# zehuichen123/Graph-DETR4D

Measured on AMD Instinct MI355X. Metric: decoder_samples_per_sec_900q_T4, higher is better.
Workload: dtype f32 (bf16x3 GEMMs)

## Files before the change

graph-detr4d_amd/csrc/gd4d_rowchain.hip:

```cpp
#include <stdlib.h>

#include "gd4d_common.h"
#include "gd4d_bf16x3.h"
#include "gd4d_pyramid_fill.h"
#include "gd4d_mha_dropout.h"
#include "gd4d_value_proj_body.h"

namespace gd4d {

GD4D_TRACE_UNIT(rowchain)

constexpr int RC_M = 16;
#ifndef RC_WAVES_N
#define RC_WAVES_N 8
#endif
#ifndef RC_TILES_N
#define RC_TILES_N 2
#endif
constexpr int RC_WAVES = RC_WAVES_N;
#ifndef RC_KPERM
#define RC_KPERM 1
#endif
#ifndef RC_LD_N
#define RC_LD_N 520
#endif
constexpr int RC_W = 512;
constexpr int RC_LD = RC_LD_N;
static_assert(RC_LD >= RC_W + 4 && RC_LD % 4 == 0, "row pitch");
constexpr int RC_KG = RC_KPERM ? 4 : 8;
constexpr int RC_K2 = RC_KPERM ? 16 : 4;
constexpr int RC_BUFS = 4;
#ifndef RC_DEPTH_N
#define RC_DEPTH_N 2
#endif
constexpr int RC_DEPTH = RC_DEPTH_N;
constexpr int RC_TILES = RC_TILES_N;
constexpr int RC_COLS = 16 * RC_TILES;
constexpr int RC_ROWS_PER_WAVE = RC_M / RC_WAVES;
static_assert((RC_TILES == 1 || RC_TILES % 2 == 0) && RC_M % RC_WAVES == 0 && RC_WAVES * RC_COLS == 256, "a pass of all waves covers 256 columns");

typedef gd4d_chain_op ChainOp;

__device__ __forceinline__ float rc_act_in(float v, int flags) { return (flags & GD4D_CHAIN_INV_SIGMOID) ? inv_sigmoid(v) : v; }

#ifndef RC_ROTATE
#define RC_ROTATE 1
#endif
#ifndef RC_PREFETCH
#define RC_PREFETCH 1
#endif
#ifndef RC_TRACE_OPS
#define RC_TRACE_OPS 0
#endif
#ifndef RC_DBG
#define RC_DBG 0
#endif
template <int PLANES>
__global__ __launch_bounds__(256) void chain_weight_image_kernel(const float* __restrict__ w, char* __restrict__ img, int N, int K) {
  const int ksteps = K / 32;
  const int frag = blockIdx.x * 4 + (threadIdx.x >> 6), lane = threadIdx.x & 63;
  const int tiles = (N + 15) / 16;
  if (frag >= tiles * ksteps) return;
  const int t = frag / ksteps, s = frag - t * ksteps;
  const int n = 16 * t + (lane & 15);
  float v[8];
#pragma unroll
  for (int j = 0; j < 8; ++j) v[j] = n < N ? w[(size_t)n * K + 32 * s + RC_KG * (lane >> 4) + (j < 4 ? j : RC_K2 + j - 4)] : 0.f;
  char* dst = img + (size_t)frag * (PLANES * 1024) + lane * 16;
  if (PLANES == 3) {
    u32x4 h, m, l;
    split8x3(v, h, m, l);
    *reinterpret_cast<u32x4*>(dst) = h;
    *reinterpret_cast<u32x4*>(dst + 1024) = m;
    *reinterpret_cast<u32x4*>(dst + 2048) = l;
  } else {
    u32x4 h, l;
    split8(v, h, l);
    *reinterpret_cast<u32x4*>(dst) = h;
    *reinterpret_cast<u32x4*>(dst + 1024) = l;
  }
}

__global__ __launch_bounds__(256) void chain_weight_image_group_kernel(const gd4d_image_job* __restrict__ jobs, int count, int total) {
  __shared__ int s_frag0[GD4D_IMAGE_JOBS_MAX];
  for (int i = threadIdx.x; i < count; i += 256) s_frag0[i] = jobs[i].frag0;
  __syncthreads();
  const int frag = blockIdx.x * 4 + (threadIdx.x >> 6), lane = threadIdx.x & 63;
  if (frag >= total) return;
  int lo = 0, hi = count - 1;
  while (lo < hi) {
    const int mid = (lo + hi + 1) >> 1;
    if (s_frag0[mid] <= frag) lo = mid; else hi = mid - 1;
  }
  const gd4d_image_job J = jobs[lo];
  const int f = frag - J.frag0;
  const int R = J.rows[0] + J.rows[1] + J.rows[2];
  auto elem = [&](int r, int c) -> float {
    if (r >= R || c >= J.cols) return 0.f;
    int j = 0;
    if (r >= J.rows[0]) { r -= J.rows[0]; j = 1; if (r >= J.rows[1]) { r -= J.rows[1]; j = 2; } }
    return J.seg[j][(size_t)r * J.cols + c];
  };
  if (J.planes == 0) {
    const int i = f * 64 + lane;
    if (i < R) static_cast<float*>(J.image)[i] = elem(i, 0);
    return;
  }
  const int N = J.transposed ? J.cols : R, K = J.transposed ? R : J.cols;
  const int ksteps = ((K + 63) & ~63) / 32;
  const int t = f / ksteps, s = f - t * ksteps;
  const int n = 16 * t + (lane & 15);
  float v[8];
  if (!J.transposed && (J.cols & 3) == 0 && RC_KG == 4) {
    float4 a = make_float4(0.f, 0.f, 0.f, 0.f), b = a;
    if (n < N) {
      int r = n, j = 0;
      if (r >= J.rows[0]) { r -= J.rows[0]; j = 1; if (r >= J.rows[1]) { r -= J.rows[1]; j = 2; } }
      const float* rowp = J.seg[j] + (size_t)r * J.cols + 32 * s + RC_KG * (lane >> 4);
      if (32 * s + RC_KG * (lane >> 4) + 3 < J.cols) a = *reinterpret_cast<const float4*>(rowp);
      if (32 * s + RC_KG * (lane >> 4) + RC_K2 + 3 < J.cols) b = *reinterpret_cast<const float4*>(rowp + RC_K2);
    }
    v[0] = a.x; v[1] = a.y; v[2] = a.z; v[3] = a.w; v[4] = b.x; v[5] = b.y; v[6] = b.z; v[7] = b.w;
  } else {
#pragma unroll
    for (int j = 0; j < 8; ++j) {
      const int k = 32 * s + RC_KG * (lane >> 4) + (j < 4 ? j : RC_K2 + j - 4);
      v[j] = n < N ? (J.transposed ? elem(k, n) : elem(n, k)) : 0.f;
    }
  }
  char* dst = static_cast<char*>(J.image) + (size_t)f * (J.planes * 1024) + lane * 16;
  if (J.planes == 3) {
    u32x4 h, m, l;
    split8x3(v, h, m, l);
    *reinterpret_cast<u32x4*>(dst) = h;
    *reinterpret_cast<u32x4*>(dst + 1024) = m;
    *reinterpret_cast<u32x4*>(dst + 2048) = l;
  } else {
    u32x4 h, l;
    split8(v, h, l);
    *reinterpret_cast<u32x4*>(dst) = h;
    *reinterpret_cast<u32x4*>(dst + 1024) = l;
  }
}

template <bool EXACT, bool TRAIN>
__device__ __forceinline__ void rc_gemm(const ChainOp& op, float (*bufs)[RC_M][RC_LD], int m0, int M, int lane, int wave) {
  constexpr int FRAG = EXACT ? 3072 : 2048;
  const int i16 = lane & 15, g = lane >> 4;
  const int K = op.K, N = op.N;
  const int steps = K / 32, tiles = (N + 15) / 16;
  const char* img = reinterpret_cast<const char*>(op.p0);
  const bool src2 = (op.flags & GD4D_CHAIN_SRC2) != 0, split_out = (op.flags & GD4D_CHAIN_SPLIT_OUT) != 0;
  const bool split_kv = (op.flags & GD4D_CHAIN_SPLIT_KV) != 0;
  const bool kv_fp32_too = (op.flags & GD4D_CHAIN_SPLIT_KV_KEEP) != 0;
  const bool mask_p2 = TRAIN && (op.flags & GD4D_CHAIN_MASK_P2) != 0;
  const float mask_scale = op.eps != 0.f ? op.eps : 1.f;
  const bool drop = TRAIN && (op.flags & GD4D_CHAIN_DROPOUT) != 0;
  const uint32_t drop_lo = drop ? reinterpret_cast<const uint32_t*>(op.p3)[0] : 0u;
  const uint32_t drop_hi = drop ? reinterpret_cast<const uint32_t*>(op.p3)[1] : 0u;
  for (int n_base = RC_COLS * wave; n_base < N; n_base += RC_COLS * RC_WAVES) {
    const float* a_row = &bufs[(src2 && n_base >= op.ld0) ? op.res : op.src][i16][RC_KG * g];
    const char* wf[RC_TILES];
#pragma unroll
    for (int c = 0; c < RC_TILES; ++c) wf[c] = img + (size_t)min(n_base / 16 + c, tiles - 1) * steps * FRAG + lane * 16;
    f32x4 acc[RC_TILES];
#pragma unroll
    for (int c = 0; c < RC_TILES; ++c) acc[c] = f32x4{0.f, 0.f, 0.f, 0.f};
    float e_bias[RC_TILES];
    {
      const float* bias_p = op.p1 ? op.p1 : reinterpret_cast<const float*>(op.p0);
      const float bias_on = op.p1 ? 1.f : 0.f;
#pragma unroll
      for (int c = 0; c < RC_TILES; ++c) e_bias[c] = bias_p[min(n_base + 16 * c + i16, N - 1)] * bias_on;
    }
    float e_add[RC_TILES][4];
    if (op.p2 && !split_out && !split_kv) {
#pragma unroll
      for (int c = 0; c < RC_TILES; ++c) {
        const int n = min(n_base + 16 * c + i16, N - 1);
#pragma unroll
        for (int r = 0; r < 4; ++r) {
          const size_t m = (size_t)min(m0 + 4 * g + r, M - 1);
          const float a2 = op.p2[m * op.ld2 + n];
          e_add[c][r] = (op.p3 && !drop) ? a2 + op.p3[m * op.ld1 + n] : a2;
        }
      }
    }
    u32x4 bh[RC_DEPTH][RC_TILES], bl[RC_DEPTH][RC_TILES], bm[EXACT ? RC_DEPTH : 1][RC_TILES];
    auto issue = [&](int slot, int j) {
      if (RC_DBG & 2) return;
#pragma unroll
      for (int c = 0; c < RC_TILES; ++c) {
        bh[slot][c] = *reinterpret_cast<const u32x4*>(wf[c] + (size_t)j * FRAG);
        if (EXACT) bm[slot][c] = *reinterpret_cast<const u32x4*>(wf[c] + (size_t)j * FRAG + 1024);
        bl[slot][c] = *reinterpret_cast<const u32x4*>(wf[c] + (size_t)j * FRAG + (EXACT ? 2048 : 1024));
      }
    };
    if (RC_DBG & 2) {
#pragma unroll
      for (int d = 0; d < RC_DEPTH; ++d)
#pragma unroll
        for (int c = 0; c < RC_TILES; ++c) { bh[d][c] = u32x4{1u, 2u, 3u, (unsigned)lane}; bl[d][c] = bh[d][c]; if (EXACT) bm[d][c] = bh[d][c]; }
    }
    const int rot = RC_ROTATE ? (int)(((unsigned)(m0 / RC_M) >> 3) % (unsigned)steps) : 0;
    auto kstep = [&](int j) { const int r = j + rot; return r >= steps ? r - steps : r; };
#pragma unroll
    for (int d = 0; d < RC_DEPTH; ++d) issue(d, kstep(min(d, steps - 1)));
    auto consume = [&](int d, int j0_) {
      const int j = kstep(j0_);
      const float4 t0 = *reinterpret_cast<const float4*>(a_row + 32 * j);
      const float4 t1 = *reinterpret_cast<const float4*>(a_row + 32 * j + RC_K2);
      const float a[8] = {t0.x, t0.y, t0.z, t0.w, t1.x, t1.y, t1.z, t1.w};
      if (EXACT) {
        u32x4 ah, am, al;
        split8x3(a, ah, am, al);
#pragma unroll
        for (int c = 0; c < RC_TILES; ++c) {
          acc[c] = __builtin_amdgcn_mfma_f32_16x16x32_bf16(frag(al), frag(bh[d][c]), acc[c], 0, 0, 0);
          acc[c] = __builtin_amdgcn_mfma_f32_16x16x32_bf16(frag(ah), frag(bl[d][c]), acc[c], 0, 0, 0);
          acc[c] = __builtin_amdgcn_mfma_f32_16x16x32_bf16(frag(am), frag(bm[d][c]), acc[c], 0, 0, 0);
          acc[c] = __builtin_amdgcn_mfma_f32_16x16x32_bf16(frag(am), frag(bh[d][c]), acc[c], 0, 0, 0);
          acc[c] = __builtin_amdgcn_mfma_f32_16x16x32_bf16(frag(ah), frag(bm[d][c]), acc[c], 0, 0, 0);
          acc[c] = __builtin_amdgcn_mfma_f32_16x16x32_bf16(frag(ah), frag(bh[d][c]), acc[c], 0, 0, 0);
        }
        return;
      }
      u32x4 ah, al;
      split8(a, ah, al);
      if (RC_DBG & 1) { asm volatile("" ::"v"(ah), "v"(al), "v"(bh[d][0]), "v"(bl[d][3])); return; }
#pragma unroll
      for (int c = 0; c < RC_TILES; ++c) {
        acc[c] = __builtin_amdgcn_mfma_f32_16x16x32_bf16(frag(ah), frag(bh[d][c]), acc[c], 0, 0, 0);
        acc[c] = __builtin_amdgcn_mfma_f32_16x16x32_bf16(frag(al), frag(bh[d][c]), acc[c], 0, 0, 0);
        acc[c] = __builtin_amdgcn_mfma_f32_16x16x32_bf16(frag(ah), frag(bl[d][c]), acc[c], 0, 0, 0);
      }
    };
    for (int j0 = 0; j0 + RC_DEPTH < steps; j0 += RC_DEPTH) {
#pragma unroll
      for (int d = 0; d < RC_DEPTH; ++d) {
        consume(d, j0 + d);
        issue(d, kstep(j0 + d + RC_DEPTH));
      }
    }
#pragma unroll
    for (int d = 0; d < RC_DEPTH; ++d) consume(d, steps - RC_DEPTH + d);
#pragma unroll
    for (int c = 0; c < RC_TILES; ++c) {
      const int n = n_base + 16 * c + i16;
      if (n >= N) continue;
      float kv[4] = {0.f, 0.f, 0.f, 0.f};
#pragma unroll
      for (int r = 0; r < 4; ++r) {
        const int row = 4 * g + r, m = m0 + row;
        float v = acc[c][r] + e_bias[c];
        if (op.flags & GD4D_CHAIN_RELU) v = fmaxf(v, 0.f);
        if (op.flags & GD4D_CHAIN_SIGMOID) v = 1.0f / (1.0f + expf(-v));
        if (drop) v = mha_drop_keep(drop_lo, drop_hi, (uint32_t)m * (uint32_t)N + (uint32_t)n, (uint32_t)op.reserved) ? v * op.eps : 0.f;
        if (mask_p2) v = e_add[c][r] > 0.f ? v * mask_scale : 0.f;
        if (op.res >= 0 && !src2) v += bufs[op.res][row][n];
        if (op.p2 && !split_out && !mask_p2 && !split_kv) v += e_add[c][r];
        if (split_kv) kv[r] = v;
        if (op.dst >= 0) bufs[op.dst][row][op.dst_col + n] = v;
        if (split_out) {
          if (m < M) {
            const int c1 = op.ldg, c2 = op.ldg + op.ld2;
            float* o = n < c1 ? op.gout + (size_t)m * op.ldg + n
                     : n < c2 ? const_cast<float*>(op.p2) + (size_t)m * op.ld2 + (n - c1)
                              : const_cast<float*>(op.p3) + (size_t)m * op.ld1 + (n - c2);
            *o = v;
          }
        } else if (op.gout && m < M && !(split_kv && !kv_fp32_too && n_base >= RC_COLS * RC_WAVES)) {
          op.gout[(size_t)m * op.ldg + n] = v;
        }
      }
      if (split_kv && n_base >= RC_COLS * RC_WAVES) {
        const unsigned h01 = cvt_pk_bf16(kv[0], kv[1]), h23 = cvt_pk_bf16(kv[2], kv[3]);
        const unsigned l01 = cvt_pk_bf16(kv[0] - __uint_as_float(h01 << 16), kv[1] - __uint_as_float(h01 & 0xffff0000u));
        const unsigned l23 = cvt_pk_bf16(kv[2] - __uint_as_float(h23 << 16), kv[3] - __uint_as_float(h23 & 0xffff0000u));
        constexpr int C3 = RC_COLS * RC_WAVES;
        const int blk = m0 / RC_M, blocks = (M + RC_M - 1) / RC_M;
        if (n_base < 2 * C3) {
          const int nn = n - C3, hd = nn >> 5, cc = nn & 31;
          unsigned short* kh = reinterpret_cast<unsigned short*>(const_cast<float*>(op.p2)) +
                               (((size_t)hd * blocks + blk) * 64 + (cc >> 3) * 16 + 4 * g) * 8 + (cc & 7);
          unsigned short* kl = kh + op.ld2;
          const unsigned hh[4] = {h01 & 0xffffu, h01 >> 16, h23 & 0xffffu, h23 >> 16};
          const unsigned ll[4] = {l01 & 0xffffu, l01 >> 16, l23 & 0xffffu, l23 >> 16};
#pragma unroll
          for (int r = 0; r < 4; ++r) { kh[r * 8] = (unsigned short)hh[r]; kl[r * 8] = (unsigned short)ll[r]; }
        } else {
          const int nn = n - 2 * C3, hd = nn >> 5, dd = nn & 31, steps = (blocks + 1) >> 1;
          unsigned short* vh = reinterpret_cast<unsigned short*>(const_cast<float*>(op.p3)) +
                               ((((size_t)hd * steps + (blk >> 1)) * 2 + (dd >> 4)) * 64 + 16 * g + (dd & 15)) * 8 + 4 * (blk & 1);
          unsigned short* vl = vh + op.ld1;
          *reinterpret_cast<uint2*>(vh) = make_uint2(h01, h23);
          *reinterpret_cast<uint2*>(vl) = make_uint2(l01, l23);
          if (blk == blocks - 1 && !(blk & 1)) {
            *reinterpret_cast<uint2*>(vh + 4) = make_uint2(0u, 0u);
            *reinterpret_cast<uint2*>(vl + 4) = make_uint2(0u, 0u);
          }
        }
      }
    }
  }
}

__device__ __forceinline__ void rc_headgemm(const ChainOp& op, float (*bufs)[RC_M][RC_LD], int m0, int M, int lane, int wave) {
  constexpr int HD = 2;
  const int i16 = lane & 15, g = lane >> 4;
  const int K = op.K, N = op.N, heads = op.ld0, Dh = N / heads;
  const int steps = K / 32, tiles = (N + 15) / 16;
  const char* img = reinterpret_cast<const char*>(op.p0);
  const int m_ld = min(m0 + i16, M - 1);
  for (int n_base = RC_COLS * wave; n_base < N; n_base += RC_COLS * RC_WAVES) {
    const char* wf[RC_TILES];
#pragma unroll
    for (int c = 0; c < RC_TILES; ++c) wf[c] = img + (size_t)min(n_base / 16 + c, tiles - 1) * steps * 2048 + lane * 16;
    constexpr int TPG = RC_TILES >= 2 ? 2 : 1;
    constexpr int NG = RC_TILES / TPG;
    int hg[NG];
    const float* ag[NG];
#pragma unroll
    for (int gi = 0; gi < NG; ++gi) {
      hg[gi] = min((n_base + 16 * TPG * gi) / Dh, heads - 1);
      ag[gi] = op.p2 + ((size_t)m_ld * heads + hg[gi]) * K + RC_KG * g;
    }
    f32x4 acc[RC_TILES];
#pragma unroll
    for (int c = 0; c < RC_TILES; ++c) acc[c] = f32x4{0.f, 0.f, 0.f, 0.f};
    float e_bias[RC_TILES];
    {
      const float* bias_p = op.p1 ? op.p1 : reinterpret_cast<const float*>(op.p0);
      const float bias_on = op.p1 ? 1.f : 0.f;
#pragma unroll
      for (int c = 0; c < RC_TILES; ++c) e_bias[c] = bias_p[min(n_base + 16 * c + i16, N - 1)] * bias_on;
    }
    float addend[RC_TILES][4];
    if (op.flags & GD4D_CHAIN_ADD_GOUT) {
#pragma unroll
      for (int c = 0; c < RC_TILES; ++c)
#pragma unroll
        for (int r = 0; r < 4; ++r)
          addend[c][r] = op.gout[(size_t)min(m0 + 4 * g + r, M - 1) * op.ldg + min(n_base + 16 * c + i16, N - 1)];
    }
    u32x4 bh[HD][RC_TILES], bl[HD][RC_TILES];
    float4 av[HD][NG][2];
    auto issue = [&](int slot, int j) {
#pragma unroll
      for (int c = 0; c < RC_TILES; ++c) {
        bh[slot][c] = *reinterpret_cast<const u32x4*>(wf[c] + (size_t)j * 2048);
        bl[slot][c] = *reinterpret_cast<const u32x4*>(wf[c] + (size_t)j * 2048 + 1024);
      }
#pragma unroll
      for (int gi = 0; gi < NG; ++gi) {
        av[slot][gi][0] = *reinterpret_cast<const float4*>(ag[gi] + 32 * j);
        av[slot][gi][1] = *reinterpret_cast<const float4*>(ag[gi] + 32 * j + RC_K2);
      }
    };
    auto consume = [&](int d) {
#pragma unroll
      for (int hh = 0; hh < NG; ++hh) {
        const float a[8] = {av[d][hh][0].x, av[d][hh][0].y, av[d][hh][0].z, av[d][hh][0].w,
                            av[d][hh][1].x, av[d][hh][1].y, av[d][hh][1].z, av[d][hh][1].w};
        u32x4 ah, al;
        split8(a, ah, al);
#pragma unroll
        for (int c = TPG * hh; c < TPG * hh + TPG; ++c) {
          acc[c] = __builtin_amdgcn_mfma_f32_16x16x32_bf16(frag(ah), frag(bh[d][c]), acc[c], 0, 0, 0);
          acc[c] = __builtin_amdgcn_mfma_f32_16x16x32_bf16(frag(al), frag(bh[d][c]), acc[c], 0, 0, 0);
          acc[c] = __builtin_amdgcn_mfma_f32_16x16x32_bf16(frag(ah), frag(bl[d][c]), acc[c], 0, 0, 0);
        }
      }
    };
#pragma unroll
    for (int d = 0; d < HD; ++d) issue(d, min(d, steps - 1));
    for (int j0 = 0; j0 + HD < steps; j0 += HD) {
#pragma unroll
      for (int d = 0; d < HD; ++d) {
        consume(d);
        issue(d, j0 + d + HD);
      }
    }
#pragma unroll
    for (int d = 0; d < HD; ++d) consume(d);
#pragma unroll
    for (int c = 0; c < RC_TILES; ++c) {
      const int n = n_base + 16 * c + i16;
      if (n >= N) continue;
      const int hc = hg[c / TPG];
#pragma unroll
      for (int r = 0; r < 4; ++r) {
        const int row = 4 * g + r, m = m0 + row;
        float v = fmaf(e_bias[c], op.p3[(size_t)min(m, M - 1) * heads + hc], acc[c][r]);
        if (op.res >= 0) v += bufs[op.res][row][n];
        if (op.flags & GD4D_CHAIN_ADD_GOUT) v += addend[c][r];
        if (op.dst >= 0) bufs[op.dst][row][op.dst_col + n] = v;
        if (op.gout && !(op.flags & GD4D_CHAIN_ADD_GOUT) && m < M) op.gout[(size_t)m * op.ldg + n] = v;
      }
    }
  }
}

__device__ __forceinline__ void rc_layernorm(const ChainOp& op, float (*bufs)[RC_M][RC_LD], int m0, int M, int lane, int wave) {
  constexpr int MAXCH = RC_W / 64;
  if (wave >= RC_M / 4) return;
  const int row = 4 * wave + (lane >> 4), l16 = lane & 15, N = op.N, nch = N / 64;
  float4 gm[MAXCH], bt[MAXCH], x[MAXCH], ad[MAXCH];
  const bool second = op.res >= 0 && op.p2;
  const size_t m_ld = (size_t)min(m0 + row, M - 1);
#pragma unroll
  for (int ch = 0; ch < MAXCH; ++ch) {
    const int n = min(64 * ch, N - 64) + 4 * l16;
    gm[ch] = *reinterpret_cast<const float4*>(op.p0 + n);
    bt[ch] = *reinterpret_cast<const float4*>(op.p1 + n);
    if (second) ad[ch] = *reinterpret_cast<const float4*>(op.p2 + m_ld * op.ld2 + n);
    x[ch] = *reinterpret_cast<const float4*>(&bufs[op.src][row][n]);
  }
  float s = 0.f;
#pragma unroll
  for (int ch = 0; ch < MAXCH; ++ch)
    if (ch < nch) s += (x[ch].x + x[ch].y) + (x[ch].z + x[ch].w);
#pragma unroll
  for (int o = 1; o < 16; o <<= 1) s += __shfl_xor(s, o);
  const float mean = s / (float)N;
  float q = 0.f;
#pragma unroll
  for (int ch = 0; ch < MAXCH; ++ch)
    if (ch < nch) {
      const float a = x[ch].x - mean, b = x[ch].y - mean, c = x[ch].z - mean, d = x[ch].w - mean;
      q += (a * a + b * b) + (c * c + d * d);
    }
#pragma unroll
  for (int o = 1; o < 16; o <<= 1) q += __shfl_xor(q, o);
  const float rstd = 1.0f / sqrtf(q / (float)N + op.eps);
  const int m = m0 + row;
  const bool relu = op.flags & GD4D_CHAIN_RELU;
#pragma unroll
  for (int ch = 0; ch < MAXCH; ++ch) {
    if (ch >= nch) break;
    const int n = 64 * ch + 4 * l16;
    float4 v;
    v.x = (x[ch].x - mean) * rstd * gm[ch].x + bt[ch].x; v.y = (x[ch].y - mean) * rstd * gm[ch].y + bt[ch].y;
    v.z = (x[ch].z - mean) * rstd * gm[ch].z + bt[ch].z; v.w = (x[ch].w - mean) * rstd * gm[ch].w + bt[ch].w;
    if (relu) { v.x = fmaxf(v.x, 0.f); v.y = fmaxf(v.y, 0.f); v.z = fmaxf(v.z, 0.f); v.w = fmaxf(v.w, 0.f); }
    if (op.dst >= 0) *reinterpret_cast<float4*>(&bufs[op.dst][row][n]) = v;
    if (op.gout && m < M) *reinterpret_cast<float4*>(op.gout + (size_t)m * op.ldg + n) = v;
    if (second)
      *reinterpret_cast<float4*>(&bufs[op.res][row][n]) = make_float4(ad[ch].x + v.x, ad[ch].y + v.y, ad[ch].z + v.z, ad[ch].w + v.w);
  }
}

__device__ __forceinline__ void rc_layernorm_bwd(const ChainOp& op, float (*bufs)[RC_M][RC_LD], float* scratch, int m0, int M, int wg,
                                                 int tid) {
  constexpr int MAXCH = RC_W / 64;
  const int lane = tid & 63, wave = tid >> 6;
  const int N = op.N, nch = N / 64;
  const bool relu = op.flags & GD4D_CHAIN_RELU;
  if (wave < RC_M / 4) {
    const int row = 4 * wave + (lane >> 4), l16 = lane & 15;
    const bool live = m0 + row < M;
    float4 gm[MAXCH], bt[MAXCH], x[MAXCH], d[MAXCH];
#pragma unroll
    for (int ch = 0; ch < MAXCH; ++ch) {
      const int n = min(64 * ch, N - 64) + 4 * l16;
      gm[ch] = *reinterpret_cast<const float4*>(op.p0 + n);
      bt[ch] = relu ? *reinterpret_cast<const float4*>(op.p1 + n) : make_float4(0.f, 0.f, 0.f, 0.f);
      x[ch] = op.p3 ? *reinterpret_cast<const float4*>(op.p3 + (size_t)min(m0 + row, M - 1) * op.ld1 + n)
                    : *reinterpret_cast<const float4*>(&bufs[op.res][row][n]);
      d[ch] = *reinterpret_cast<const float4*>(&bufs[op.src][row][n]);
      if (!live) d[ch] = make_float4(0.f, 0.f, 0.f, 0.f);
    }
    float s = 0.f;
#pragma unroll
    for (int ch = 0; ch < MAXCH; ++ch)
      if (ch < nch) s += (x[ch].x + x[ch].y) + (x[ch].z + x[ch].w);
#pragma unroll
    for (int o = 1; o < 16; o <<= 1) s += __shfl_xor(s, o);
    const float mean = s / (float)N;
    float q = 0.f;
#pragma unroll
    for (int ch = 0; ch < MAXCH; ++ch)
      if (ch < nch) {
        const float a = x[ch].x - mean, b = x[ch].y - mean, c = x[ch].z - mean, e = x[ch].w - mean;
        q += (a * a + b * b) + (c * c + e * e);
      }
#pragma unroll
    for (int o = 1; o < 16; o <<= 1) q += __shfl_xor(q, o);
    const float rstd = 1.0f / sqrtf(q / (float)N + op.eps);
    float s1 = 0.f, s2 = 0.f;
    float4 xh[MAXCH], g[MAXCH];
#pragma unroll
    for (int ch = 0; ch < MAXCH; ++ch) {
      xh[ch] = make_float4((x[ch].x - mean) * rstd, (x[ch].y - mean) * rstd, (x[ch].z - mean) * rstd, (x[ch].w - mean) * rstd);
      if (relu) {
        if (xh[ch].x * gm[ch].x + bt[ch].x <= 0.f) d[ch].x = 0.f;
        if (xh[ch].y * gm[ch].y + bt[ch].y <= 0.f) d[ch].y = 0.f;
        if (xh[ch].z * gm[ch].z + bt[ch].z <= 0.f) d[ch].z = 0.f;
        if (xh[ch].w * gm[ch].w + bt[ch].w <= 0.f) d[ch].w = 0.f;
      }
      g[ch] = make_float4(d[ch].x * gm[ch].x, d[ch].y * gm[ch].y, d[ch].z * gm[ch].z, d[ch].w * gm[ch].w);
      if (ch < nch) {
        s1 += (g[ch].x + g[ch].y) + (g[ch].z + g[ch].w);
        s2 += (g[ch].x * xh[ch].x + g[ch].y * xh[ch].y) + (g[ch].z * xh[ch].z + g[ch].w * xh[ch].w);
      }
    }
#pragma unroll
    for (int o = 1; o < 16; o <<= 1) { s1 += __shfl_xor(s1, o); s2 += __shfl_xor(s2, o); }
    const float m1 = s1 / (float)N, m2 = s2 / (float)N;
    const int m = m0 + row;
#pragma unroll
    for (int ch = 0; ch < MAXCH; ++ch) {
      if (ch >= nch) break;
      const int n = 64 * ch + 4 * l16;
      const float4 v = make_float4(rstd * (g[ch].x - m1 - xh[ch].x * m2), rstd * (g[ch].y - m1 - xh[ch].y * m2),
                                   rstd * (g[ch].z - m1 - xh[ch].z * m2), rstd * (g[ch].w - m1 - xh[ch].w * m2));
      if (op.dst >= 0) *reinterpret_cast<float4*>(&bufs[op.dst][row][n]) = v;
      if (op.gout && m < M) *reinterpret_cast<float4*>(op.gout + (size_t)m * op.ldg + n) = v;
      if (op.p2) {
        float4 a = make_float4(d[ch].x * xh[ch].x, d[ch].y * xh[ch].y, d[ch].z * xh[ch].z, d[ch].w * xh[ch].w), b = d[ch];
#pragma unroll
        for (int o = 16; o < 64; o <<= 1) {
          a.x += __shfl_xor(a.x, o); a.y += __shfl_xor(a.y, o); a.z += __shfl_xor(a.z, o); a.w += __shfl_xor(a.w, o);
          b.x += __shfl_xor(b.x, o); b.y += __shfl_xor(b.y, o); b.z += __shfl_xor(b.z, o); b.w += __shfl_xor(b.w, o);
        }
        if (lane < 16) {
          *reinterpret_cast<float4*>(scratch + (wave * 2 + 0) * RC_W + n) = a;
          *reinterpret_cast<float4*>(scratch + (wave * 2 + 1) * RC_W + n) = b;
        }
      }
    }
  }
  if (!op.p2) return;
  __syncthreads();
  float* part = const_cast<float*>(op.p2);
  for (int e = tid; e < 2 * N; e += 64 * RC_WAVES) {
    const int k = e / N, c = e - k * N;
    const float t = (scratch[(0 * 2 + k) * RC_W + c] + scratch[(1 * 2 + k) * RC_W + c]) +
                    (scratch[(2 * 2 + k) * RC_W + c] + scratch[(3 * 2 + k) * RC_W + c]);
    part[((size_t)wg * 2 + k) * N + c] = t;
  }
}

template <bool IS_ADD, bool TRAIN>
__device__ __forceinline__ void rc_rows(const ChainOp& op, float (*bufs)[RC_M][RC_LD], int m0, int M, int lane, int wave) {
  const int N = op.N;
  const float* ga = IS_ADD ? op.p2 : op.p0;
  const float* gb = IS_ADD ? nullptr : op.p1;
  const int lda = IS_ADD ? op.ld2 : op.ld0, ldb = op.ld1;
  float4 va[RC_ROWS_PER_WAVE][2], vb[RC_ROWS_PER_WAVE][2];
#pragma unroll
  for (int r = 0; r < RC_ROWS_PER_WAVE; ++r) {
    const int m = min(m0 + RC_ROWS_PER_WAVE * wave + r, M - 1);
#pragma unroll
    for (int cb = 0; cb < 2; ++cb) {
      const int n = min(256 * cb + 4 * lane, N - 4);
      va[r][cb] = ga ? *reinterpret_cast<const float4*>(ga + (size_t)m * lda + n) : make_float4(0.f, 0.f, 0.f, 0.f);
      vb[r][cb] = gb ? *reinterpret_cast<const float4*>(gb + (size_t)m * ldb + n) : make_float4(0.f, 0.f, 0.f, 0.f);
    }
  }
#pragma unroll
  for (int r = 0; r < RC_ROWS_PER_WAVE; ++r) {
    const int row = RC_ROWS_PER_WAVE * wave + r;
#pragma unroll
    for (int cb = 0; cb < 2; ++cb) {
      const int n = 256 * cb + 4 * lane;
      if (n >= N) continue;
      float4 v = va[r][cb];
      if (!IS_ADD && (op.flags & GD4D_CHAIN_INV_SIGMOID)) { v.x = inv_sigmoid(v.x); v.y = inv_sigmoid(v.y); v.z = inv_sigmoid(v.z); v.w = inv_sigmoid(v.w); }
      v.x += vb[r][cb].x; v.y += vb[r][cb].y; v.z += vb[r][cb].z; v.w += vb[r][cb].w;
      if (IS_ADD) {
        const float4 s0 = *reinterpret_cast<const float4*>(&bufs[op.src][row][n]);
        v.x += s0.x; v.y += s0.y; v.z += s0.z; v.w += s0.w;
        if (op.res >= 0) {
          const float4 s1 = *reinterpret_cast<const float4*>(&bufs[op.res][row][n]);
          v.x += s1.x; v.y += s1.y; v.z += s1.z; v.w += s1.w;
        }
      }
      *reinterpret_cast<float4*>(&bufs[op.dst][row][(IS_ADD ? 0 : op.dst_col) + n]) = v;
      if (TRAIN && op.gout && m0 + row < M) *reinterpret_cast<float4*>(op.gout + (size_t)(m0 + row) * op.ldg + n) = v;
    }
  }
}

struct ChainProgram {
  int nops, M, nops2, split;
  ChainOp ops[GD4D_CHAIN_MAX_OPS];
};

#if defined(__HIP_DEVICE_COMPILE__)
typedef const __attribute__((address_space(4))) ChainProgram* rc_prog_ptr_t;
#else
typedef const ChainProgram* rc_prog_ptr_t;
#endif

template <bool TRAIN>
__device__ __forceinline__ void row_chain_body(const rc_prog_ptr_t pp, const int bx) {
  const int M = pp->M, split = pp->split;
  const int blocks = (M + RC_M - 1) / RC_M;
  if (split > 0 && bx >= blocks && bx < split) return;
  const bool second = split > 0 && bx >= split;
  const int op_base = second ? pp->nops : 0;
  const int nops = second ? pp->nops2 : pp->nops;
  const int wg = second ? bx - split : bx;
  const int wg_lo = second ? split : 0, wg_hi = wg_lo + blocks;
  extern __shared__ __attribute__((aligned(16))) char rc_smem[];
  float (*bufs)[RC_M][RC_LD] = reinterpret_cast<float (*)[RC_M][RC_LD]>(rc_smem);
  const int tid = threadIdx.x, lane = tid & 63, wave = tid >> 6;
  const int m0 = wg * RC_M;
  trace_mark_if(g_trace_rowchain, (second ? 7ull : 1ull) | ((unsigned long long)nops << 8), wg == 0);
#if RC_PREFETCH
  typedef __attribute__((address_space(3))) void rc_lds_void_t;
  typedef const __attribute__((address_space(1))) void rc_glb_void_t;
  rc_lds_void_t* rc_dump = (rc_lds_void_t*)(rc_smem + sizeof(float) * RC_BUFS * RC_M * RC_LD + 256 * wave);
  auto touch1 = [&](const char* q) { __builtin_amdgcn_global_load_lds((rc_glb_void_t*)q, rc_dump, 4, 0, 0); };
  const unsigned xcd = (unsigned)bx & 7u;
  const unsigned first = (unsigned)wg_lo + ((xcd - (unsigned)wg_lo) & 7u);
  const unsigned mine = ((unsigned)bx - first) >> 3, share = ((unsigned)wg_hi - 1u - first) / 8u + 1u;
  auto touch = [&](const void* base, size_t bytes) {
    if (!base || bytes < 4) return;
    const char* b = reinterpret_cast<const char*>(base);
    const unsigned pieces = (unsigned)((bytes + 63) / 64) + 1u;
    for (unsigned c = tid; c < pieces; c += 64 * RC_WAVES) touch1(b + min((size_t)c * 64, bytes - 4));
  };
  auto touch_small = [&](int from) {
    const int rows = min(RC_M, M - m0);
    for (int oi = from; oi < op_base + nops; ++oi) {
      const ChainOp& o = pp->ops[oi];
      const size_t nb = (size_t)o.N * 4;
      switch (o.kind) {
        case GD4D_CHAIN_LOAD:
          for (int r = 0; r < rows; ++r) {
            touch(o.p0 + (size_t)(m0 + r) * o.ld0, nb);
            if (o.p1) touch(o.p1 + (size_t)(m0 + r) * o.ld1, nb);
          }
          break;
        case GD4D_CHAIN_ADD:
          if (o.p2) for (int r = 0; r < rows; ++r) touch(o.p2 + (size_t)(m0 + r) * o.ld2, nb);
          break;
        case GD4D_CHAIN_GEMM: touch(o.p1, nb); break;
        case GD4D_CHAIN_HEADGEMM: touch(o.p1, nb); touch(o.p3 + (size_t)m0 * o.ld0, (size_t)rows * o.ld0 * 4); break;
        case GD4D_CHAIN_LAYERNORM: touch(o.p0, nb); touch(o.p1, nb); break;
        case GD4D_CHAIN_SMALL_LINEAR: touch(o.p0, nb * o.K); touch(o.p1, nb); break;
        case GD4D_CHAIN_REFINE: touch(o.p0 + (size_t)m0 * 3, (size_t)rows * 12); break;
        default: break;
      }
    }
  };
  auto touch_images = [&]() {
    for (int oi = op_base; oi < op_base + nops; ++oi) {
      if (pp->ops[oi].kind == GD4D_CHAIN_HEADGEMM) {
        const int rows = min(RC_M, M - m0);
        const char* a = reinterpret_cast<const char*>(pp->ops[oi].p2 + (size_t)m0 * pp->ops[oi].ld0 * pp->ops[oi].K);
        const unsigned pieces = (unsigned)rows * (unsigned)pp->ops[oi].ld0 * (unsigned)pp->ops[oi].K / 16u;
        for (unsigned c = tid; c < pieces; c += 64 * RC_WAVES) touch1(a + (size_t)c * 64);
      }
      if (pp->ops[oi].kind != GD4D_CHAIN_GEMM && pp->ops[oi].kind != GD4D_CHAIN_HEADGEMM) continue;
      const char* img = reinterpret_cast<const char*>(pp->ops[oi].p0);
      const unsigned chunks = (unsigned)((pp->ops[oi].N + 15) / 16) * (unsigned)(pp->ops[oi].K / 32) *
                              ((pp->ops[oi].flags & GD4D_CHAIN_EXACT) ? 48u : 32u);
      const unsigned lo = (unsigned)((unsigned long long)chunks * mine / share), hi = (unsigned)((unsigned long long)chunks * (mine + 1) / share);
      for (unsigned c = lo + tid; c < hi; c += 64 * RC_WAVES) touch1(img + (size_t)c * 64);
    }
  };
  int lead = 0;
  if (RC_PREFETCH & 4)
    while (lead < nops && pp->ops[op_base + lead].kind == GD4D_CHAIN_LOAD) ++lead;
  if (RC_PREFETCH & 2) touch_small(op_base + lead);
  if ((RC_PREFETCH & 1) && lead == 0) touch_images();
#endif
  __shared__ int rc_poison;
  if (tid == 0) rc_poison = 0;
  bool poisoned = false;
  for (int oi = op_base; oi < op_base + nops; ++oi) {
#if RC_PREFETCH
    if ((RC_PREFETCH & 1) && lead > 0 && oi == op_base + lead) touch_images();
#endif
    const ChainOp op = pp->ops[oi];
    switch (op.kind) {
      case GD4D_CHAIN_LOAD: {
        if ((op.N & 3) == 0 && (op.dst_col & 3) == 0) { rc_rows<false, TRAIN>(op, bufs, m0, M, lane, wave); break; }
        for (int e = tid; e < RC_M * op.N; e += 64 * RC_WAVES) {
          const int row = e / op.N, n = e - row * op.N;
          const int m = min(m0 + row, M - 1);
          float v = rc_act_in(op.p0[(size_t)m * op.ld0 + n], op.flags);
          if (op.p1) v += op.p1[(size_t)m * op.ld1 + n];
          bufs[op.dst][row][op.dst_col + n] = v;
          if (TRAIN && op.gout && m0 + row < M) op.gout[(size_t)(m0 + row) * op.ldg + n] = v;
        }
        break;
      }
      case GD4D_CHAIN_GEMM:
        if (op.flags & GD4D_CHAIN_EXACT) rc_gemm<true, TRAIN>(op, bufs, m0, M, lane, wave);
        else rc_gemm<false, TRAIN>(op, bufs, m0, M, lane, wave);
        break;
      case GD4D_CHAIN_HEADGEMM: rc_headgemm(op, bufs, m0, M, lane, wave); break;
      case GD4D_CHAIN_LAYERNORM: rc_layernorm(op, bufs, m0, M, lane, wave); break;
      case GD4D_CHAIN_ADD: rc_rows<true, TRAIN>(op, bufs, m0, M, lane, wave); break;
      case GD4D_CHAIN_DROPMASK: {
        if (!TRAIN) break;
        const uint32_t lo = reinterpret_cast<const uint32_t*>(op.p0)[0], hi = reinterpret_cast<const uint32_t*>(op.p0)[1];
        const int nv = op.N / 4;
        for (int e = tid; e < RC_M * nv; e += 64 * RC_WAVES) {
          const int row = e / nv, n = 4 * (e - row * nv);
          const uint32_t id = (uint32_t)(m0 + row) * (uint32_t)op.N + (uint32_t)n;
          float4 v = *reinterpret_cast<const float4*>(&bufs[op.src][row][n]);
          v.x = mha_drop_keep(lo, hi, id, (uint32_t)op.reserved) ? v.x * op.eps : 0.f;
          v.y = mha_drop_keep(lo, hi, id + 1, (uint32_t)op.reserved) ? v.y * op.eps : 0.f;
          v.z = mha_drop_keep(lo, hi, id + 2, (uint32_t)op.reserved) ? v.z * op.eps : 0.f;
          v.w = mha_drop_keep(lo, hi, id + 3, (uint32_t)op.reserved) ? v.w * op.eps : 0.f;
          *reinterpret_cast<float4*>(&bufs[op.dst][row][n]) = v;
          if (op.gout && m0 + row < M) *reinterpret_cast<float4*>(op.gout + (size_t)(m0 + row) * op.ldg + n) = v;
        }
        break;
      }
      case GD4D_CHAIN_LN_BWD:
        if (TRAIN)
          rc_layernorm_bwd(op, bufs, reinterpret_cast<float*>(rc_smem + sizeof(float) * RC_BUFS * RC_M * RC_LD + 256 * RC_WAVES), m0, M, wg, tid);
        break;
      case GD4D_CHAIN_SMALL_LINEAR: {
        const int K = op.K, N = op.N;
        if (op.flags & GD4D_CHAIN_INV_SIGMOID) {
          if (tid < RC_M * K) {
            const int row = tid / K, k = tid - row * K;
            bufs[op.src][row][8 + k] = inv_sigmoid(bufs[op.src][row][k]);
          }
          __syncthreads();
        }
        const int col0 = (op.flags & GD4D_CHAIN_INV_SIGMOID) ? 8 : 0;
        if ((64 * RC_WAVES) % N == 0) {
          const int n = tid % N;
          float w[8];
#pragma unroll
          for (int k = 0; k < 8; ++k) w[k] = k < K ? op.p0[(size_t)n * K + k] : 0.f;
          const float b = op.p1 ? op.p1[n] : 0.f;
          for (int row = tid / N; row < RC_M; row += (64 * RC_WAVES) / N) {
            float v = b;
#pragma unroll
            for (int k = 0; k < 8; ++k)
              if (k < K) v = fmaf(bufs[op.src][row][col0 + k], w[k], v);
            if (op.flags & GD4D_CHAIN_RELU) v = fmaxf(v, 0.f);
            bufs[op.dst][row][n] = v;
            if (TRAIN && op.gout && m0 + row < M) op.gout[(size_t)(m0 + row) * op.ldg + n] = v;
          }
        } else {
          for (int e = tid; e < RC_M * N; e += 64 * RC_WAVES) {
            const int row = e / N, n = e - row * N;
            float v = op.p1 ? op.p1[n] : 0.f;
            for (int k = 0; k < K; ++k) v = fmaf(bufs[op.src][row][col0 + k], op.p0[(size_t)n * K + k], v);
            if (op.flags & GD4D_CHAIN_RELU) v = fmaxf(v, 0.f);
            bufs[op.dst][row][n] = v;
            if (TRAIN && op.gout && m0 + row < M) op.gout[(size_t)(m0 + row) * op.ldg + n] = v;
          }
        }
        break;
      }
      case GD4D_CHAIN_REFINE: {
        if (tid < RC_M && m0 + tid < M) {
          const int m = m0 + tid;
          const float* t = bufs[op.src][tid];
          const float* r = op.p0 + (size_t)m * 3;
          float* o = op.gout + (size_t)m * 3;
          const float x = t[0] + inv_sigmoid(r[0]), y = t[1] + inv_sigmoid(r[1]), z = t[4] + inv_sigmoid(r[2]);
          o[0] = 1.0f / (1.0f + expf(-x));
          o[1] = 1.0f / (1.0f + expf(-y));
          o[2] = 1.0f / (1.0f + expf(-z));
          if (op.dst >= 0) { bufs[op.dst][tid][0] = o[0]; bufs[op.dst][tid][1] = o[1]; bufs[op.dst][tid][2] = o[2]; }
        } else if (tid < RC_M && op.dst >= 0) {
          bufs[op.dst][tid][0] = bufs[op.dst][tid][1] = bufs[op.dst][tid][2] = 0.5f;
        }
        break;
      }
      case GD4D_CHAIN_SIGNAL: {
        asm volatile("s_waitcnt vmcnt(0)" ::: "memory");
        __syncthreads();
        if (tid == 0) __hip_atomic_store(reinterpret_cast<unsigned*>(op.gout) + wg, 1u, __ATOMIC_RELAXED, __HIP_MEMORY_SCOPE_AGENT);
        break;
      }
      case GD4D_CHAIN_WAIT: {
        if (tid == 0) {
          const unsigned* f = reinterpret_cast<const unsigned*>(op.p0) + wg;
          unsigned spins = 0;
          while (__hip_atomic_load(f, __ATOMIC_RELAXED, __HIP_MEMORY_SCOPE_AGENT) == 0u) {
            if (++spins > (1u << 20)) {
              if (op.gout) atomicAdd(reinterpret_cast<unsigned*>(op.gout), 1u);
              rc_poison = 1;
              break;
            }
            __builtin_amdgcn_s_sleep(8);
          }
          if (!rc_poison) __hip_atomic_store(const_cast<unsigned*>(f), 0u, __ATOMIC_RELAXED, __HIP_MEMORY_SCOPE_AGENT);
        }
        break;
      }
      default: break;
    }
    __syncthreads();
    if (op.kind == GD4D_CHAIN_WAIT) poisoned = rc_poison != 0;
    if (poisoned && op.kind == GD4D_CHAIN_LOAD && op.dst >= 0) {
      for (int e = tid; e < RC_M * op.N; e += 64 * RC_WAVES) {
        const int row = e / op.N, n = e - row * op.N;
        bufs[op.dst][row][op.dst_col + n] = __builtin_nanf("");
        if (TRAIN && op.gout && m0 + row < M) op.gout[(size_t)(m0 + row) * op.ldg + n] = __builtin_nanf("");
      }
      __syncthreads();
    }
#if RC_TRACE_OPS
    trace_mark_if(g_trace_rowchain, 0x40ull | ((unsigned long long)op.kind << 8) | ((unsigned long long)op.N << 16) | ((unsigned long long)op.K << 32) | (second ? 1ull << 63 : 0ull), wg == 0);
#endif
  }
  trace_mark_if(g_trace_rowchain, (second ? 0x87ull : 0x81ull) | ((unsigned long long)nops << 8), wg == 0);
}

template <bool TRAIN>
__global__ __launch_bounds__(64 * RC_WAVES) void row_chain_kernel(const ChainProgram by_value) {
#if defined(__HIP_DEVICE_COMPILE__)
  const rc_prog_ptr_t pp = (rc_prog_ptr_t)__builtin_amdgcn_kernarg_segment_ptr();
#else
  const ChainProgram* pp = &by_value;
#endif
  (void)by_value;
  row_chain_body<TRAIN>(pp, (int)blockIdx.x);
}

template <bool IN_CHLAST>
__global__ __launch_bounds__(64 * RC_WAVES) void row_chain_guest_kernel(const ChainProgram by_value, const VpaParams guest, const int gbase,
                                                                         const int gcount) {
#if defined(__HIP_DEVICE_COMPILE__)
  const rc_prog_ptr_t pp = (rc_prog_ptr_t)__builtin_amdgcn_kernarg_segment_ptr();
#else
  const ChainProgram* pp = &by_value;
#endif
  (void)by_value;
  if ((int)blockIdx.x >= gbase) {
    extern __shared__ __attribute__((aligned(16))) char rc_smem[];
    trace_mark_if(g_trace_rowchain, 9ull, (int)blockIdx.x == gbase);
    value_proj_astat_body<RC_WAVES, false, false, false, 0, IN_CHLAST>(guest, (int)blockIdx.x - gbase, gcount, rc_smem);
    trace_mark_if(g_trace_rowchain, 0x89ull, (int)blockIdx.x == gbase);
    return;
  }
  row_chain_body<false>(pp, (int)blockIdx.x);
}

#ifndef RC_FILL_FP
#define RC_FILL_FP 8
#endif
__global__ __launch_bounds__(64 * RC_WAVES) void row_chain_fill_kernel(const ChainProgram by_value, const FillGuest fg, const int gbase,
                                                                        const int gcount) {
#if defined(__HIP_DEVICE_COMPILE__)
  const rc_prog_ptr_t pp = (rc_prog_ptr_t)__builtin_amdgcn_kernarg_segment_ptr();
#else
  const ChainProgram* pp = &by_value;
#endif
  (void)by_value;
  if ((int)blockIdx.x >= gbase) {
    const int rows0 = fg.BQ[0] * fg.HH, rows1 = fg.hdr[1] ? fg.BQ[1] * fg.HH : 0;
    const int wave = (int)(threadIdx.x >> 6), step = gcount * RC_WAVES;
    for (int ph = ((int)blockIdx.x - gbase) * RC_WAVES + wave; ph < rows0 + rows1; ph += step) {
      const int job = ph >= rows0 ? 1 : 0;
      pyramid_grad_fill_body<RC_FILL_FP>(fg.hdr[job], fg.pair[job], fg.slots[job], fg.cap_t, fg.HH, fg.BQ[job], fg.start, fg.rec,
                                         fg.order[job], fg.id_base[job], ph - (job ? rows0 : 0));
    }
    return;
  }
  row_chain_body<true>(pp, (int)blockIdx.x);
}

__global__ void xcd_placement_probe_kernel(int32_t* out) {
  unsigned v;
  asm volatile("s_getreg_b32 %0, hwreg(HW_REG_XCC_ID)" : "=s"(v));
  if (threadIdx.x == 0) out[blockIdx.x] = (int32_t)(v & 0xfu);
}

}

extern "C" void gd4d_trace_set_rowchain(unsigned long long* p) { gd4d::trace_set_rowchain(p); }

extern "C" size_t gd4d_chain_op_bytes(void) { return sizeof(gd4d_chain_op); }

extern "C" size_t gd4d_chain_weight_image_bytes(int N, int K) {
  if (N <= 0 || K <= 0 || K % 32 != 0) return 0;
  return (size_t)((N + 15) / 16) * (K / 32) * 2048;
}

extern "C" int gd4d_chain_weight_image(const float* weight, int N, int K, void* image, void* stream) {
  using namespace gd4d;
  if (!weight || !image || N <= 0 || K <= 0) return GD4D_EINVAL;
  if (K % 64 != 0) return GD4D_EUNSUPPORTED;
  if (!aligned16(image)) return GD4D_EALIGN;
  const int frags = ((N + 15) / 16) * (K / 32);
  hipLaunchKernelGGL(chain_weight_image_kernel<2>, dim3((frags + 3) / 4), dim3(256), 0, static_cast<hipStream_t>(stream), weight,
                     static_cast<char*>(image), N, K);
  return check_launch();
}

extern "C" size_t gd4d_chain_weight_image_exact_bytes(int N, int K) {
  if (N <= 0 || K <= 0 || K % 32 != 0) return 0;
  return (size_t)((N + 15) / 16) * (K / 32) * 3072;
}

extern "C" int gd4d_chain_weight_image_exact(const float* weight, int N, int K, void* image, void* stream) {
  using namespace gd4d;
  if (!weight || !image || N <= 0 || K <= 0) return GD4D_EINVAL;
  if (K % 64 != 0) return GD4D_EUNSUPPORTED;
  if (!aligned16(image)) return GD4D_EALIGN;
  const int frags = ((N + 15) / 16) * (K / 32);
  hipLaunchKernelGGL(chain_weight_image_kernel<3>, dim3((frags + 3) / 4), dim3(256), 0, static_cast<hipStream_t>(stream), weight,
                     static_cast<char*>(image), N, K);
  return check_launch();
}

extern "C" size_t gd4d_image_job_bytes(void) { return sizeof(gd4d_image_job); }

extern "C" int gd4d_chain_weight_image_group(const gd4d_image_job* jobs_device, int count, int total_frags, void* stream) {
  using namespace gd4d;
  if (!jobs_device || count <= 0 || total_frags <= 0) return GD4D_EINVAL;
  if (count > GD4D_IMAGE_JOBS_MAX) return GD4D_EUNSUPPORTED;
  hipLaunchKernelGGL(chain_weight_image_group_kernel, dim3((total_frags + 3) / 4), dim3(256), 0, static_cast<hipStream_t>(stream),
                     jobs_device, count, total_frags);
  return check_launch();
}

static int rc_validate(const gd4d_chain_op* program, int nops, int which) {
  const bool two_programs = which != 0;
  using namespace gd4d;
  for (int i = 0; i < nops; ++i) {
    const gd4d_chain_op& op = program[i];
    const bool buf_ok = op.src < RC_BUFS && op.dst < RC_BUFS && op.res < RC_BUFS;
    if (!buf_ok) return GD4D_EINVAL;
    switch (op.kind) {
      case GD4D_CHAIN_LOAD:
        if (!op.p0 || op.dst < 0 || op.N <= 0 || op.dst_col < 0 || op.dst_col + op.N > RC_W) return GD4D_EINVAL;
        if ((op.N & 3) == 0 && (op.dst_col & 3) == 0 &&
            (!aligned16(op.p0) || (op.ld0 & 3) || (op.p1 && (!aligned16(op.p1) || (op.ld1 & 3))))) return GD4D_EALIGN;
        if (op.gout && (op.N & 3) == 0 && (op.dst_col & 3) == 0 && (!aligned16(op.gout) || (op.ldg & 3))) return GD4D_EALIGN;
        break;
      case GD4D_CHAIN_GEMM:
        if (!op.p0 || op.src < 0 || op.K <= 0 || op.N <= 0 || (op.dst < 0 && !op.gout)) return GD4D_EINVAL;
        if (op.p3 && !op.p2 && !(op.flags & GD4D_CHAIN_DROPOUT)) return GD4D_EINVAL;
        if (op.K % (32 * RC_DEPTH) != 0 || op.K > RC_W) return GD4D_EUNSUPPORTED;
        if (op.dst >= 0 && (op.dst_col < 0 || op.dst_col + op.N > RC_W)) return GD4D_EINVAL;
        if (op.dst >= 0 && op.dst == op.src) return GD4D_EINVAL;
        if (!aligned16(op.p0)) return GD4D_EALIGN;
        if (op.flags & GD4D_CHAIN_SRC2)
          if (op.res < 0 || op.res == op.dst || op.ld0 <= 0 || op.ld0 % (RC_COLS * RC_WAVES) != 0 || op.ld0 >= op.N) return GD4D_EINVAL;
        if ((op.flags & GD4D_CHAIN_DROPOUT) && (!op.p3 || ((uintptr_t)op.p3 & 7) || (op.flags & (GD4D_CHAIN_SPLIT_OUT | GD4D_CHAIN_MASK_P2))))
          return GD4D_EINVAL;
        if ((op.flags & GD4D_CHAIN_MASK_P2) && (!op.p2 || op.p3 || (op.flags & (GD4D_CHAIN_SPLIT_OUT | GD4D_CHAIN_SRC2)))) return GD4D_EINVAL;
        if (op.flags & GD4D_CHAIN_SPLIT_OUT)
          if (!op.gout || !op.p2 || !op.p3 || op.ldg <= 0 || op.ld2 <= 0 || op.ld1 <= 0 || op.ldg + op.ld2 + op.ld1 != op.N)
            return GD4D_EINVAL;
        if (op.flags & GD4D_CHAIN_SPLIT_KV) {
          if (op.flags & (GD4D_CHAIN_SPLIT_OUT | GD4D_CHAIN_MASK_P2 | GD4D_CHAIN_DROPOUT | GD4D_CHAIN_RELU | GD4D_CHAIN_SIGMOID)) return GD4D_EINVAL;
          if (op.N != 3 * RC_COLS * RC_WAVES) return GD4D_EUNSUPPORTED;
          if (!op.p2 || !op.p3 || op.ld2 <= 0 || op.ld1 <= 0 || (op.ld1 & 7) || (op.ld2 & 7)) return GD4D_EINVAL;
          if (!aligned16(op.p2) || !aligned16(op.p3)) return GD4D_EALIGN;
        }
        break;
      case GD4D_CHAIN_HEADGEMM:
        if (!op.p0 || !op.p2 || !op.p3 || op.K <= 0 || op.N <= 0 || op.ld0 <= 0 || (op.dst < 0 && !op.gout)) return GD4D_EINVAL;
        if (op.N % op.ld0 != 0 || (op.N / op.ld0) % 32 != 0 || op.K % 64 != 0 || op.N % 64 != 0) return GD4D_EUNSUPPORTED;
        if ((op.flags & GD4D_CHAIN_ADD_GOUT) && (!op.gout || op.dst < 0 || op.ldg < op.N)) return GD4D_EINVAL;
        if (op.dst >= 0 && (op.dst_col < 0 || op.dst_col + op.N > RC_W)) return GD4D_EINVAL;
        if (!aligned16(op.p0) || !aligned16(op.p2)) return GD4D_EALIGN;
        break;
      case GD4D_CHAIN_LAYERNORM:
        if (!op.p0 || !op.p1 || op.src < 0 || op.N <= 0 || op.N > RC_W || (op.dst < 0 && !op.gout)) return GD4D_EINVAL;
        if (op.N % 64 != 0) return GD4D_EUNSUPPORTED;
        if (!aligned16(op.p0) || !aligned16(op.p1) || (op.gout && (!aligned16(op.gout) || (op.ldg & 3)))) return GD4D_EALIGN;
        if (op.p2 && (op.res < 0 || op.res == op.src || op.res == op.dst)) return GD4D_EINVAL;
        if (op.p2 && (!aligned16(op.p2) || (op.ld2 & 3))) return GD4D_EALIGN;
        break;
      case GD4D_CHAIN_DROPMASK:
        if (!op.p0 || ((uintptr_t)op.p0 & 7) || op.src < 0 || op.dst < 0 || op.N <= 0 || op.N > RC_W || (op.N & 3)) return GD4D_EINVAL;
        if (op.gout && (!aligned16(op.gout) || (op.ldg & 3))) return GD4D_EALIGN;
        break;
      case GD4D_CHAIN_LN_BWD:
        if (!op.p0 || op.src < 0 || op.N <= 0 || op.N > RC_W) return GD4D_EINVAL;
        if (!op.p3 && (op.res < 0 || op.res == op.src || op.res == op.dst)) return GD4D_EINVAL;
        if (op.p3 && (!aligned16(op.p3) || (op.ld1 & 3) || op.ld1 < op.N)) return GD4D_EALIGN;
        if (op.dst < 0 && !op.gout && !op.p2) return GD4D_EINVAL;
        if ((op.flags & GD4D_CHAIN_RELU) && !op.p1) return GD4D_EINVAL;
        if (op.N % 64 != 0) return GD4D_EUNSUPPORTED;
        if (!aligned16(op.p0) || (op.p1 && !aligned16(op.p1)) || (op.gout && (!aligned16(op.gout) || (op.ldg & 3)))) return GD4D_EALIGN;
        break;
      case GD4D_CHAIN_ADD:
        if (op.src < 0 || op.dst < 0 || op.N <= 0 || op.N > RC_W || (op.N & 3)) return GD4D_EINVAL;
        if (op.p2 && (!aligned16(op.p2) || (op.ld2 & 3))) return GD4D_EALIGN;
        if (op.gout && (!aligned16(op.gout) || (op.ldg & 3))) return GD4D_EALIGN;
        break;
      case GD4D_CHAIN_SMALL_LINEAR:
        if (!op.p0 || op.src < 0 || op.dst < 0 || op.dst == op.src || op.K <= 0 || op.K > 8 || op.N <= 0 || op.N > RC_W)
          return GD4D_EINVAL;
        break;
      case GD4D_CHAIN_REFINE:
        if (op.src < 0 || !op.p0 || !op.gout || (op.dst >= 0 && op.dst == op.src)) return GD4D_EINVAL;
        break;
      case GD4D_CHAIN_SIGNAL:
        if (!op.gout || !two_programs || which != 1) return GD4D_EINVAL;
        break;
      case GD4D_CHAIN_WAIT:
        if (!op.p0 || !op.gout || !two_programs || which != 2 || i + 1 >= nops || program[i + 1].kind != GD4D_CHAIN_LOAD) return GD4D_EINVAL;
        break;
      default: return GD4D_EINVAL;
    }
  }
  return GD4D_OK;
}

static int rc_launch(const gd4d_chain_op* a, int na, const gd4d_chain_op* b, int nb, int M, void* stream,
                     const gd4d_chain_guest* guest = nullptr, const gd4d::FillGuest* fills = nullptr, int fill_workgroups = 0) {
  using namespace gd4d;
  if (!a || na <= 0 || M <= 0 || nb < 0 || (nb > 0 && !b)) return GD4D_EINVAL;
  if (na + nb > GD4D_CHAIN_MAX_OPS) return GD4D_EUNSUPPORTED;
  if (int rc = rc_validate(a, na, nb > 0 ? 1 : 0)) return rc;
  if (nb > 0)
    if (int rc = rc_validate(b, nb, 2)) return rc;
  for (int w = 0; w < 2; ++w)
    for (int i = 0; i < (w ? nb : na); ++i) {
      const gd4d_chain_op& op = (w ? b : a)[i];
      if (op.kind == GD4D_CHAIN_GEMM && (op.flags & GD4D_CHAIN_SPLIT_KV)) {
        const long long blocks = (M + RC_M - 1) / RC_M, heads = RC_COLS * RC_WAVES / 32;
        if (op.ld2 < heads * blocks * 512 || op.ld1 < heads * ((blocks + 1) / 2) * 1024) return GD4D_EINVAL;
      }
    }
  bool train = false;
  for (int w = 0; w < 2; ++w) {
    const gd4d_chain_op* pr = w ? b : a;
    for (int i = 0; i < (w ? nb : na); ++i) {
      const gd4d_chain_op& op = pr[i];
      train = train || op.kind == GD4D_CHAIN_LN_BWD || op.kind == GD4D_CHAIN_DROPMASK ||
              (op.kind == GD4D_CHAIN_GEMM && (op.flags & (GD4D_CHAIN_MASK_P2 | GD4D_CHAIN_DROPOUT))) ||
              ((op.kind == GD4D_CHAIN_LOAD || op.kind == GD4D_CHAIN_ADD || op.kind == GD4D_CHAIN_SMALL_LINEAR) && op.gout);
    }
  }
  VpaParams g{};
  if (guest) {
    if (train) return GD4D_EUNSUPPORTED;
    if (int rc = va_guest_params(guest, g)) return rc;
  }
  const size_t lds = sizeof(float) * RC_BUFS * RC_M * RC_LD + 256 * RC_WAVES + (train ? sizeof(float) * 8 * RC_W : 0);
  const void* kern = train ? reinterpret_cast<const void*>(row_chain_kernel<true>) : reinterpret_cast<const void*>(row_chain_kernel<false>);
  if (!allow_dynamic_lds(kern, (int)lds)) return GD4D_ELAUNCH;
  const int blocks = (M + RC_M - 1) / RC_M;
  ChainProgram prog{};
  const int split = nb > 0 ? (blocks + 7) & ~7 : 0;
  prog.nops = na; prog.M = M; prog.nops2 = nb; prog.split = split;
  for (int i = 0; i < na; ++i) prog.ops[i] = a[i];
  for (int i = 0; i < nb; ++i) prog.ops[na + i] = b[i];
  if (guest) {
    const int base = g.total;
    if (va_lds_bytes(1, false, RC_WAVES) > lds) return GD4D_EUNSUPPORTED;
    const int chain_wgs = nb > 0 ? split + blocks : blocks;
    const int gbase = chain_wgs;
    int cus = 256, dev = 0;
    if (hipGetDevice(&dev) != hipSuccess || hipDeviceGetAttribute(&cus, hipDeviceAttributeMultiprocessorCount, dev) != hipSuccess || cus <= 0) cus = 256;
    const int need = (base + RC_WAVES - 1) / RC_WAVES;
    int gcount = guest->workgroups > 0 ? guest->workgroups : cus;
    if (gcount < 8) gcount = 8;
    if (gcount > need) gcount = need;
    auto go = [&](auto kern) -> int {
      if (!allow_dynamic_lds(reinterpret_cast<const void*>(kern), (int)lds)) return GD4D_ELAUNCH;
      hipLaunchKernelGGL(kern, dim3(gbase + gcount), dim3(64 * RC_WAVES), lds, static_cast<hipStream_t>(stream), prog, g, gbase, gcount);
      return check_launch();
    };
    return g.in_chlast ? go(row_chain_guest_kernel<true>) : go(row_chain_guest_kernel<false>);
  }
  if (fills) {
    if (guest) return GD4D_EINVAL;
    const void* fk = reinterpret_cast<const void*>(row_chain_fill_kernel);
    const size_t flds = sizeof(float) * RC_BUFS * RC_M * RC_LD + 256 * RC_WAVES + sizeof(float) * 8 * RC_W;
    if (!allow_dynamic_lds(fk, (int)flds)) return GD4D_ELAUNCH;
    const int gbase = nb > 0 ? split + blocks : blocks;
    int cus = 256, dev = 0;
    if (hipGetDevice(&dev) != hipSuccess || hipDeviceGetAttribute(&cus, hipDeviceAttributeMultiprocessorCount, dev) != hipSuccess || cus <= 0) cus = 256;
    const int rows = fills->BQ[0] * fills->HH + (fills->hdr[1] ? fills->BQ[1] * fills->HH : 0);
    const int need = (rows + RC_WAVES - 1) / RC_WAVES;
    int gcount = fill_workgroups > 0 ? fill_workgroups : 2 * cus;
    if (gcount > need) gcount = need;
    if (gcount < 1) gcount = 1;
    hipLaunchKernelGGL(row_chain_fill_kernel, dim3(gbase + gcount), dim3(64 * RC_WAVES), flds, static_cast<hipStream_t>(stream), prog, *fills,
                       gbase, gcount);
    return check_launch();
  }
  if (train)
    hipLaunchKernelGGL(row_chain_kernel<true>, dim3(nb > 0 ? split + blocks : blocks), dim3(64 * RC_WAVES), lds, static_cast<hipStream_t>(stream), prog);
  else
    hipLaunchKernelGGL(row_chain_kernel<false>, dim3(nb > 0 ? split + blocks : blocks), dim3(64 * RC_WAVES), lds, static_cast<hipStream_t>(stream), prog);
  return check_launch();
}

extern "C" int gd4d_xcd_placement_probe(int32_t* out, int blocks, void* stream) {
  if (!out || blocks <= 0) return GD4D_EINVAL;
  hipLaunchKernelGGL(gd4d::xcd_placement_probe_kernel, dim3(blocks), dim3(64), 0, static_cast<hipStream_t>(stream), out);
  return gd4d::check_launch();
}

extern "C" int gd4d_row_chain_fwd(const gd4d_chain_op* program, int nops, int M, void* stream) {
  return rc_launch(program, nops, nullptr, 0, M, stream);
}

extern "C" int gd4d_row_chain2_fwd(const gd4d_chain_op* program_a, int nops_a, const gd4d_chain_op* program_b, int nops_b, int M,
                                   void* stream) {
  if (!program_b || nops_b <= 0) return GD4D_EINVAL;
  return rc_launch(program_a, nops_a, program_b, nops_b, M, stream);
}

extern "C" size_t gd4d_chain_guest_bytes(void) { return sizeof(gd4d_chain_guest); }

extern "C" int gd4d_row_chain_guest_fwd(const gd4d_chain_op* program_a, int nops_a, const gd4d_chain_op* program_b, int nops_b, int M,
                                        const gd4d_chain_guest* guest, void* stream) {
  if (!guest || nops_b < 0 || (nops_b > 0 && !program_b)) return GD4D_EINVAL;
  return rc_launch(program_a, nops_a, nops_b > 0 ? program_b : nullptr, nops_b, M, stream, guest);
}

extern "C" int gd4d_row_chain_fill_fwd(const gd4d_chain_op* program_a, int nops_a, const gd4d_chain_op* program_b, int nops_b, int M,
                                       const gd4d_fill_job* jobs, int njobs, const int32_t* start, void* records, int fill_B, int fill_N,
                                       int fill_Hh, int fill_P, int workgroups, void* stream) {
  using namespace gd4d;
  if (!jobs || njobs < 1 || njobs > 2 || !start || !records || fill_B <= 0 || fill_N <= 0 || fill_Hh <= 0) return GD4D_EINVAL;
  if (nops_b < 0 || (nops_b > 0 && !program_b) || workgroups < 0) return GD4D_EINVAL;
  if ((fill_P != kPoints && fill_P != 8) || fill_N > 64 || fill_B > 16 || fill_Hh > kPlanHdr) return GD4D_EUNSUPPORTED;
  FillGuest fg{};
  for (int j = 0; j < njobs; ++j) {
    const gd4d_fill_job& jb = jobs[j];
    if (!jb.plan || !jb.slots || jb.Q <= 0) return GD4D_EINVAL;
    if ((unsigned long long)jb.id_base + (unsigned long long)fill_B * jb.Q * fill_Hh > (1ull << 26)) return GD4D_EUNSUPPORTED;
    fg.hdr[j] = static_cast<const int*>(jb.plan);
    fg.pair[j] = reinterpret_cast<const uint2*>(static_cast<const char*>(jb.plan) + plan_hdr_bytes(fill_B, jb.Q));
    fg.slots[j] = static_cast<const uint2*>(jb.slots);
    fg.order[j] = jb.query_order;
    fg.id_base[j] = jb.id_base;
    fg.BQ[j] = fill_B * jb.Q;
  }
  fg.HH = fill_Hh;
  fg.cap_t = plan_cap_t(fill_N, fill_P);
  fg.start = start;
  fg.rec = static_cast<uint2*>(records);
  return rc_launch(program_a, nops_a, nops_b > 0 ? program_b : nullptr, nops_b, M, stream, nullptr, &fg, workgroups);
}
```

graph-detr4d_amd/functional.py:

```python
import numpy as np
import os

import torch

from . import _lib, ops


def wants_grad(module, *tensors):
    if not torch.is_grad_enabled():
        return False
    if any(t is not None and torch.is_tensor(t) and t.requires_grad for t in tensors):
        return True
    return module is not None and any(p.requires_grad for p in module.parameters())


def require_inference(*tensors):
    if torch.is_grad_enabled() and any(t is not None and t.requires_grad for t in tensors):
        raise NotImplementedError(
            'graph-detr4d_amd: this entry point has no backward - call it under torch.no_grad()')


def main_grad(t, rows=None):
    m = getattr(t, '_gd4d_main_grad', None) if t is not None else None
    if m is None or rows is None:
# ... 206 lines not shown
    return layer_norm(linear(x, weight, bias, **kw), norm, relu=relu_after)


def take_fused_norm(kwargs, autograd=False):
    holder = kwargs.get(NORM_KEY)
    if holder is None or holder['done'] or bool(holder.get('autograd')) != autograd:
        return None
    return holder


def position_encoder(seq, ref):
    if ref.shape[-1] <= 4 and seq[0].out_features % 4 == 0 and seq[0].out_features <= 1024:
        h = ops.small_linear_layernorm_fwd(ref.contiguous(), seq[0].weight.contiguous(), seq[0].bias,
                                           seq[1].weight.contiguous(), seq[1].bias.contiguous(), seq[1].eps,
                                           relu=True, inv_sigmoid_in=True)
    else:
        h = linear(ref, seq[0].weight, seq[0].bias, inv_sigmoid_in=True)
        h = layer_norm(h, seq[1], relu=True)
    return linear_norm(h, seq[3].weight, seq[3].bias, seq[4], relu_after=True)


def use_head_major(value_dtype):
    import os
    o = os.environ.get('GD4D_VALUE_LAYOUT')
    if o in ('pixel', 'head'):
        return o == 'head'
    return value_dtype == torch.bfloat16


def value_projection(value, weight, bias, num_heads, out_dtype=torch.float32, max_cus=0):
    shapes = [tuple(v.shape[-2:]) for v in value]
    b, n, c = value[0].shape[:3]
    hm = use_head_major(out_dtype)
    out = ops.value_proj_fwd([v.contiguous() for v in value], weight.contiguous(),
                             None if bias is None else bias.contiguous(), out_dtype,
                             num_heads=num_heads, head_major=hm, bf16_math=out_dtype == torch.bfloat16, max_cus=max_cus)
    return (out if hm else out.view(b * n, -1, num_heads, c // num_heads)), shapes


def run_branch(branch, x):
    nn = torch.nn
    mods = list(branch) if isinstance(branch, nn.Sequential) else None
    if not mods or not x.is_cuda or not all(isinstance(m, (nn.Linear, nn.ReLU, nn.LayerNorm)) for m in mods) \
            or not isinstance(mods[0], nn.Linear):
        return branch(x)
    i = 0
    while i < len(mods):
        m = mods[i]
        relu = i + 1 < len(mods) and isinstance(mods[i + 1], nn.ReLU)
        if isinstance(m, nn.Linear):
            x = linear(x, m.weight, m.bias, relu=relu)
        elif isinstance(m, nn.LayerNorm):
            x = layer_norm(x, m, relu=relu)
        else:
            x, relu = torch.relu(x), False
        i += 2 if relu else 1
    return x


def _branch_program(branch, x_rows, out_rows, exact=False, width=512):
    nn = torch.nn
    mods = list(branch) if isinstance(branch, nn.Sequential) else None
    if not mods or not isinstance(mods[0], nn.Linear) or not isinstance(mods[-1], nn.Linear):
        return None
    prog, src, i = [ops.chain_load(0, x_rows)], 0, 0
    while i < len(mods):
        m = mods[i]
        relu = i + 1 < len(mods) and isinstance(mods[i + 1], nn.ReLU)
        last = i + (2 if relu else 1) >= len(mods)
        dst = (src + 1) % 3
        if isinstance(m, nn.Linear):
            if m.in_features % 64 or m.in_features > width or (not last and (m.out_features % 64 or m.out_features > width)):
                return None
            prog.append(ops.chain_gemm(src, m.weight, m.bias, dst=-1 if last else dst, relu=relu, exact=exact,
                                       out=out_rows if last else None))
        elif isinstance(m, nn.LayerNorm) and not last:
            if len(m.normalized_shape) != 1 or m.normalized_shape[0] % 64 or m.weight is None:
                return None
            prog.append(ops.chain_layernorm(src, m, dst=dst, relu=relu))
        else:
            return None
        src = dst
        i += 2 if relu else 1
    return prog


def head_outputs(hs, init_reference, inter_references, cls_branches, reg_branches, pc_range, depth_factor=None):
    hs = hs.permute(0, 2, 1, 3)
    classes, coords = [], []
    if wants_grad(cls_branches, hs) or wants_grad(reg_branches):
        from .autograd import BoxHeadFunction
        tmps = []
        for lvl in range(hs.shape[0]):
            x = hs[lvl].contiguous()
            classes.append(sequential_autograd(cls_branches[lvl], x))
            tmps.append(sequential_autograd(reg_branches[lvl], x))
        refs = torch.cat([init_reference.unsqueeze(0), inter_references[:-1]], 0) if hs.shape[0] > 1 else init_reference.unsqueeze(0)
        boxes = BoxHeadFunction.apply(torch.stack(tmps), refs, pc_range, 1.0 if depth_factor is None else float(depth_factor))
        return {'all_cls_scores': torch.stack(classes), 'all_bbox_preds': boxes,
                'enc_cls_scores': None, 'enc_bbox_preds': None}
    chains = hs.is_cuda and hs.dtype == torch.float32 and os.environ.get('GD4D_HEAD_CHAINS', '1') != '0'
    for lvl in range(hs.shape[0]):
        reference = init_reference if lvl == 0 else inter_references[lvl - 1]
        x = hs[lvl].contiguous()
        if chains:
            rows = x.view(-1, x.shape[-1])
            last_c, last_r = cls_branches[lvl][-1], reg_branches[lvl][-1]
            if isinstance(last_c, torch.nn.Linear) and isinstance(last_r, torch.nn.Linear):
                cls = torch.empty(*x.shape[:-1], last_c.out_features, device=x.device, dtype=torch.float32)
                tmp = torch.empty(*x.shape[:-1], last_r.out_features, device=x.device, dtype=torch.float32)
                pc = _branch_program(cls_branches[lvl], rows, cls.view(rows.shape[0], -1))
                pr = _branch_program(reg_branches[lvl], rows, tmp.view(rows.shape[0], -1), exact=True)
                if pc is not None and pr is not None:
                    ops.row_chain2_fwd(pc, pr, rows.shape[0])
                    classes.append(cls)
                    coords.append(ops.box_head_fwd(tmp, reference.contiguous(), pc_range,
                                                   1.0 if depth_factor is None else float(depth_factor), out=tmp))
                    continue
        classes.append(run_branch(cls_branches[lvl], x))
        tmp = run_branch(reg_branches[lvl], x).contiguous()
        coords.append(ops.box_head_fwd(tmp, reference.contiguous(), pc_range,
                                       1.0 if depth_factor is None else float(depth_factor), out=tmp))
    return {'all_cls_scores': torch.stack(classes), 'all_bbox_preds': torch.stack(coords),
            'enc_cls_scores': None, 'enc_bbox_preds': None}


def refine_reference(tmp, reference_points):
    return ops.refine_reference_fwd(tmp.contiguous(), reference_points.contiguous())


VALUE_CACHE_KEY = '_gd4d_value_cache'


def project_values_for_layers(modules, value):
    shapes = [tuple(v.shape[-2:]) for v in value]
    b, n, c = value[0].shape[:3]
    hh = modules[0].num_heads
    hm = use_head_major(modules[0].value_dtype)
    outs = ops.value_proj_multi_fwd([v.contiguous() for v in value],
                                    [m.value_proj.weight.contiguous() for m in modules],
                                    [m.value_proj.bias.contiguous() for m in modules],
                                    modules[0].value_dtype, num_heads=hh, head_major=hm,
                                    bf16_math=modules[0].value_dtype == torch.bfloat16)
    return {id(m): ((o if hm else o.view(b * n, -1, hh, c // hh)), shapes, value) for m, o in zip(modules, outs)}


def raw_pyramid_for_training(modules, value):
    if os.environ.get('GD4D_TRAIN_VALUES', 'raw') != 'raw' or not LateValues.applicable(modules, value, ignore_mode=True):
        return None
    if any(v.dtype != torch.float32 for v in value):
        return None
    from .autograd import PyramidSourceFunction, RawPyramid
    raw = RawPyramid()
    raw.copy_dtype = modules[0].value_dtype
    token = PyramidSourceFunction.apply(raw, *value)
    shapes = [tuple(v.shape[-2:]) for v in value]
    return {id(m): (None, shapes, value, (raw, token)) for m in modules}


def project_values_for_layers_autograd(modules, value):
    from .autograd import ValueProjMultiFunction
    shapes = [tuple(v.shape[-2:]) for v in value]
    b, n, c = value[0].shape[:3]
    hh = modules[0].num_heads
    cl = None
    if LateValues.applicable(modules, value, ignore_mode=True):
        with torch.no_grad():
# ... 337 lines not shown
```

graph-detr4d_amd/fused_decoder.py:

```python
import ctypes
import os
import weakref

import torch
import torch.nn as nn

from . import _lib
from . import functional as Fn
from . import ops
from .deform3d_cross_attn import Deform3DCrossAttn
from .transformer_layers import FFN, MultiheadAttention

ORDER = ('self_attn', 'norm', 'cross_attn', 'norm', 'ffn', 'norm')
OFFSETS_EXACT = True


def _plain_reg_branch(branch, c):
    if not isinstance(branch, nn.Sequential) or len(branch) % 2 == 0:
        return None
    lins = []
    for i, m in enumerate(branch):
        if i % 2 == 0:
            if not isinstance(m, nn.Linear) or m.in_features != c or (i + 1 < len(branch) and m.out_features != c):
                return None
# ... 8 lines not shown
            decoder, query, query_pos, reference_points, *(value if isinstance(value, (list, tuple)) else ())):
        return False
    if not query.is_cuda or query.dtype != torch.float32 or query.dim() != 3 or query.shape[1] != 1:
        return False
    if reference_points is None or reference_points.shape[-1] != 3 or not isinstance(value, (list, tuple)):
        return False
    c = query.shape[-1]
    if c % 64 or c > 512:
        return False
    for layer in decoder.layers:
        if tuple(layer.operation_order) != ORDER or layer.training or len(layer.attentions) != 2 or len(layer.ffns) != 1:
            return False
        sa, ca, ffn = layer.attentions[0], layer.attentions[1], layer.ffns[0]
        if not isinstance(sa, MultiheadAttention) or sa.batch_first or sa.embed_dims != c:
            return False
        if type(ca) is not Deform3DCrossAttn or ca.embed_dims != c or len(value) != ca.num_levels:
            return False
        if ca.num_points not in ((1, 2, 4, 8) if ca.num_heads == 8 else (4,)):
            return False
        if not isinstance(ffn, FFN) or len(ffn.layers) != 3 or not ffn.add_identity or ffn.feedforward_channels % 64 \
                or ffn.feedforward_channels > 512:
            return False
    if attn_masks is not None and not (isinstance(attn_masks, (list, tuple)) or torch.is_tensor(attn_masks)):
        return False
    if reg_branches is not None and any(_plain_reg_branch(reg_branches[i], c) is None for i in range(len(decoder.layers))):
        return False
    return True


def takes_single_stream_loop(decoder, query, value, reference_points, reg_branches, attn_masks, query_pos):
    if not applicable(decoder, query, value, reference_points, reg_branches, attn_masks, query_pos=query_pos):
        return False
    c = query.shape[-1]
    return all((c // l.attentions[1].num_heads) % 32 == 0 and not l.attentions[1].depth_encode for l in decoder.layers)


def _in_proj_ops(sa, x_pos_buf, x_buf, qkv, kv=None):
    c = sa.embed_dims
    w, b = sa.attn.in_proj_weight, sa.attn.in_proj_bias
    if c % 128 == 0:
        return [ops.chain_gemm_two_sources(x_pos_buf, x_buf, 2 * c, w, b, qkv, kv=kv)]
    return [ops.chain_gemm(x_pos_buf, w[:2 * c], b[:2 * c], out=qkv[..., :2 * c]),
            ops.chain_gemm(x_buf, w[2 * c:], b[2 * c:], out=qkv[..., 2 * c:])]


def _kv_planes(layers, q, c, attn_mask, dev):
    if c != 256 or (attn_mask is not None and attn_mask.dim() != 2) or os.environ.get('GD4D_MHA_FP32') == '1':
        return None
    if layers[0].attentions[0].num_heads != 8:
        return None
    return ops.KVPlanes(q, c, dev, heads=8)


def initial_reference(linear, query_pos):
    q = query_pos.shape[0]
    out = torch.empty(1, q, linear.out_features, device=query_pos.device, dtype=torch.float32)
    if query_pos.device.index != torch.cuda.current_device():
        with torch.cuda.device(query_pos.device):
            return initial_reference(linear, query_pos)
    ops.row_chain_fwd([ops.chain_load(0, query_pos),
                       ops.chain_gemm(0, linear.weight, linear.bias, out=out.view(q, -1), sigmoid=True, exact=True)], q)
    return out


def fast_input(module, query_embed, mlvl_feats):
    return (os.environ.get('GD4D_FUSED_DECODER', '1') != '0' and query_embed.is_cuda and query_embed.dtype == torch.float32
            and mlvl_feats[0].size(0) == 1 and query_embed.dim() == 2 and query_embed.stride(1) == 1
            and query_embed.shape[1] % 8 == 0 and (query_embed.shape[1] // 2) % 128 == 0
            and not Fn.wants_grad(module, query_embed, *mlvl_feats))


def _position_features(ca, reference_points, q):
    ref3d = reference_points
    if ca.depth_encode:
        depth = (ref3d[..., 0:1] ** 2 + ref3d[..., 1:2] ** 2) ** 0.5
        ref3d = torch.cat([ref3d, depth], dim=-1).contiguous()
    seq = ca.position_encoder
    out = torch.empty(1, q, ca.embed_dims, device=ref3d.device, dtype=torch.float32)
    prog = [ops.chain_load(0, ref3d.view(q, -1), inv_sigmoid=True),
            ops.chain_small_linear(0, seq[0].weight, seq[0].bias, 1),
            ops.chain_layernorm(1, seq[1], dst=0, relu=True),
            ops.chain_gemm(0, seq[3].weight, seq[3].bias, dst=1),
            ops.chain_layernorm(1, seq[4], relu=True, out=out.view(q, -1))]
    ops.row_chain_fwd(prog, q)
    return out, ref3d


def _position_ops(ca, out, ref=None, ref_buf=None):
    seq = ca.position_encoder
    if ref_buf is None:
        head, src, inv = [ops.chain_load(0, ref, inv_sigmoid=True)], 0, False
    else:
        head, src, inv = [], ref_buf, True
    mid = 1 if src != 1 else 2
    nxt = [b for b in (0, 2, 3) if b not in (src, mid)][0]
    return head + [ops.chain_small_linear(src, seq[0].weight, seq[0].bias, mid, inv_sigmoid=inv),
                   ops.chain_layernorm(mid, seq[1], dst=nxt, relu=True),
                   ops.chain_gemm(nxt, seq[3].weight, seq[3].bias, dst=mid),
                   ops.chain_layernorm(mid, seq[4], relu=True, out=out)]


def run_single(decoder, query, query_pos, value, reference_points, reg_branches, img_metas, attn_masks, order,
               return_intermediate, late):
    q, _, c = query.shape
    dev = query.device
    layers = list(decoder.layers)
    nl = len(layers)
    if attn_masks is None:
        attn_masks = [None, None]
    elif torch.is_tensor(attn_masks):
        attn_masks = [attn_masks, attn_masks]
    lidar2img = Fn.lidar2img_device(img_metas, query)
    img_h, img_w = Fn.img_hw(img_metas)
    x = query[:, 0, :]
    pos = query_pos[:, 0, :]
    keep = []
    qkv = torch.empty(q, 1, 3 * c, device=dev, dtype=torch.float32)
    kv = _kv_planes(layers, q, c, attn_masks[0], dev)
    coarse = late.mode == 'sliced' and late.coarse_setup([l.attentions[1] for l in layers])
    first_guest = None
    if coarse and not late.take_first(layers[0].attentions[1]):
        first_guest = late.coarse_guest(layers[0].attentions[1])
    ops.row_chain_fwd([ops.chain_load(0, x, pos), ops.chain_load(1, x)] + _in_proj_ops(layers[0].attentions[0], 0, 1, qkv.view(q, -1), kv), q,
                      guest=first_guest)
    n_out = nl if return_intermediate else 1
    out_all = torch.empty(n_out, q, 1, c, device=dev, dtype=torch.float32)
    ref_all = torch.empty(n_out, 1, q, 3, device=dev, dtype=torch.float32)
    ref = reference_points.contiguous()
    pending = None
    pos_late = ops.handoff_enabled(dev, 'GD4D_POS_ENCODER')
    if pos_late:
        blocks = (q + 15) // 16
        flags = ops.handoff_flags(dev, nl, (blocks + 7) // 8 * 8 + 8, Fn.slot_key(dev))
        err = ops.handoff_error_word(dev)
        keep.append(flags)
    for lid, layer in enumerate(layers):
        sa, ca, ffn = layer.attentions[0], layer.attentions[1], layer.ffns[0]
        hh, npt, nlv, ncam = ca.num_heads, ca.num_points, ca.num_levels, ca.num_cams
        last = lid + 1 == nl
        slot = lid if return_intermediate else 0
        qh, kh, vh = qkv.split(c, dim=-1)
        if kv is not None:
            o = ops.mha_core_presplit_fwd(qh, kv, sa.num_heads, attn_masks[0])
        else:
            o = ops.mha_core_fwd(qh, kh, vh, sa.num_heads, attn_masks[0])

        x1 = torch.empty(q, c, device=dev, dtype=torch.float32)
        cam = torch.empty(1, q, ncam, device=dev, dtype=torch.float32)
        off = torch.empty(1, q, hh * npt * 3, device=dev, dtype=torch.float32)
        att = torch.empty(1, q, hh * nlv * npt, device=dev, dtype=torch.float32)
        prog_a = [ops.chain_load(0, o.view(q, c)),
                  ops.chain_gemm(0, sa.attn.out_proj.weight, sa.attn.out_proj.bias, dst=1, add=x),
                  ops.chain_layernorm(1, layer.norms[0], dst=2, out=x1, dst2=0, add=pos)]
        prog_a.append(ops.chain_gemm_three_outputs(
            0, [ca.cam_attention_weights, ca.deform_sampling_offsets, ca.attention_weights],
            [cam.view(q, -1), off.view(q, -1), att.view(q, -1)], exact=OFFSETS_EXACT))
        pos_feat = torch.empty(1, q, c, device=dev, dtype=torch.float32)
        if pending is not None:
            lins, x_prev, ref_prev, new_ref = pending
            prog_b, src, tmp = [ops.chain_load(3, x_prev)], 3, (1, 2)
            for i, lin in enumerate(lins):
                prog_b.append(ops.chain_gemm(src, lin.weight, lin.bias, dst=tmp[i % 2], relu=i + 1 < len(lins), exact=True))
                src = tmp[i % 2]
            park = 0 if src != 0 else 3
            prog_b.append(ops.chain_refine(src, ref_prev, new_ref, dst=-1 if pos_late else park))
            if not pos_late:
                prog_b += _position_ops(ca, pos_feat.view(q, c), ref_buf=park)
            keep += [x_prev, ref_prev]
            ref = new_ref
        else:
            prog_b = None if pos_late else _position_ops(ca, pos_feat.view(q, c), ref=ref.view(q, 3))
        if prog_b is None:
            ops.row_chain_fwd(prog_a, q)
        else:
            ops.row_chain2_fwd(prog_a, prog_b, q)

        if late.mode != 'sliced':
            agg = late.sample_aggregate(ca, ref, off.view(1, q, hh, npt, 3), att.view(1, q, hh, nlv, npt), cam, lidar2img,
                                        img_h, img_w, order=order)
            first = ops.chain_load(0, agg.view(q, c))
            agg_raw, wsum = agg, agg
        elif coarse:
            agg_raw, wsum, pagg = late.aggregate(ca, ref, off.view(1, q, hh, npt, 3), att.view(1, q, hh, nlv, npt), cam, lidar2img,
                                                 img_h, img_w, order=order, coarse=True)
            first = ops.chain_headgemm(agg_raw, wsum, ca.value_proj.weight, ca.value_proj.bias, dst=0, addend=pagg.view(q, c))
            keep.append(pagg)
        else:
            agg_raw, wsum = late.aggregate(ca, ref, off.view(1, q, hh, npt, 3), att.view(1, q, hh, nlv, npt), cam, lidar2img,
                                           img_h, img_w, order=order)
            first = ops.chain_headgemm(agg_raw, wsum, ca.value_proj.weight, ca.value_proj.bias, dst=0)
        guest = late.coarse_guest(layers[lid + 1].attentions[1]) if coarse and not last else None
        x3 = out_all[slot]
        prog = [first] + ([ops.chain_wait(flags[lid], err)] if pos_late else []) + [
                ops.chain_load(3, x1, pos_feat.view(q, c)),
                ops.chain_gemm(0, ca.output_proj.weight, ca.output_proj.bias, dst=1, res=3),
                ops.chain_layernorm(1, layer.norms[1], dst=2),
                ops.chain_gemm(2, ffn.layers[0][0].weight, ffn.layers[0][0].bias, dst=0, relu=True),
                ops.chain_gemm(0, ffn.layers[1].weight, ffn.layers[1].bias, dst=1, res=2)]
        if not last:
            qkv = torch.empty(q, 1, 3 * c, device=dev, dtype=torch.float32)
            prog.append(ops.chain_layernorm(1, layer.norms[2], dst=3, out=x3.view(q, c), dst2=0, add=pos))
            prog += _in_proj_ops(layers[lid + 1].attentions[0], 0, 3, qkv.view(q, -1), kv)
        else:
            prog.append(ops.chain_layernorm(1, layer.norms[2], dst=3, out=x3.view(q, c)))
        pending = None
        if reg_branches is not None:
            lins = _plain_reg_branch(reg_branches[lid], c)
            new_ref = ref_all[slot]
            if last:
                src, tmp = 3, (1, 2)
                for i, lin in enumerate(lins):
                    prog.append(ops.chain_gemm(src, lin.weight, lin.bias, dst=tmp[i % 2], relu=i + 1 < len(lins), exact=True))
                    src = tmp[i % 2]
                prog.append(ops.chain_refine(src, ref, new_ref))
            else:
                pending = (lins, x3.view(q, c), ref, new_ref)
        elif return_intermediate or last:
            ops.copy_into(ref_all[slot], ref)
        if pos_late:
            ops.row_chain2_fwd(_position_ops(ca, pos_feat.view(q, c), ref=ref.view(q, 3)) + [ops.chain_signal(flags[lid])], prog, q,
                               guest=guest)
        else:
            ops.row_chain_fwd(prog, q, guest=guest)
        keep += [o, x1, cam, off, att, agg_raw, wsum, pos_feat, x]
        x = x3.view(q, c)
    if pos_late and _lib.recorder() is None:
        ops.poll_handoff(dev)
    del keep
    return out_all, ref_all


def run(decoder, query, query_pos, value, reference_points, reg_branches, img_metas, attn_masks, pipeline, value_cache,
        order, order_pc_range, return_intermediate, late=None):
    if query.device.index != torch.cuda.current_device():
        with torch.cuda.device(query.device):
            return run(decoder, query, query_pos, value, reference_points, reg_branches, img_metas, attn_masks, pipeline,
                       value_cache, order, order_pc_range, return_intermediate, late=late)
    q, _, c = query.shape
    dev = query.device
    layers = list(decoder.layers)
    nl = len(layers)
    if late is not None and all((c // l.attentions[1].num_heads) % 32 == 0 and not l.attentions[1].depth_encode for l in layers):
        if order is None or order.numel() != q:
            order = Fn.query_order(reference_points.contiguous(), layers[0].attentions[1].pc_range)
        return run_single(decoder, query, query_pos, value, reference_points, reg_branches, img_metas, attn_masks, order,
                          return_intermediate, late)
    main = torch.cuda.current_stream(dev)
    aux = Fn.aux_stream(dev)
    if attn_masks is None:
        attn_masks = [None, None]
    elif torch.is_tensor(attn_masks):
        attn_masks = [attn_masks, attn_masks]
    lidar2img = Fn.lidar2img_device(img_metas, query)
    img_h, img_w = Fn.img_hw(img_metas)
    x = query[:, 0, :]
    pos = query_pos[:, 0, :]
    keep = []

    qkv = torch.empty(q, 1, 3 * c, device=dev, dtype=torch.float32)
    ops.row_chain_fwd([ops.chain_load(0, x, pos), ops.chain_load(1, x)] + _in_proj_ops(layers[0].attentions[0], 0, 1, qkv.view(q, -1)), q)

    n_out = nl if return_intermediate else 1
    out_all = torch.empty(n_out, q, 1, c, device=dev, dtype=torch.float32)
    ref_all = torch.empty(n_out, 1, q, 3, device=dev, dtype=torch.float32)
    ref = reference_points.contiguous()
    ref_event = None
    for lid, layer in enumerate(layers):
        sa, ca, ffn = layer.attentions[0], layer.attentions[1], layer.ffns[0]
        hh, npt, nlv, ncam = ca.num_heads, ca.num_points, ca.num_levels, ca.num_cams
        ev_pos = None
        if aux is not None:
            fork = torch.cuda.Event()
            fork.record(main)
            with torch.cuda.stream(aux):
                aux.wait_event(fork)
                pos_feat, ref_keep = _position_features(ca, ref, q)
                ev_pos = torch.cuda.Event()
                ev_pos.record(aux)
        else:
            if ref_event is not None:
                main.wait_event(ref_event)
            pos_feat, ref_keep = _position_features(ca, ref, q)
        keep += [pos_feat, ref_keep]

        qh, kh, vh = qkv.split(c, dim=-1)
        o = ops.mha_core_fwd(qh, kh, vh, sa.num_heads, attn_masks[0])

        x1 = torch.empty(q, c, device=dev, dtype=torch.float32)
        cam = torch.empty(1, q, ncam, device=dev, dtype=torch.float32)
        off = torch.empty(1, q, hh * npt * 3, device=dev, dtype=torch.float32)
        att = torch.empty(1, q, hh * nlv * npt, device=dev, dtype=torch.float32)
        prog = [ops.chain_load(0, o.view(q, c)),
                ops.chain_load(3, x),
                ops.chain_gemm(0, sa.attn.out_proj.weight, sa.attn.out_proj.bias, dst=1, res=3),
                ops.chain_layernorm(1, layer.norms[0], dst=2, out=x1),
                ops.chain_add(0, 2, c, add=pos),
                ops.chain_gemm(0, ca.cam_attention_weights.weight, ca.cam_attention_weights.bias, out=cam.view(q, -1)),
                ops.chain_gemm(0, ca.deform_sampling_offsets.weight, ca.deform_sampling_offsets.bias, out=off.view(q, -1)),
                ops.chain_gemm(0, ca.attention_weights.weight, ca.attention_weights.bias, out=att.view(q, -1))]
        ops.row_chain_fwd(prog, q)

# ... 7 lines not shown
                                           img_h, img_w, order=order)
            agg = agg_raw
        elif late is not None:
            agg = late.sample_aggregate(ca, ref, off.view(1, q, hh, npt, 3), att.view(1, q, hh, nlv, npt), cam, lidar2img,
                                        img_h, img_w, order=order)
        else:
            taken = pipeline.take(ca, value) if pipeline is not None else None
            cached = (value_cache or {}).get(id(ca))
            if taken is not None:
                val, shapes = taken
            elif cached is not None and cached[2] is value:
                val, shapes = cached[0], cached[1]
            else:
                val, shapes = Fn.value_projection(value, ca.value_proj.weight, ca.value_proj.bias, hh, ca.value_dtype)
            agg = Fn.sample_aggregate(val, shapes, ref, off.view(1, q, hh, npt, 3), att.view(1, q, hh, nlv, npt), cam,
                                      lidar2img, ca.pc_range, img_h, img_w, order=order)
            if taken is not None:
                del val, taken
                pipeline.gather_enqueued(ca)

        if ev_pos is not None:
            main.wait_event(ev_pos)
        last = lid + 1 == nl
        slot = lid if return_intermediate else 0
        x3 = out_all[slot]
        if agg_raw is not None:
            bias = ca.value_proj.bias
            first = ops.chain_headgemm(agg_raw, wsum, ca.value_proj.weight, bias, dst=0)
            keep.append(wsum)
        else:
            first = ops.chain_load(0, agg.view(q, c))
        prog = [first,
                ops.chain_load(3, x1, pos_feat.view(q, c)),
                ops.chain_gemm(0, ca.output_proj.weight, ca.output_proj.bias, dst=1, res=3),
                ops.chain_layernorm(1, layer.norms[1], dst=2),
                ops.chain_gemm(2, ffn.layers[0][0].weight, ffn.layers[0][0].bias, dst=0, relu=True),
                ops.chain_gemm(0, ffn.layers[1].weight, ffn.layers[1].bias, dst=1, res=2),
                ops.chain_layernorm(1, layer.norms[2], dst=3, out=x3.view(q, c))]
        if not last:
            qkv = torch.empty(q, 1, 3 * c, device=dev, dtype=torch.float32)
            prog += [ops.chain_add(0, 3, c, add=pos)] + _in_proj_ops(layers[lid + 1].attentions[0], 0, 3, qkv.view(q, -1))
        new_ref = None
        reg_prog = []
        if reg_branches is not None:
            lins = _plain_reg_branch(reg_branches[lid], c)
            src, tmp = 3, (1, 2)
            for i, lin in enumerate(lins):
                reg_prog.append(ops.chain_gemm(src, lin.weight, lin.bias, dst=tmp[i % 2], relu=i + 1 < len(lins), exact=True))
                src = tmp[i % 2]
            new_ref = ref_all[slot]
            reg_prog.append(ops.chain_refine(src, ref, new_ref))
        split_reg = bool(reg_prog) and aux is not None
        if not split_reg:
            prog += reg_prog
        ops.row_chain_fwd(prog, q)
        keep += [o, x1, cam, off, att, agg, x]

        x = x3.view(q, c)
        if new_ref is not None:
            old_ref, ref = ref, new_ref
            ref_event = None
            if aux is not None and (split_reg or (not last and order is not None)):
                done = torch.cuda.Event()
                done.record(main)
                with torch.cuda.stream(aux):
                    aux.wait_event(done)
                    if split_reg:
                        ops.row_chain_fwd([ops.chain_load(3, x)] + reg_prog, q)
                        keep.append(old_ref)
                    if not last and order is not None:
                        order = Fn.query_order(ref, order_pc_range)
                    ref_event = torch.cuda.Event()
                    ref_event.record(aux)
            elif not last and order is not None:
                order = Fn.query_order(ref, order_pc_range)
        if new_ref is None and (return_intermediate or last):
            ref_all[slot].copy_(ref)
    if aux is not None:
        main.wait_stream(aux)
    del keep
    return out_all, ref_all


ROUTE_SWITCHES = ('GD4D_POS_ENCODER', 'GD4D_COARSE', 'GD4D_FIRST_PROJ', 'GD4D_MHA_FP32', 'GD4D_AGG', 'GD4D_PLAN', 'GD4D_PROJECT',
                  'GD4D_COPY_CUS', 'GD4D_COARSE_MAX_ROWS', 'GD4D_QUERY_ORDER')
_PROGRAMS = weakref.WeakKeyDictionary()
_B_QUERY, _B_POS, _B_REF, _B_L2I, _B_IMG_H, _B_IMG_W, _B_MASK, _B_OUT, _B_REFS, _B_LEVEL0 = range(10)


def request_enabled():
    return os.environ.get('GD4D_REQUEST', '0') == '1' and _lib.recorder() is None and not torch.cuda.is_current_stream_capturing()


class RequestProgram:

    def __init__(self, decoder, query, query_pos, reference_points, reg_branches, value, img_metas, mask):
        dev = query.device
        self.device = dev
        self.sources = list(decoder.parameters()) + ([] if reg_branches is None else [p for b in reg_branches for p in b.parameters()])
        try:
            self.regs = None if reg_branches is None else weakref.ref(reg_branches)
        except TypeError:
            self.regs = (lambda held: (lambda: held))(reg_branches)
        self.stamp = ops._Stamp(self.sources)
        ops.handoff_enabled(dev, 'GD4D_POS_ENCODER')
        main = torch.cuda.current_stream(dev)
        lib = _lib.load()
        Fn.lidar2img_device(img_metas, query)
        self.pool = torch.cuda.MemPool()
        rec = ops.StepRecorder(lib, main.cuda_stream)
        kwargs = dict(key=None, value=value, query_pos=query_pos, img_metas=img_metas)
        if mask is not None:
            kwargs['attn_masks'] = [mask, None]
        with torch.cuda.use_mem_pool(self.pool, device=dev), _lib.recording(rec):
            outs, refs = decoder(query, reference_points=reference_points, reg_branches=reg_branches, **kwargs)
        lead = () if decoder.return_intermediate else (1,)
        self.out_shape, self.ref_shape = lead + tuple(outs.shape), lead + tuple(refs.shape)
        tensors = {_B_QUERY: query, _B_POS: query_pos, _B_REF: reference_points, _B_OUT: outs, _B_REFS: refs}
        if mask is not None:
            tensors[_B_MASK] = mask
        tensors.update({_B_LEVEL0 + i: v for i, v in enumerate(value)})
        self.nbindings = _B_LEVEL0 + len(value)
        steps, keep = rec.steps(tensors, {'lidar2img': _B_L2I, 'img_h': _B_IMG_H, 'img_w': _B_IMG_W})
        handle = ctypes.c_void_p()
        _lib.check(lib.gd4d_decoder_request_create(ctypes.addressof(steps), len(steps), self.nbindings, ctypes.addressof(handle)),
                   'gd4d_decoder_request_create')
        del keep
        self.handle, self.nsteps, self._lib = handle, len(steps), lib
        self.main, self.side = main.cuda_stream, rec.side
        self.bind = (ops.RequestBinding * self.nbindings)()
        self.polls = ops.handoff_enabled(dev, 'GD4D_POS_ENCODER')

    def valid(self, reg_branches=None):
        return self.handle is not None and (self.regs is None or self.regs() is reg_branches) and self.stamp.valid(self.sources)

    def describe(self):
        return [self._lib.gd4d_decoder_request_describe(self.handle, i).decode() for i in range(self.nsteps)]

    def run(self, query, query_pos, reference_points, value, img_metas, mask):
        b, dev = self.bind, self.device
        lidar2img = Fn.lidar2img_device(img_metas, query)
        img_h, img_w = Fn.img_hw(img_metas)
        out_all = torch.empty(self.out_shape, device=dev, dtype=torch.float32)
        ref_all = torch.empty(self.ref_shape, device=dev, dtype=torch.float32)
        b[_B_QUERY].ptr, b[_B_POS].ptr, b[_B_REF].ptr = query.data_ptr(), query_pos.data_ptr(), reference_points.data_ptr()
        b[_B_L2I].ptr, b[_B_IMG_H].scalar, b[_B_IMG_W].scalar = lidar2img.data_ptr(), img_h, img_w
        b[_B_MASK].ptr = None if mask is None else mask.data_ptr()
        b[_B_OUT].ptr, b[_B_REFS].ptr = out_all.data_ptr(), ref_all.data_ptr()
        for i, v in enumerate(value):
            b[_B_LEVEL0 + i].ptr = v.data_ptr()
        code = _lib.load().gd4d_decoder_request_run(self.handle, b, self.nbindings, self.main, self.side)
        _lib.check(code, 'gd4d_decoder_request_run')
        if self.polls:
            ops.poll_handoff(dev)
        return out_all, ref_all

    def close(self):
        if self.handle is not None:
            torch.cuda.synchronize(self.device)
            self._lib.gd4d_decoder_request_destroy(self.handle)
            self.handle = None

    def __del__(self):
        try:
            self.close()
        except Exception:
            pass
# ... 62 lines not shown
```

graph-detr4d_amd/ops.py:

```python
import ctypes
import functools
import inspect
import os
import weakref

import torch

from . import _lib


def _dev(t, name, dtype=None):
    if not t.is_cuda:
        raise _lib.Gd4dError(f'{name} must live on the GPU (no CPU fallback in graph-detr4d_amd)')
    if dtype is not None and t.dtype != dtype:
        raise TypeError(f'{name} must be {dtype}, got {t.dtype}')
    if not t.is_contiguous():
        raise ValueError(f'{name} must be contiguous')
    return ctypes.c_void_p(t.data_ptr())


def _stream():
    return ctypes.c_void_p(torch.cuda.current_stream().cuda_stream)


# ... 1600 lines not shown

def distill_loss_fwd_bwd(s_cls, s_box, t_cls, t_box, assigned, code_weights, avg_factors, reweight_score=False,
                         loss_cls_weight=1.0, loss_reg_weight=1.0):
    lib = _lib.load()
    f32, i32 = torch.float32, torch.int32
    nl, b, qs, c = s_cls.shape
    qt = t_cls.shape[2]
    if tuple(assigned.shape) != (nl, b, qs) or tuple(t_box.shape) != (nl, b, qt, 10) or tuple(t_cls.shape) != (nl, b, qt, c):
        raise ValueError('distill_loss_fwd_bwd: shapes disagree')
    loss = torch.empty(nl, 2, device=s_cls.device, dtype=f32)
    gcls, gbox = torch.empty_like(s_cls), torch.empty_like(s_box)
    code = lib.gd4d_distill_loss_fwd_bwd(_dev(s_cls, 's_cls', f32), _dev(s_box, 's_box', f32), _dev(t_cls, 't_cls', f32),
                                         _dev(t_box, 't_box', f32), _dev(assigned, 'assigned', i32),
                                         _dev(code_weights, 'code_weights', f32), _dev(avg_factors, 'avg_factors', f32),
                                         _dev(loss, 'loss'), _dev(gcls, 'grad_cls'), _dev(gbox, 'grad_box'), nl, b, qs, qt, c,
                                         s_box.shape[-1], 1 if reweight_score else 0, float(loss_cls_weight), float(loss_reg_weight),
                                         _stream())
    _lib.check(code, 'gd4d_distill_loss_fwd_bwd')
    return loss, gcls, gbox


def _feat_distill_levels(levels, name, like=None):
    if not levels or any(t.dim() != 4 for t in levels) or any(t.shape[0] != levels[0].shape[0] or t.shape[1] != levels[0].shape[1] for t in levels):
        raise ValueError(f'{name}: levels (R, C, H_l, W_l) with the same R and C expected')
    if like is not None and [tuple(t.shape) for t in levels] != [tuple(t.shape) for t in like]:
        raise ValueError(f'{name}: the levels\' shapes differ from the other pyramid\'s')
    nl = len(levels)
    ptrs = (ctypes.c_void_p * nl)(*[_dev(t, name, torch.float32).value for t in levels])
    lv = (ctypes.c_int32 * (2 * nl))(*[int(x) for t in levels for x in t.shape[2:]])
    return ptrs, lv, int(levels[0].shape[0])


def feat_distill_stats_fwd(teacher, temperature=0.5):
    lib = _lib.load()
    f32 = torch.float32
    tp, lv, r = _feat_distill_levels(teacher, 'teacher')
    nl, c, dev = len(teacher), int(teacher[0].shape[1]), teacher[0].device
    a_c = [torch.empty(r, t.shape[2] * t.shape[3], device=dev, dtype=f32) for t in teacher]
    a_s = [torch.empty(r, c, device=dev, dtype=f32) for t in teacher]
    ws = torch.empty(max(int(lib.gd4d_feat_distill_stats_workspace_bytes(lv, nl, r)), 16), device=dev, dtype=torch.uint8)
    cp = (ctypes.c_void_p * nl)(*[_dev(t, 'a_c', f32).value for t in a_c])
    sp = (ctypes.c_void_p * nl)(*[_dev(t, 'a_s', f32).value for t in a_s])
    code = lib.gd4d_feat_distill_stats_fwd(tp, lv, nl, r, c, float(temperature), cp, sp, _dev(ws, 'workspace', torch.uint8), ws.numel(),
                                           _stream())
    _lib.check(code, 'gd4d_feat_distill_stats_fwd')
    return a_c, a_s


def feat_distill_fwd(student, teacher, weight, bias, loss_weight, a_c=None, a_s=None):
    lib = _lib.load()
    f32 = torch.float32
    sp, lv, r = _feat_distill_levels(student, 'student')
    tp, _, _ = _feat_distill_levels(teacher, 'teacher', like=student)
    nl, c, dev = len(student), int(student[0].shape[1]), student[0].device
    if tuple(weight.shape) != (nl, c, c) or tuple(bias.shape) != (nl, c):
        raise ValueError(f'feat_distill_fwd: weight ({nl}, {c}, {c}) and bias ({nl}, {c}) expected')
    if (a_c is None) != (a_s is None):
        raise ValueError('feat_distill_fwd: both attention maps or neither')
    cp = ap = None
    if a_c is not None:
        if len(a_c) != nl or len(a_s) != nl or any(tuple(m.shape) != (r, s.shape[2] * s.shape[3]) for m, s in zip(a_c, student)) or \
                any(tuple(m.shape) != (r, c) for m in a_s):
            raise ValueError('feat_distill_fwd: a_c[l] (R, H_l W_l) and a_s[l] (R, C) expected')
        cp = (ctypes.c_void_p * nl)(*[_dev(t, 'a_c', f32).value for t in a_c])
        ap = (ctypes.c_void_p * nl)(*[_dev(t, 'a_s', f32).value for t in a_s])
    loss = torch.empty(1, device=dev, dtype=f32)
    gx = [torch.empty_like(s) for s in student]
    gw, gb = torch.empty_like(weight), torch.empty_like(bias)
    gp = (ctypes.c_void_p * nl)(*[_dev(t, 'grad_student', f32).value for t in gx])
    ws = torch.empty(max(int(lib.gd4d_feat_distill_workspace_bytes(lv, nl, r)), 16), device=dev, dtype=torch.uint8)
    code = lib.gd4d_feat_distill_fwd(sp, tp, lv, nl, r, c, _dev(weight, 'weight', f32), _dev(bias, 'bias', f32), cp, ap, float(loss_weight),
                                     _dev(loss, 'loss', f32), gp, _dev(gw, 'grad_weight', f32), _dev(gb, 'grad_bias', f32),
                                     _dev(ws, 'workspace', torch.uint8), ws.numel(), _stream())
    _lib.check(code, 'gd4d_feat_distill_fwd')
    return loss, gx, gw, gb


class ChainOp(ctypes.Structure):
    _fields_ = [('kind', ctypes.c_int32), ('src', ctypes.c_int32), ('dst', ctypes.c_int32), ('res', ctypes.c_int32),
                ('K', ctypes.c_int32), ('N', ctypes.c_int32), ('flags', ctypes.c_int32), ('dst_col', ctypes.c_int32),
                ('ld0', ctypes.c_int32), ('ld1', ctypes.c_int32), ('ld2', ctypes.c_int32), ('ldg', ctypes.c_int32),
                ('eps', ctypes.c_float), ('reserved', ctypes.c_int32),
                ('p0', ctypes.c_void_p), ('p1', ctypes.c_void_p), ('p2', ctypes.c_void_p), ('gout', ctypes.c_void_p),
                ('p3', ctypes.c_void_p)]


CHAIN_LOAD, CHAIN_GEMM, CHAIN_LAYERNORM, CHAIN_ADD, CHAIN_REFINE, CHAIN_SMALL_LINEAR, CHAIN_HEADGEMM, CHAIN_SIGNAL, CHAIN_WAIT = 1, 2, 3, 4, 5, 6, 7, 8, 9
CHAIN_LN_BWD, CHAIN_DROPMASK = 10, 11
CHAIN_RELU, CHAIN_INV_SIGMOID, CHAIN_SIGMOID, CHAIN_EXACT, CHAIN_SRC2, CHAIN_SPLIT_OUT, CHAIN_MASK_P2, CHAIN_DROPOUT = 1, 2, 4, 8, 16, 32, 64, 128
CHAIN_SPLIT_KV, CHAIN_SPLIT_KV_KEEP, CHAIN_ADD_GOUT = 256, 512, 1024


def _rows(t, name):
    if t is None:
        return None, 0
    if not t.is_cuda or t.dtype != torch.float32:
        raise _lib.Gd4dError(f'{name} must be a float32 GPU tensor')
    if t.dim() == 1:
        return t.data_ptr(), 0
    if t.stride(-1) != 1:
        raise ValueError(f'{name}: the last dimension must be dense')
    ld = t.stride(-2)
    for d in range(t.dim() - 2):
        if t.shape[d] != 1 and t.stride(d) != t.stride(d + 1) * t.shape[d + 1]:
            raise ValueError(f'{name}: rows must have one stride')
    return t.data_ptr(), ld


def chain_load(dst, x, x2=None, dst_col=0, inv_sigmoid=False, out=None):
    p0, ld0 = _rows(x, 'x')
    p1, ld1 = _rows(x2, 'x2')
    g, ldg = _rows(out, 'out')
    return ChainOp(kind=CHAIN_LOAD, src=-1, dst=dst, res=-1, N=x.shape[-1], dst_col=dst_col, ld0=ld0, ld1=ld1, ldg=ldg,
                   flags=CHAIN_INV_SIGMOID if inv_sigmoid else 0, p0=p0, p1=p1, gout=g)


_CHAIN_IMAGES = {}
_CHAIN_EPOCH = [0]


def invalidate_chain_images():
    for table in (_CHAIN_IMAGES, _VP_IMAGES, _STACKED):
        table.clear()
    _CHAIN_EPOCH[0] += 1


class _Stamp:
    __slots__ = ('_refs', '_marks', '_epoch')

    def __init__(self, sources=(), on_death=None):
        self._refs = [weakref.ref(_base(t), on_death) for t in sources if t is not None]
        self._marks = [_mark(t) for t in sources]
        self._epoch = _CHAIN_EPOCH[0] if sources else -1

    def valid(self, sources):
        return self._epoch == _CHAIN_EPOCH[0] and all(r() is not None for r in self._refs) and [_mark(t) for t in sources] == self._marks

    def __reduce__(self):
        return _Stamp, ()


def _base(t):
    return t if t._base is None else t._base


def _mark(t):
    return None if t is None else (id(_base(t)), t.data_ptr(), t.shape, t.dtype, t.device, t._version)


def _kept(table, key, sources, build):
    hit = table.get(key)
    if hit is not None and hit[0].valid(sources):
        return hit[1]
    value = build()
    table[key] = (_Stamp(sources, lambda _r: table.pop(key, None)), value)
    return value


def chain_weight_image(weight, exact=False):
    if not weight.is_cuda or weight.dtype != torch.float32 or weight.dim() != 2 or weight.stride(1) != 1 \
            or weight.stride(0) != weight.shape[1]:
        raise ValueError('chain weights must be dense (N, K) float32 GPU tensors')

    def build():
        lib = _lib.load()
        n, k = weight.shape
        nbytes = (lib.gd4d_chain_weight_image_exact_bytes if exact else lib.gd4d_chain_weight_image_bytes)(n, k)
        if nbytes == 0:
            raise _lib.Gd4dError(f'chain GEMM: K = {k} must be a multiple of 64')
        img = torch.empty(nbytes, device=weight.device, dtype=torch.uint8)
        with torch.cuda.device(weight.device):
            fn = lib.gd4d_chain_weight_image_exact if exact else lib.gd4d_chain_weight_image
            code = fn(ctypes.c_void_p(weight.data_ptr()), n, k, ctypes.c_void_p(img.data_ptr()), _stream())
# ... 156 lines not shown
    img, n, k = _image_of(weight, ALL_EXACT[0])
    op = ChainOp(kind=CHAIN_GEMM, src=src, dst=-1, res=src2, K=k, N=n, flags=CHAIN_SRC2 | (CHAIN_EXACT if ALL_EXACT[0] else 0), ld0=int(split),
                 ldg=ldg, p0=img, p1=None if bias is None else bias.data_ptr(), gout=g)
    if kv is not None:
        if n != 3 * kv.c or kv.c != 256 or kv.heads != 8:
            raise ValueError('kv planes: the packed in-projection of 256 channels, 8 heads')
        op.flags |= CHAIN_SPLIT_KV | (CHAIN_SPLIT_KV_KEEP if keep_fp32 else 0)
        op.p2, op.ld2 = kv.k.data_ptr(), kv.k[0].numel()
        op.p3, op.ld1 = kv.v.data_ptr(), kv.v[0].numel()
    return op


_STACKED = {}


def _stacked_linears(linears):
    def build():
        with torch.no_grad():
            w = torch.cat([m.weight for m in linears], 0).contiguous()
            b = torch.cat([m.bias if m.bias is not None else m.weight.new_zeros(m.weight.shape[0]) for m in linears], 0).contiguous()
        return w, b
    if len(_STACKED) > 256:
        _STACKED.clear()
    return _kept(_STACKED, tuple(id(m) for m in linears), [t for m in linears for t in (m.weight, m.bias)], build)


def chain_gemm_three_outputs(src, linears, outs, stacked=None, exact=False):
    if len(linears) != 3 or len(outs) != 3:
        raise ValueError('chain_gemm_three_outputs takes three Linears and three outputs')
    ptrs = [_rows(o, 'out') for o in outs]
    for (ptr, ld), m in zip(ptrs, linears):
        if ld != m.weight.shape[0]:
            raise ValueError('chain_gemm_three_outputs: every output must be dense, as wide as its Linear')
    if stacked is not None:
        img, n, k = _image_of(stacked[0], exact)
        b = stacked[1]
    else:
        w, b = _stacked_linears(linears)
        img, n, k = _image_of(w, exact)
    return ChainOp(kind=CHAIN_GEMM, src=src, dst=-1, res=-1, K=k, N=n, flags=CHAIN_SPLIT_OUT | (CHAIN_EXACT if exact else 0),
                   ldg=ptrs[0][1], ld2=ptrs[1][1], ld1=ptrs[2][1], p0=img, p1=b.data_ptr(),
                   gout=ptrs[0][0], p2=ptrs[1][0], p3=ptrs[2][0])


def chain_headgemm(agg, wsum, weight, bias=None, dst=-1, res=-1, out=None, addend=None):
    heads, k = agg.shape[-2], agg.shape[-1]
    img, n, wk = _image_of(weight)
    if wk != k or n % heads or (n // heads) % 32 or wsum.numel() * k != agg.numel():
        raise ValueError('chain_headgemm: weight (N, K), agg (..., Hh, K), wsum (..., Hh) with (N / Hh) % 32 == 0')
    if addend is not None and (out is not None or dst < 0 or addend.shape[-1] != n):
        raise ValueError('chain_headgemm: an addend (M, N) goes with dst >= 0 and no `out`')
    g, ldg = _rows(out if addend is None else addend, 'out')
    return ChainOp(kind=CHAIN_HEADGEMM, src=-1, dst=dst, res=res, K=k, N=n, ld0=heads, ldg=ldg, p0=img,
                   flags=CHAIN_ADD_GOUT if addend is not None else 0,
                   p1=None if bias is None else bias.data_ptr(), p2=_dev(agg, 'agg', torch.float32).value,
                   p3=_dev(wsum, 'wsum', torch.float32).value, gout=g)


def chain_small_linear(src, weight, bias, dst, relu=False, inv_sigmoid=False, out=None):
    g, ldg = _rows(out, 'out')
    return ChainOp(kind=CHAIN_SMALL_LINEAR, src=src, dst=dst, res=-1, K=weight.shape[1], N=weight.shape[0], ldg=ldg, gout=g,
                   flags=(CHAIN_RELU if relu else 0) | (CHAIN_INV_SIGMOID if inv_sigmoid else 0), p0=weight.data_ptr(),
                   p1=None if bias is None else bias.data_ptr())


def chain_layernorm_bwd(src, x_buf, norm, dst=-1, relu=False, out=None, part=None):
    g, ldg = _rows(out, 'out')
    p3, ld3 = (None, 0) if isinstance(x_buf, int) else _rows(x_buf, 'x')
    return ChainOp(kind=CHAIN_LN_BWD, src=src, dst=dst, res=x_buf if isinstance(x_buf, int) else -1, N=norm.weight.shape[0],
                   eps=float(norm.eps), flags=CHAIN_RELU if relu else 0, ldg=ldg, ld1=ld3, p0=norm.weight.data_ptr(),
                   p1=norm.bias.data_ptr(), p2=None if part is None else _dev(part, 'part', torch.float32).value, gout=g, p3=p3)


def chain_layernorm(src, norm, dst=-1, relu=False, out=None, dst2=-1, add=None):
    g, ldg = _rows(out, 'out')
    p2, ld2 = _rows(add, 'add')
    if (p2 is None) != (dst2 < 0):
        raise ValueError('chain_layernorm: dst2 and add go together')
    return ChainOp(kind=CHAIN_LAYERNORM, src=src, dst=dst, res=dst2, N=norm.weight.shape[0], eps=float(norm.eps),
                   flags=CHAIN_RELU if relu else 0, ldg=ldg, ld2=ld2, p0=norm.weight.data_ptr(), p1=norm.bias.data_ptr(),
                   p2=p2, gout=g)


def chain_add(dst, src, n, res=-1, add=None, out=None):
    p2, ld2 = _rows(add, 'add')
    g, ldg = _rows(out, 'out')
    return ChainOp(kind=CHAIN_ADD, src=src, dst=dst, res=res, N=n, ld2=ld2, p2=p2, ldg=ldg, gout=g)


def chain_refine(src, ref, out, dst=-1):
    return ChainOp(kind=CHAIN_REFINE, src=src, dst=dst, res=-1, p0=ref.data_ptr(), gout=out.data_ptr())


def chain_signal(flags):
    return ChainOp(kind=CHAIN_SIGNAL, src=-1, dst=-1, res=-1, gout=_dev(flags, 'flags', torch.int32).value)


_HANDOFF = {}


def _handoff_state(device):
    device = torch.device(device)
    idx = device.index if device.index is not None else torch.cuda.current_device()
    st = _HANDOFF.get(idx)
    if st is None:
        dev = torch.device('cuda', idx)
        st = _HANDOFF[idx] = {'word': None, 'dev': dev, 'pinned': None, 'event': None, 'placement': None}
    return st


def handoff_error_word(device):
    st = _handoff_state(device)
    if st['word'] is None:
        st['word'] = torch.zeros(1, device=st['dev'], dtype=torch.int32)
    return st['word']


_HANDOFF_FLAGS = {}


def handoff_flags(device, rows, cols, slot_key):
    device = torch.device(device)
    key = (device.index, slot_key, int(rows), int(cols))
    buf = _HANDOFF_FLAGS.get(key)
    if buf is None:
        if torch.cuda.is_current_stream_capturing():
            return torch.zeros(rows, cols, device=device, dtype=torch.int32)
        buf = _HANDOFF_FLAGS[key] = torch.zeros(rows, cols, device=device, dtype=torch.int32)
    return buf


def check_handoff(device=None):
    sts = list(_HANDOFF.items()) if device is None else [(None, _handoff_state(device))]
    for _, st in sts:
        if st['word'] is None:
            continue
        n = int(st['word'].item())
        st['event'] = None
        if n:
            st['word'].zero_()
            for buf in _HANDOFF_FLAGS.values():
                buf.zero_()
            st['placement'] = False
            raise _lib.Gd4dError(f'{n} SIGNAL / WAIT hand-off(s) between chain programs timed out: the affected rows are NaN. '
                                 'GD4D_POS_ENCODER=dual / GD4D_TRAIN_REG_BESIDE=0 run the same step without hand-offs.')


def poll_handoff(device):
    if torch.cuda.is_current_stream_capturing():
        return
    st = _handoff_state(device)
    if st['word'] is None:
        return
    if st['event'] is not None and st['event'].query():
        st['event'] = None
        if int(st['pinned'][0]) != 0:
            check_handoff(device)
    if st['event'] is None:
        if st['pinned'] is None:
            st['pinned'] = torch.zeros(1, dtype=torch.int32).pin_memory()
        st['pinned'].copy_(st['word'], non_blocking=True)
        st['event'] = torch.cuda.Event()
        st['event'].record()


def handoff_placement_ok(device):
    st = _handoff_state(device)
    if st['placement'] is None:
        if torch.cuda.is_current_stream_capturing():
            import warnings
            warnings.warn('graph-detr4d_amd: first use inside a graph capture - the XCD placement self-test cannot run, the step is '
                          'built without SIGNAL / WAIT hand-offs (run one eager forward before capturing to get them)')
            return False
        lib = _lib.load()
        idx = torch.device(device).index
        with torch.cuda.device(idx if idx is not None else torch.cuda.current_device()):
            blocks = 2048
            out = torch.full((blocks,), -1, device=st['dev'], dtype=torch.int32)
            _lib.check(lib.gd4d_xcd_placement_probe(_dev(out, 'out', torch.int32), blocks, _stream()), 'gd4d_xcd_placement_probe')
            ids = out.cpu()
        st['placement'] = bool((ids >= 0).all() and (ids == ids[:8].repeat(blocks // 8)).all())
        if not st['placement']:
            import warnings
            warnings.warn('graph-detr4d_amd: workgroups j and j + 8 k do not share an XCD on this device - chain programs run '
                          'without SIGNAL / WAIT hand-offs')
    return st['placement']


def handoff_enabled(device, env):
    import os
    if os.environ.get(env, '1') in ('0', 'dual'):
        return False
    return handoff_placement_ok(device)


def chain_wait(flags, errors=None):
    return ChainOp(kind=CHAIN_WAIT, src=-1, dst=-1, res=-1, p0=_dev(flags, 'flags', torch.int32).value,
                   gout=None if errors is None else _dev(errors, 'errors', torch.int32).value)


class ChainGuest(ctypes.Structure):
    _fields_ = [('feats', ctypes.c_void_p * 8), ('level_hw', ctypes.c_int32 * 16), ('L', ctypes.c_int32), ('R', ctypes.c_int32),
                ('chlast', ctypes.c_int32), ('workgroups', ctypes.c_int32), ('image', ctypes.c_void_p), ('out', ctypes.c_void_p)]


_VP_IMAGES = {}


def value_proj_image(weight, bias=None):
    if not weight.is_cuda or weight.dtype != torch.float32 or tuple(weight.shape) != (256, 256) or not weight.is_contiguous():
        raise ValueError('value_proj_image: a contiguous (256, 256) float32 GPU weight')
    if bias is not None and (bias.dtype != torch.float32 or bias.numel() != 256 or not bias.is_contiguous() or bias.device != weight.device):
        raise ValueError('value_proj_image: bias (256) float32 on the weight\'s GPU')

    def build():
        lib = _lib.load()
        img = torch.empty(int(lib.gd4d_value_proj_image_bytes()), device=weight.device, dtype=torch.uint8)
        code = lib.gd4d_value_proj_image(_dev(weight, 'weight', torch.float32), None if bias is None else _dev(bias, 'bias', torch.float32),
                                         _dev(img, 'image'), _stream())
        _lib.check(code, 'gd4d_value_proj_image')
        return img
    return _kept(_VP_IMAGES, (weight.data_ptr(), None if bias is None else bias.data_ptr()), (weight, bias), build)


def chain_guest(levels, image, out, workgroups=0):
    chlast = [PyramidView.is_channels_last_level(t) and not t.is_contiguous() for t in levels]
    if any(chlast) != all(chlast) or (not any(chlast) and not all(t.is_contiguous() for t in levels)):
        raise ValueError('chain_guest: the levels must be all NCHW-contiguous or all channels-last')
    if any(t.dtype != torch.float32 or not t.is_cuda or t.shape[-3] != 256 for t in levels) or len(levels) > 4:
        raise ValueError('chain_guest: up to 4 float32 GPU levels of 256 channels')
    r = levels[0].numel() // (256 * levels[0].shape[-1] * levels[0].shape[-2])
    s = sum(t.shape[-1] * t.shape[-2] for t in levels)
    if tuple(out.shape) != (r, s, 256) or out.dtype != torch.float32 or not out.is_contiguous() or out.device != levels[0].device:
        raise ValueError(f'chain_guest: out must be ({r}, {s}, 256) float32, contiguous')
    g = ChainGuest()
    for i, t in enumerate(levels):
        g.feats[i] = t.data_ptr()
        g.level_hw[2 * i], g.level_hw[2 * i + 1] = int(t.shape[-2]), int(t.shape[-1])
    g.L, g.R, g.chlast, g.workgroups = len(levels), r, int(all(chlast)), int(workgroups)
    g.image, g.out = image.data_ptr(), out.data_ptr()
    g._keep = (levels, image, out)
    return g


def value_proj_guest_fwd(guest, max_cus=0):
    code = _lib.load().gd4d_value_proj_guest_fwd(ctypes.byref(guest), int(max_cus), _stream())
    _lib.check(code, 'gd4d_value_proj_guest_fwd')


def _chain_fills(lib, a, na, b, nb, m, fills):
    jobs, start, records, fb, fn, fhh = fills
    arr = (FillJob * len(jobs))(*[FillJob(_dev(pl.buf, 'plan', torch.uint8).value, _dev(sl, 'slots').value,
                                           None if pl.order is None else _order_ptr(pl.order, fb * pl.q).value, int(base), int(pl.q))
                                   for pl, sl, base in jobs])
    code = lib.gd4d_row_chain_fill_fwd(a, na, b, nb, int(m), arr, len(jobs), _dev(start, 'start', torch.int32), _dev(records, 'records'),
                                       fb, fn, fhh, int(jobs[0][0].points), 0, _stream())
    _lib.check(code, 'gd4d_row_chain_fill_fwd')


def row_chain_fwd(program, m, guest=None, fills=None):
    lib = _lib.load()
    arr = (ChainOp * len(program))(*program)
    if fills is not None:
        return _chain_fills(lib, arr, len(program), None, 0, m, fills)
    if guest is not None:
        code = lib.gd4d_row_chain_guest_fwd(arr, len(program), None, 0, int(m), ctypes.byref(guest), _stream())
        _lib.check(code, 'gd4d_row_chain_guest_fwd')
        return
    code = lib.gd4d_row_chain_fwd(arr, len(program), int(m), _stream())
    _lib.check(code, 'gd4d_row_chain_fwd')


def row_chain2_fwd(program_a, program_b, m, guest=None, fills=None):
    lib = _lib.load()
    a = (ChainOp * len(program_a))(*program_a)
    b = (ChainOp * len(program_b))(*program_b)
    if fills is not None:
        return _chain_fills(lib, a, len(program_a), b, len(program_b), m, fills)
    if guest is not None:
        code = lib.gd4d_row_chain_guest_fwd(a, len(program_a), b, len(program_b), int(m), ctypes.byref(guest), _stream())
        _lib.check(code, 'gd4d_row_chain_guest_fwd')
        return
    code = lib.gd4d_row_chain2_fwd(a, len(program_a), b, len(program_b), int(m), _stream())
    _lib.check(code, 'gd4d_row_chain2_fwd')


def mha_core_presplit_fwd(q, kv, num_heads, attn_mask=None, want_lse=False, dropout_p=0., seed=None):
    lib = _lib.load()
    lq, b, c = q.shape
    _, _, _, _, _, _, kind, mptr, keep = _mha_args(q, q, q, num_heads, attn_mask)
    if b != 1 or lq != kv.m or c != kv.c or num_heads != kv.heads:
        raise ValueError('mha_core_presplit_fwd: batch 1, the planes of these rows')
    if not q.is_cuda or q.dtype != torch.float32 or q.stride(2) != 1:
        raise _lib.Gd4dError('q must be a float32 GPU tensor with unit channel stride')
    d = c // num_heads
    out = torch.empty(lq, 1, c, device=q.device, dtype=torch.float32)
    lse = torch.empty(lq, 1, num_heads, device=q.device, dtype=torch.float32) if want_lse else None
    sptr = _mha_seed(dropout_p, seed, q.device)
    code = lib.gd4d_mha_core_presplit_fwd(ctypes.c_void_p(q.data_ptr()), ctypes.c_void_p(kv.k.data_ptr()),
                                          ctypes.c_void_p(kv.v.data_ptr()), _dev(out, 'out'), lq, num_heads, d, q.stride(0), c,
                                          kv.k[0].numel(), kv.v[0].numel(), mptr, kind, 1.0 / (d ** 0.5),
                                          None if lse is None else _dev(lse, 'lse'), float(dropout_p), sptr, _stream())
    _lib.check(code, 'gd4d_mha_core_presplit_fwd')
    return (out, lse) if want_lse else out


class RequestRef(ctypes.Structure):
    _fields_ = [('binding', ctypes.c_int32), ('reserved', ctypes.c_int32), ('value', ctypes.c_int64)]


class RequestPatch(ctypes.Structure):
    _fields_ = [('table', ctypes.c_int32), ('binding', ctypes.c_int32), ('offset', ctypes.c_int64), ('add', ctypes.c_int64)]


class RequestBinding(ctypes.Union):
    _fields_ = [('ptr', ctypes.c_void_p), ('scalar', ctypes.c_double)]


class RequestStep(ctypes.Structure):
    _fields_ = [('kind', ctypes.c_int32), ('side', ctypes.c_int32), ('event', ctypes.c_int32), ('npatches', ctypes.c_int32),
                ('nops_a', ctypes.c_int32), ('nops_b', ctypes.c_int32), ('fbind', ctypes.c_int32 * 2),
                ('prog_a', ctypes.c_void_p), ('prog_b', ctypes.c_void_p), ('guest', ctypes.c_void_p), ('patches', ctypes.c_void_p),
                ('p', RequestRef * 10), ('i', ctypes.c_int32 * 10), ('l', ctypes.c_int64 * 2), ('f', ctypes.c_float * 2),
                ('table', ctypes.c_void_p * 5), ('table_bytes', ctypes.c_int64 * 5)]


(REQ_ROW_CHAIN, REQ_ROW_CHAIN2, REQ_ROW_CHAIN_GUEST, REQ_MHA_CORE, REQ_MHA_PRESPLIT, REQ_PLAN, REQ_AGG_COARSE, REQ_AGG_ITEMS,
 REQ_AGG_SLICED, REQ_SLICE_PLANAR, REQ_VALUE_PROJ_GUEST, REQ_QUERY_ORDER, REQ_EVENT_RECORD, REQ_STREAM_WAIT, REQ_COPY) = range(1, 16)


def _addr(a):
    if a is None:
        return 0
    if isinstance(a, int):
        return a
    return a.value or 0


def tensor_extent(t):
    span = sum((n - 1) * st for n, st in zip(t.shape, t.stride())) + 1 if t.numel() else 0
    return t.data_ptr(), t.data_ptr() + span * t.element_size()


class _Pending:

    def __init__(self, kind, side, **kw):
        self.kind, self.side, self.event = kind, side, 0
        self.prog_a = self.prog_b = self.guest = None
        self.p, self.i, self.l, self.f, self.tables, self.special, self.fbind = [], [], [], [], [], {}, [-1, -1]
        for k, v in kw.items():
            setattr(self, k, v)


_CHAIN_POINTERS = ('p0', 'p1', 'p2', 'gout', 'p3')


class StepRecorder:

    RUN_NOW = {'gd4d_chain_weight_image', 'gd4d_chain_weight_image_exact', 'gd4d_value_proj_image', 'gd4d_xcd_placement_probe'}

    def __init__(self, lib, main_stream):
        self._lib, self.main, self.side = lib, int(main_stream), None
        self.pending, self.events = [], 0

    def __getattr__(self, name):
        if name.startswith('gd4d_'):
            fn = getattr(self._lib, name)
            if name in self.RUN_NOW or not fn.argtypes or name.endswith('_bytes') or fn.restype is not ctypes.c_int:
                return fn
            raise _lib.Gd4dError(f'{name}: a request program (GD4D_REQUEST=1) has no step for this entry point - the route '
                                 'switches in force select a schedule it does not cover')
        raise AttributeError(name)

    def _side(self, handle):
        handle = int(_addr(handle))
        if handle == self.main:
            return 0
        if self.side not in (None, handle):
            raise _lib.Gd4dError('a request program runs on two streams: the caller\'s and one side stream')
        self.side = handle
        return 1

    def record_event(self, stream):
        if self.events >= 64:
            raise _lib.Gd4dError('a request program holds at most 64 events')
        self.pending.append(_Pending(REQ_EVENT_RECORD, self._side(stream.cuda_stream), event=self.events))
        self.events += 1
        return self.events - 1

    def wait_event(self, stream, event):
        self.pending.append(_Pending(REQ_STREAM_WAIT, self._side(stream.cuda_stream), event=event))

    def copy(self, dst, src):
        if not (dst.is_contiguous() and src.is_contiguous()) or dst.numel() != src.numel() or dst.dtype != src.dtype:
            raise ValueError('request program: a copy step takes two dense tensors of one size')
        self.pending.append(_Pending(REQ_COPY, self._side(torch.cuda.current_stream(dst.device).cuda_stream),
                                     p=[dst.data_ptr(), src.data_ptr()], l=[dst.numel() * dst.element_size()]))

    @staticmethod
    def _ops(arr, n):
        return None if arr is None or n == 0 else (ChainOp * n).from_buffer_copy(arr)

    @staticmethod
    def _guest(ref):
        return ChainGuest.from_buffer_copy(ref._obj)

    def gd4d_row_chain_fwd(self, a, na, m, stream):
        self.pending.append(_Pending(REQ_ROW_CHAIN, self._side(stream), prog_a=self._ops(a, na), i=[m]))
        return 0

    def gd4d_row_chain2_fwd(self, a, na, b, nb, m, stream):
        self.pending.append(_Pending(REQ_ROW_CHAIN2, self._side(stream), prog_a=self._ops(a, na), prog_b=self._ops(b, nb), i=[m]))
        return 0

    def gd4d_row_chain_guest_fwd(self, a, na, b, nb, m, guest, stream):
        self.pending.append(_Pending(REQ_ROW_CHAIN_GUEST, self._side(stream), prog_a=self._ops(a, na), prog_b=self._ops(b, nb), i=[m],
                                     guest=self._guest(guest)))
        return 0

    def gd4d_value_proj_guest_fwd(self, guest, max_cus, stream):
        self.pending.append(_Pending(REQ_VALUE_PROJ_GUEST, self._side(stream), guest=self._guest(guest), i=[max_cus]))
        return 0

    def gd4d_mha_core_fwd(self, q, k, v, mask, out, lq, lk, b, h, d, ldq, ldk, ldv, ldo, kind, scale, lse, drop_p, seed, stream):
        if _addr(lse) or drop_p:
            raise _lib.Gd4dError('request program: the attention core without lse / dropout (inference)')
        self.pending.append(_Pending(REQ_MHA_CORE, self._side(stream), p=[q, k, v, mask, out], i=[lq, lk, b, h, d, ldq, ldk, ldv, ldo, kind],
                                     f=[scale]))
        return 0

    def gd4d_mha_core_presplit_fwd(self, q, kp, vp, out, l, h, d, ldq, ldo, ks, vs, mask, kind, scale, lse, drop_p, seed, stream):
        if _addr(lse) or drop_p:
            raise _lib.Gd4dError('request program: the attention core without lse / dropout (inference)')
        self.pending.append(_Pending(REQ_MHA_PRESPLIT, self._side(stream), p=[q, kp, vp, out, mask], i=[l, h, d, ldq, ldo, kind], l=[ks, vs],
                                     f=[scale]))
        return 0

# ... 455 lines not shown
```

include/gd4d.h:

```cpp
#ifndef GD4D_H_
#define GD4D_H_

#include <stddef.h>
#include <stdint.h>

#ifdef __cplusplus
extern "C" {
#endif

#define GD4D_ABI_VERSION 56

enum { GD4D_F32 = 0, GD4D_BF16 = 1, GD4D_F16 = 2 };

enum { GD4D_LAYOUT_PIXEL_MAJOR = 0, GD4D_LAYOUT_HEAD_MAJOR = 1 };

enum { GD4D_VP_PRECISION_F32 = 0, GD4D_VP_PRECISION_BF16 = 1 };

enum {
  GD4D_OK = 0,
  GD4D_EINVAL = -1,
  GD4D_EUNSUPPORTED = -2,
  GD4D_EALIGN = -3,
  GD4D_ELAUNCH = -4,
  GD4D_EWORKSPACE = -5
// ... 100 lines not shown
                             int channels_last, void* stream);

int gd4d_query_order_fwd(const float* ref, const double* pc_range, int32_t* order, int B, int Q, void* stream);

int gd4d_refine_reference_order_fwd(const float* tmp, const float* ref, float* out, const double* pc_range,
                                    int32_t* order, int B, int Q, int ldt, void* stream);

int gd4d_detr3d_fwd(const void* const* feats, const int32_t* level_hw, const float* ref,
                    const float* attn_logits, const float* lidar2img, const double* pc_range,
                    float img_h, float img_w, float* out, uint8_t* mask_out, float* sampled_out,
                    int B, int N, int Q, int C, int L, int P, void* stream);

int gd4d_detr3d_bwd(const void* const* feats, const int32_t* level_hw, const float* ref, const float* attn_logits,
                    const float* lidar2img, const double* pc_range, float img_h, float img_w, const float* grad_out,
                    void* const* grad_feats, float* grad_logits, float* grad_ref, int B, int N, int Q, int C, int L, int P,
                    void* stream);

int gd4d_detr3d_v2_fwd(const void* const* feats, const int32_t* level_hw, const float* ref,
                       const float* attn_logits, const float* offsets, const float* lidar2img,
                       const double* pc_range, float img_h, float img_w, float* out, uint8_t* mask_out, int B,
                       int N, int Q, int C, int Hh, int L, int P, void* stream);
int gd4d_detr3d_v2_bwd(const void* const* feats, const int32_t* level_hw, const float* ref, const float* attn_logits,
                       const float* offsets, const float* lidar2img, const double* pc_range, float img_h, float img_w,
                       const float* grad_out, void* const* grad_feats, float* grad_logits, float* grad_offsets, float* grad_ref,
                       int B, int N, int Q, int C, int L, int Hh, void* stream);

int gd4d_value_proj_fwd(const void* const* feats, const int32_t* level_hw, const float* weight,
                        const float* bias, void* out, int R, int C, int L, int Hh, int in_dtype,
                        int out_dtype, int out_layout, int precision, void* workspace, size_t workspace_bytes,
                        int max_cus, void* stream);
size_t gd4d_value_proj_workspace_bytes(int NL);

int gd4d_value_proj_multi_fwd(const void* const* feats, const int32_t* level_hw,
                              const float* const* weights, const float* const* biases,
                              void* const* outs, int R, int C, int L, int NL, int Hh, int in_dtype,
                              int out_dtype, int out_layout, int precision, void* workspace,
                              size_t workspace_bytes, int max_cus, void* stream);

int gd4d_value_proj_bwd_input(const float* grad_out, const float* weight, float* const* grad_feats,
                              const int32_t* level_hw, int R, int C, int L, int accumulate, void* stream);
size_t gd4d_value_proj_bwd_weight_workspace_bytes(void);
int gd4d_value_proj_bwd_weight(const float* grad_out, const void* const* feats, const int32_t* level_hw,
                               float* grad_weight, float* grad_bias, void* workspace, size_t workspace_bytes, int R,
                               int C, int L, void* stream);

#define GD4D_LIN_RELU 1
#define GD4D_LIN_INV_SIGMOID_IN 2
#define GD4D_LIN_RELU_AFTER_LN 4
#define GD4D_LIN_WEIGHT_KN 8
#define GD4D_GEMM_RELU_IN 16
#define GD4D_GEMM_MASK_C 32
int gd4d_linear_fwd(const float* x, const float* x2, const float* w, const float* bias,
                    const float* r1, const float* r2, float* y, int M, int K, int N, int n_split,
                    int flags, int ldx, int ldy, int ldr1, int ldr2, float* xsum, void* stream);

int gd4d_linear_group_fwd(const float* x, const float* x2, const float* const* w, const float* const* bias,
                          float* const* y, const int32_t* n_out, int G, int M, int K, int ldx, float* xsum, void* stream);

int gd4d_linear_bwd_weight(const float* x, const float* grad_y, float* grad_w, float* grad_b, int M, int K, int N,
                           int ldx, int ldy, int accumulate, void* stream);
int gd4d_linear_bwd_weight_group(const void* const* x, const void* const* grad_y, void* const* grad_w, void* const* grad_b,
                                 const int32_t* dims, int count, int accumulate, void* stream);

int gd4d_layernorm_fwd(const float* x, const float* res, const float* gamma, const float* beta,
                       float* y, int M, int C, float eps, int relu, void* stream);

int gd4d_linear_ln_fwd(const float* x, const float* x2, const float* w, const float* bias, const float* r1,
                       const float* r2, const float* gamma, const float* beta, float* y, int M, int K, int N,
                       int n_split, int flags, float eps, int ldx, int ldy, int ldr1, int ldr2, void* stream);

enum { GD4D_CHAIN_LOAD = 1, GD4D_CHAIN_GEMM = 2, GD4D_CHAIN_LAYERNORM = 3, GD4D_CHAIN_ADD = 4, GD4D_CHAIN_REFINE = 5,
       GD4D_CHAIN_SMALL_LINEAR = 6, GD4D_CHAIN_HEADGEMM = 7, GD4D_CHAIN_SIGNAL = 8, GD4D_CHAIN_WAIT = 9, GD4D_CHAIN_LN_BWD = 10, GD4D_CHAIN_DROPMASK = 11 };
#define GD4D_CHAIN_RELU 1
#define GD4D_CHAIN_INV_SIGMOID 2
#define GD4D_CHAIN_SIGMOID 4
#define GD4D_CHAIN_EXACT 8
#define GD4D_CHAIN_SRC2 16
#define GD4D_CHAIN_SPLIT_OUT 32
#define GD4D_CHAIN_MASK_P2 64
#define GD4D_CHAIN_DROPOUT 128
#define GD4D_CHAIN_SPLIT_KV 256
#define GD4D_CHAIN_SPLIT_KV_KEEP 512
#define GD4D_CHAIN_ADD_GOUT 1024
#define GD4D_CHAIN_MAX_OPS 32
typedef struct gd4d_chain_op {
  int32_t kind, src, dst, res;
  int32_t K, N, flags, dst_col;
  int32_t ld0, ld1, ld2, ldg;
  float eps;
  int32_t reserved;
  const float* p0;
  const float* p1;
  const float* p2;
  float* gout;
  const float* p3;
} gd4d_chain_op;
size_t gd4d_chain_op_bytes(void);
size_t gd4d_chain_weight_image_bytes(int N, int K);
int gd4d_chain_weight_image(const float* weight, int N, int K, void* image, void* stream);
size_t gd4d_chain_weight_image_exact_bytes(int N, int K);
int gd4d_chain_weight_image_exact(const float* weight, int N, int K, void* image, void* stream);
#define GD4D_IMAGE_JOBS_MAX 1024
typedef struct gd4d_image_job {
  const float* seg[3];
  int32_t rows[3];
  int32_t cols, transposed, planes, frag0, reserved;
  void* image;
} gd4d_image_job;
size_t gd4d_image_job_bytes(void);
int gd4d_chain_weight_image_group(const gd4d_image_job* jobs_device, int count, int total_frags, void* stream);
int gd4d_row_chain_fwd(const gd4d_chain_op* program, int nops, int M, void* stream);
int gd4d_row_chain2_fwd(const gd4d_chain_op* program_a, int nops_a, const gd4d_chain_op* program_b, int nops_b, int M,
                        void* stream);

typedef struct gd4d_chain_guest {
  const void* feats[GD4D_MAX_LEVELS];
  int32_t level_hw[2 * GD4D_MAX_LEVELS];
  int32_t L, R, chlast, workgroups;
  const void* image;
  void* out;
} gd4d_chain_guest;
size_t gd4d_chain_guest_bytes(void);
size_t gd4d_value_proj_image_bytes(void);
int gd4d_value_proj_image(const float* weight, const float* bias, void* image, void* stream);
int gd4d_row_chain_guest_fwd(const gd4d_chain_op* program_a, int nops_a, const gd4d_chain_op* program_b, int nops_b, int M,
                             const gd4d_chain_guest* guest, void* stream);
int gd4d_value_proj_guest_fwd(const gd4d_chain_guest* job, int max_cus, void* stream);

int gd4d_mha_core_presplit_fwd(const float* q, const void* k_planes, const void* v_planes, float* out, int L, int H, int D,
                               int ldq, int ldo, long long k_plane_stride, long long v_plane_stride, const void* mask,
                               int mask_kind, float scale, float* lse, float drop_p, const void* seed, void* stream);

size_t gd4d_mlp2_image_bytes(int K1, int H, int N2);
int gd4d_mlp2_image(const float* w1, const float* b1, const float* w2, int K1, int H, int N2, void* image, void* stream);
int gd4d_mlp2_bf16x3_fwd(const float* x, const void* image, const float* b2, float* out, int M, int K1, int H, int N2, int ldx,
                         int ldo, void* stream);
int gd4d_mlp2_se_fuse_fwd(const void* const* feats, const int32_t* level_hw, int L, int R, const void* image, const float* b2,
                          const float* pe, const float* sine, void* const* outs, int C, int H, void* stream);
int gd4d_mlp2_frustum_fwd(const float* img2lidar, const int32_t* level_hw, int L, int R, float pad_h, float pad_w, int D,
                          float depth_start, const double* pc_range, const void* image, const float* b2, float* out, int H, int ldo,
                          void* stream);
int gd4d_mlp2_pe_se_fwd(const float* img2lidar, const void* const* feats, const int32_t* level_hw, int L, int R, float pad_h,
                        float pad_w, int D, float depth_start, const double* pc_range, const void* pe_image, const float* pe_b2,
                        int pe_H, const void* se_image, const float* se_b2, int se_H, const float* sine, void* const* outs,
                        float* pe_out, void* stream);

size_t gd4d_adamw_flat_workspace_bytes(void);
int gd4d_adamw_flat(float* params, const float* grads, float* exp_avg, float* exp_avg_sq, float* state, void* workspace,
                    size_t workspace_bytes, int64_t n, float lr, float beta1, float beta2, float eps, float weight_decay,
                    float max_norm, void* stream);

#define GD4D_RECIPE_MAX_RANGES 1024
#define GD4D_RECIPE_MAX_MILESTONES 16
enum { GD4D_LR_FIXED = 0, GD4D_LR_COSINE = 1, GD4D_LR_STEP = 2 };
enum { GD4D_WARMUP_NONE = 0, GD4D_WARMUP_CONSTANT = 1, GD4D_WARMUP_LINEAR = 2, GD4D_WARMUP_EXP = 3 };
typedef struct gd4d_recipe_range {
  int64_t begin, end;
  float lr_mult, decay_mult;
} gd4d_recipe_range;
typedef struct gd4d_recipe_state {
  int64_t iteration;
  int64_t optimizer_steps;
  int64_t skipped_steps;
  int64_t step_in_flight;
  float loss_scale;
  float scale_in_use;
  float lr;
  float grad_norm;
  int32_t found_inf;
  int32_t growth_tracker;
  int32_t reserved[2];
} gd4d_recipe_state;
typedef struct gd4d_recipe_config {
  double base_lr, end_lr, gamma, warmup_ratio;
  double init_scale, growth_factor, backoff_factor;
  int64_t iters_per_epoch, max_epochs, max_iters, warmup_iters, step_every;
  int64_t milestones[GD4D_RECIPE_MAX_MILESTONES];
  int32_t policy, by_epoch, warmup, n_milestones, dynamic_scale, growth_interval, zero_grads, reserved;
// ... 227 lines not shown
```

Baseline: 668.4.

## Fuse layernorm into preceding GEMM epilogue, stage op table in LDS, early wait prefetch

Adds a layernorm-epilogue mode to the row-chain GEMM and ADD ops, with a host-side pass that merges a GEMM/ADD followed by a layernorm into one op. The gamma, beta and residual operands are prefetched into LDS with global_load_lds while the GEMM runs. The chain op table is also copied into LDS and read with readfirstlane instead of coming from kernel-argument memory, and the wait op gains an early-prefetch flag. The intent is to cut per-op barriers and global-load latency between chained ops, at the cost of extra LDS use, a larger op struct and an ABI change.

```diff
diff --git a/graph-detr4d_amd/csrc/gd4d_rowchain.hip b/graph-detr4d_amd/csrc/gd4d_rowchain.hip
--- a/graph-detr4d_amd/csrc/gd4d_rowchain.hip
+++ b/graph-detr4d_amd/csrc/gd4d_rowchain.hip
@@ -48,6 +48,15 @@
 #endif
 #ifndef RC_PREFETCH
 #define RC_PREFETCH 1
+#endif
+#ifndef RC_OPS_LDS
+#define RC_OPS_LDS 1
+#endif
+#ifndef RC_LN_EPI
+#define RC_LN_EPI 1
+#endif
+#ifndef RC_WAIT_EARLY
+#define RC_WAIT_EARLY 1
 #endif
 #ifndef RC_TRACE_OPS
 #define RC_TRACE_OPS 0
@@ -143,8 +152,128 @@
   }
 }
 
+struct LnArgs {
+  const float* gamma;
+  const float* beta;
+  const float* add;
+  float* gout;
+  int src, dst, dst2, N, ld_add, ldg;
+  float eps;
+  bool relu;
+};
+template <int MAXCH>
+struct LnRegs { float4 gm[MAXCH], bt[MAXCH], ad[MAXCH]; };
+constexpr int RC_LN_EPI_CH = 4;
+
+__device__ __forceinline__ LnArgs rc_ln_of_op(const ChainOp& op) {
+  return LnArgs{op.p0, op.p1, op.p2, op.gout, op.src, op.dst, op.res, op.N, op.ld2, op.ldg, op.eps, (op.flags & GD4D_CHAIN_RELU) != 0};
+}
+__device__ __forceinline__ LnArgs rc_ln_of_epi(const ChainOp& op) {
+  const int d = op.reserved & 255, d2 = (op.reserved >> 8) & 255;
+  return LnArgs{op.ln_gamma, op.ln_beta, op.p3, op.gout, op.dst, d == 255 ? -1 : d, d2 == 255 ? -1 : d2, op.N, op.ld1, op.ldg, op.eps,
+                (op.reserved & (1 << 16)) != 0};
+}
+
+template <int MAXCH>
+__device__ __forceinline__ void rc_ln_request(const LnArgs& a, LnRegs<MAXCH>& rg, int m0, int M, int lane, int wave) {
+  if (wave >= RC_M / 4) return;
+  const int row = 4 * wave + (lane >> 4), l16 = lane & 15, N = a.N;
+  const bool second = a.dst2 >= 0 && a.add;
+  const size_t m_ld = (size_t)min(m0 + row, M - 1);
+#pragma unroll
+  for (int ch = 0; ch < MAXCH; ++ch) {
+    const int n = min(64 * ch, N - 64) + 4 * l16;
+    rg.gm[ch] = *reinterpret_cast<const float4*>(a.gamma + n);
+    rg.bt[ch] = *reinterpret_cast<const float4*>(a.beta + n);
+    if (second) rg.ad[ch] = *reinterpret_cast<const float4*>(a.add + m_ld * a.ld_add + n);
+  }
+}
+
+template <int MAXCH>
+__device__ __forceinline__ void rc_ln_apply(const LnArgs& a, const LnRegs<MAXCH>& rg, float (*bufs)[RC_M][RC_LD], int m0, int M, int lane,
+                                            int wave) {
+  if (wave >= RC_M / 4) return;
+  const int row = 4 * wave + (lane >> 4), l16 = lane & 15, N = a.N, nch = N / 64;
+  const bool second = a.dst2 >= 0 && a.add;
+  float4 x[MAXCH];
+#pragma unroll
+  for (int ch = 0; ch < MAXCH; ++ch) x[ch] = *reinterpret_cast<const float4*>(&bufs[a.src][row][min(64 * ch, N - 64) + 4 * l16]);
+  float s = 0.f;
+#pragma unroll
+  for (int ch = 0; ch < MAXCH; ++ch)
+    if (ch < nch) s += (x[ch].x + x[ch].y) + (x[ch].z + x[ch].w);
+#pragma unroll
+  for (int o = 1; o < 16; o <<= 1) s += __shfl_xor(s, o);
+  const float mean = s / (float)N;
+  float q = 0.f;
+#pragma unroll
+  for (int ch = 0; ch < MAXCH; ++ch)
+    if (ch < nch) {
+      const float a_ = x[ch].x - mean, b = x[ch].y - mean, c = x[ch].z - mean, d = x[ch].w - mean;
+      q += (a_ * a_ + b * b) + (c * c + d * d);
+    }
+#pragma unroll
+  for (int o = 1; o < 16; o <<= 1) q += __shfl_xor(q, o);
+  const float rstd = 1.0f / sqrtf(q / (float)N + a.eps);
+  const int m = m0 + row;
+#pragma unroll
+  for (int ch = 0; ch < MAXCH; ++ch) {
+    if (ch >= nch) break;
+    const int n = 64 * ch + 4 * l16;
+    const float4 gm = rg.gm[ch], bt = rg.bt[ch];
+    float4 v;
+    v.x = (x[ch].x - mean) * rstd * gm.x + bt.x; v.y = (x[ch].y - mean) * rstd * gm.y + bt.y;
+    v.z = (x[ch].z - mean) * rstd * gm.z + bt.z; v.w = (x[ch].w - mean) * rstd * gm.w + bt.w;
+    if (a.relu) { v.x = fmaxf(v.x, 0.f); v.y = fmaxf(v.y, 0.f); v.z = fmaxf(v.z, 0.f); v.w = fmaxf(v.w, 0.f); }
+    if (a.dst >= 0) *reinterpret_cast<float4*>(&bufs[a.dst][row][n]) = v;
+    if (a.gout && m < M) *reinterpret_cast<float4*>(a.gout + (size_t)m * a.ldg + n) = v;
+    if (second) {
+      const float4 ad = rg.ad[ch];
+      *reinterpret_cast<float4*>(&bufs[a.dst2][row][n]) = make_float4(ad.x + v.x, ad.y + v.y, ad.z + v.z, ad.w + v.w);
+    }
+  }
+}
+
+constexpr size_t RC_LN_PARK = sizeof(float) * 64 * RC_LN_EPI_CH * (2 + RC_M);
+__device__ __forceinline__ void rc_ln_request_lds(const LnArgs& a, char* park, int m0, int M, int lane, int wave) {
+  typedef __attribute__((address_space(3))) void lds_void_t;
+  typedef const __attribute__((address_space(1))) void glb_void_t;
+  const int nch = a.N / 64, units = (a.dst2 >= 0 && a.add) ? 2 + RC_M : 2;
+  for (int i = wave; i < units * nch; i += RC_WAVES) {
+    const int u = i / nch, ch = i - u * nch;
+    const float* src = u == 0 ? a.gamma : u == 1 ? a.beta : a.add + (size_t)min(m0 + u - 2, M - 1) * a.ld_add;
+    __builtin_amdgcn_global_load_lds((glb_void_t*)(src + 64 * ch + lane), (lds_void_t*)(park + sizeof(float) * (64 * RC_LN_EPI_CH * u + 64 * ch)), 4, 0, 0);
+  }
+}
+__device__ __forceinline__ void rc_ln_fetch_lds(const LnArgs& a, LnRegs<RC_LN_EPI_CH>& rg, const char* park, int lane, int wave) {
+  if (wave >= RC_M / 4) return;
+  const float* f = reinterpret_cast<const float*>(park);
+  const int row = 4 * wave + (lane >> 4), l16 = lane & 15;
+#pragma unroll
+  for (int ch = 0; ch < RC_LN_EPI_CH; ++ch) {
+    const int n = min(64 * ch, a.N - 64) + 4 * l16;
+    rg.gm[ch] = *reinterpret_cast<const float4*>(f + n);
+    rg.bt[ch] = *reinterpret_cast<const float4*>(f + 64 * RC_LN_EPI_CH + n);
+    rg.ad[ch] = *reinterpret_cast<const float4*>(f + 64 * RC_LN_EPI_CH * (2 + row) + n);
+  }
+}
+__device__ __forceinline__ void rc_ln_epilogue(const LnArgs& a, char* park, float (*bufs)[RC_M][RC_LD], int m0, int M, int lane, int wave) {
+  asm volatile("s_waitcnt vmcnt(0)" ::: "memory");
+  __syncthreads();
+  LnRegs<RC_LN_EPI_CH> rg;
+  rc_ln_fetch_lds(a, rg, park, lane, wave);
+  rc_ln_apply(a, rg, bufs, m0, M, lane, wave);
+}
+
+__device__ __forceinline__ void rc_layernorm(const ChainOp& op, float (*bufs)[RC_M][RC_LD], int m0, int M, int lane, int wave) {
+  const LnArgs a = rc_ln_of_op(op);
+  LnRegs<RC_W / 64> rg;
+  rc_ln_request(a, rg, m0, M, lane, wave);
+  rc_ln_apply(a, rg, bufs, m0, M, lane, wave);
+}
+
 template <bool EXACT, bool TRAIN>
-__device__ __forceinline__ void rc_gemm(const ChainOp& op, float (*bufs)[RC_M][RC_LD], int m0, int M, int lane, int wave) {
+__device__ __forceinline__ void rc_gemm(const ChainOp& op, float (*bufs)[RC_M][RC_LD], int m0, int M, int lane, int wave, char* ln_park) {
   constexpr int FRAG = EXACT ? 3072 : 2048;
   const int i16 = lane & 15, g = lane >> 4;
   const int K = op.K, N = op.N;
@@ -158,6 +287,10 @@
   const bool drop = TRAIN && (op.flags & GD4D_CHAIN_DROPOUT) != 0;
   const uint32_t drop_lo = drop ? reinterpret_cast<const uint32_t*>(op.p3)[0] : 0u;
   const uint32_t drop_hi = drop ? reinterpret_cast<const uint32_t*>(op.p3)[1] : 0u;
+  const bool ln_epi = RC_LN_EPI && !TRAIN && (op.flags & GD4D_CHAIN_LN_EPI) != 0;
+  const LnArgs ln_a = rc_ln_of_epi(op);
+  if (ln_epi) rc_ln_request_lds(ln_a, ln_park, m0, M, lane, wave);
+  const bool add2 = op.p3 && !drop && !ln_epi;
   for (int n_base = RC_COLS * wave; n_base < N; n_base += RC_COLS * RC_WAVES) {
     const float* a_row = &bufs[(src2 && n_base >= op.ld0) ? op.res : op.src][i16][RC_KG * g];
     const char* wf[RC_TILES];
@@ -182,7 +315,7 @@
         for (int r = 0; r < 4; ++r) {
           const size_t m = (size_t)min(m0 + 4 * g + r, M - 1);
           const float a2 = op.p2[m * op.ld2 + n];
-          e_add[c][r] = (op.p3 && !drop) ? a2 + op.p3[m * op.ld1 + n] : a2;
+          e_add[c][r] = add2 ? a2 + op.p3[m * op.ld1 + n] : a2;
         }
       }
     }
@@ -269,7 +402,7 @@
                               : const_cast<float*>(op.p3) + (size_t)m * op.ld1 + (n - c2);
             *o = v;
           }
-        } else if (op.gout && m < M && !(split_kv && !kv_fp32_too && n_base >= RC_COLS * RC_WAVES)) {
+        } else if (op.gout && !ln_epi && m < M && !(split_kv && !kv_fp32_too && n_base >= RC_COLS * RC_WAVES)) {
           op.gout[(size_t)m * op.ldg + n] = v;
         }
       }
@@ -303,6 +436,7 @@
       }
     }
   }
+  if (ln_epi) rc_ln_epilogue(ln_a, ln_park, bufs, m0, M, lane, wave);
 }
 
 __device__ __forceinline__ void rc_headgemm(const ChainOp& op, float (*bufs)[RC_M][RC_LD], int m0, int M, int lane, int wave) {
@@ -398,55 +532,6 @@
         if (op.gout && !(op.flags & GD4D_CHAIN_ADD_GOUT) && m < M) op.gout[(size_t)m * op.ldg + n] = v;
       }
     }
-  }
-}
-
-__device__ __forceinline__ void rc_layernorm(const ChainOp& op, float (*bufs)[RC_M][RC_LD], int m0, int M, int lane, int wave) {
-  constexpr int MAXCH = RC_W / 64;
-  if (wave >= RC_M / 4) return;
-  const int row = 4 * wave + (lane >> 4), l16 = lane & 15, N = op.N, nch = N / 64;
-  float4 gm[MAXCH], bt[MAXCH], x[MAXCH], ad[MAXCH];
-  const bool second = op.res >= 0 && op.p2;
-  const size_t m_ld = (size_t)min(m0 + row, M - 1);
-#pragma unroll
-  for (int ch = 0; ch < MAXCH; ++ch) {
-    const int n = min(64 * ch, N - 64) + 4 * l16;
-    gm[ch] = *reinterpret_cast<const float4*>(op.p0 + n);
-    bt[ch] = *reinterpret_cast<const float4*>(op.p1 + n);
-    if (second) ad[ch] = *reinterpret_cast<const float4*>(op.p2 + m_ld * op.ld2 + n);
-    x[ch] = *reinterpret_cast<const float4*>(&bufs[op.src][row][n]);
-  }
-  float s = 0.f;
-#pragma unroll
-  for (int ch = 0; ch < MAXCH; ++ch)
-    if (ch < nch) s += (x[ch].x + x[ch].y) + (x[ch].z + x[ch].w);
-#pragma unroll
-  for (int o = 1; o < 16; o <<= 1) s += __shfl_xor(s, o);
-  const float mean = s / (float)N;
-  float q = 0.f;
-#pragma unroll
-  for (int ch = 0; ch < MAXCH; ++ch)
-    if (ch < nch) {
-      const float a = x[ch].x - mean, b = x[ch].y - mean, c = x[ch].z - mean, d = x[ch].w - mean;
-      q += (a * a + b * b) + (c * c + d * d);
-    }
-#pragma unroll
-  for (int o = 1; o < 16; o <<= 1) q += __shfl_xor(q, o);
-  const float rstd = 1.0f / sqrtf(q / (float)N + op.eps);
-  const int m = m0 + row;
-  const bool relu = op.flags & GD4D_CHAIN_RELU;
-#pragma unroll
-  for (int ch = 0; ch < MAXCH; ++ch) {
-    if (ch >= nch) break;
-    const int n = 64 * ch + 4 * l16;
-    float4 v;
-    v.x = (x[ch].x - mean) * rstd * gm[ch].x + bt[ch].x; v.y = (x[ch].y - mean) * rstd * gm[ch].y + bt[ch].y;
-    v.z = (x[ch].z - mean) * rstd * gm[ch].z + bt[ch].z; v.w = (x[ch].w - mean) * rstd * gm[ch].w + bt[ch].w;
-    if (relu) { v.x = fmaxf(v.x, 0.f); v.y = fmaxf(v.y, 0.f); v.z = fmaxf(v.z, 0.f); v.w = fmaxf(v.w, 0.f); }
-    if (op.dst >= 0) *reinterpret_cast<float4*>(&bufs[op.dst][row][n]) = v;
-    if (op.gout && m < M) *reinterpret_cast<float4*>(op.gout + (size_t)m * op.ldg + n) = v;
-    if (second)
-      *reinterpret_cast<float4*>(&bufs[op.res][row][n]) = make_float4(ad[ch].x + v.x, ad[ch].y + v.y, ad[ch].z + v.z, ad[ch].w + v.w);
   }
 }
 
@@ -541,8 +626,18 @@
   }
 }
 
+__device__ __forceinline__ void rc_rows_request(const ChainOp& op, float4 (&va)[RC_ROWS_PER_WAVE][2], int m0, int M, int lane, int wave) {
+#pragma unroll
+  for (int r = 0; r < RC_ROWS_PER_WAVE; ++r) {
+    const int m = min(m0 + RC_ROWS_PER_WAVE * wave + r, M - 1);
+#pragma unroll
+    for (int cb = 0; cb < 2; ++cb) va[r][cb] = *reinterpret_cast<const float4*>(op.p0 + (size_t)m * op.ld0 + min(256 * cb + 4 * lane, op.N - 4));
+  }
+}
+
 template <bool IS_ADD, bool TRAIN>
-__device__ __forceinline__ void rc_rows(const ChainOp& op, float (*bufs)[RC_M][RC_LD], int m0, int M, int lane, int wave) {
+__device__ __forceinline__ void rc_rows(const ChainOp& op, float (*bufs)[RC_M][RC_LD], int m0, int M, int lane, int wave,
+                                        const float4 (*pre)[2] = nullptr) {
   const int N = op.N;
   const float* ga = IS_ADD ? op.p2 : op.p0;
   const float* gb = IS_ADD ? nullptr : op.p1;
@@ -554,7 +649,7 @@
 #pragma unroll
     for (int cb = 0; cb < 2; ++cb) {
       const int n = min(256 * cb + 4 * lane, N - 4);
-      va[r][cb] = ga ? *reinterpret_cast<const float4*>(ga + (size_t)m * lda + n) : make_float4(0.f, 0.f, 0.f, 0.f);
+      va[r][cb] = pre ? pre[r][cb] : ga ? *reinterpret_cast<const float4*>(ga + (size_t)m * lda + n) : make_float4(0.f, 0.f, 0.f, 0.f);
       vb[r][cb] = gb ? *reinterpret_cast<const float4*>(gb + (size_t)m * ldb + n) : make_float4(0.f, 0.f, 0.f, 0.f);
     }
   }
@@ -586,6 +681,16 @@
   int nops, M, nops2, split;
   ChainOp ops[GD4D_CHAIN_MAX_OPS];
 };
+
+constexpr size_t RC_LDS_ROWS = sizeof(float) * RC_BUFS * RC_M * RC_LD;
+constexpr size_t RC_LDS_TABLE_AT = RC_LDS_ROWS + 256 * RC_WAVES;
+constexpr size_t RC_LDS_TABLE = RC_OPS_LDS ? sizeof(ChainOp) * GD4D_CHAIN_MAX_OPS : 0;
+constexpr size_t RC_LDS_SCRATCH_AT = RC_LDS_TABLE_AT + RC_LDS_TABLE;
+constexpr size_t RC_LDS_INFER = RC_LDS_SCRATCH_AT + (RC_LN_EPI ? RC_LN_PARK : 0), RC_LDS_TRAIN = RC_LDS_SCRATCH_AT + sizeof(float) * 8 * RC_W;
+static_assert(sizeof(ChainOp) % 16 == 0 && RC_LDS_TABLE_AT % 16 == 0, "the table is copied and read in 16-byte pieces");
+static_assert(RC_LDS_TABLE <= 3584 && RC_LDS_TRAIN <= 160 * 1024 && RC_LDS_INFER <= 160 * 1024,
+              "row buffers 133120 + dump 2048 + table 3584 + (LN_EPI's operands 18432 | LN_BWD's sums 16384) = 157184 | 155136 of 163840 bytes");
+static_assert(sizeof(ChainProgram) + sizeof(VpaParams) + 8 <= 4096 && sizeof(ChainProgram) + sizeof(FillGuest) + 8 <= 4096, "the kernel argument segment");
 
 #if defined(__HIP_DEVICE_COMPILE__)
 typedef const __attribute__((address_space(4))) ChainProgram* rc_prog_ptr_t;
@@ -608,10 +713,29 @@
   const int tid = threadIdx.x, lane = tid & 63, wave = tid >> 6;
   const int m0 = wg * RC_M;
   trace_mark_if(g_trace_rowchain, (second ? 7ull : 1ull) | ((unsigned long long)nops << 8), wg == 0);
+#if RC_OPS_LDS
+  {
+    constexpr int PIECES = sizeof(ChainOp) / 16;
+    uint4* table = reinterpret_cast<uint4*>(rc_smem + RC_LDS_TABLE_AT);
+    const ChainProgram* gp = (const ChainProgram*)pp;
+    if (tid < nops * PIECES) table[tid] = reinterpret_cast<const uint4*>(gp->ops + op_base)[tid];
+    __syncthreads();
+  }
+  auto get_op = [&](int oi) -> ChainOp {
+    constexpr int WORDS = sizeof(ChainOp) / 4;
+    const uint32_t* t = reinterpret_cast<const uint32_t*>(rc_smem + RC_LDS_TABLE_AT) + (oi - op_base) * WORDS;
+    union { ChainOp op; uint32_t w[WORDS]; } u;
+#pragma unroll
+    for (int i = 0; i < WORDS; ++i) u.w[i] = (uint32_t)__builtin_amdgcn_readfirstlane((int)t[i]);
+    return u.op;
+  };
+#else
+  auto get_op = [&](int oi) -> ChainOp { const ChainOp o = pp->ops[oi]; return o; };
+#endif
 #if RC_PREFETCH
   typedef __attribute__((address_space(3))) void rc_lds_void_t;
   typedef const __attribute__((address_space(1))) void rc_glb_void_t;
-  rc_lds_void_t* rc_dump = (rc_lds_void_t*)(rc_smem + sizeof(float) * RC_BUFS * RC_M * RC_LD + 256 * wave);
+  rc_lds_void_t* rc_dump = (rc_lds_void_t*)(rc_smem + RC_LDS_ROWS + 256 * wave);
   auto touch1 = [&](const char* q) { __builtin_amdgcn_global_load_lds((rc_glb_void_t*)q, rc_dump, 4, 0, 0); };
   const unsigned xcd = (unsigned)bx & 7u;
   const unsigned first = (unsigned)wg_lo + ((xcd - (unsigned)wg_lo) & 7u);
@@ -625,7 +749,7 @@
   auto touch_small = [&](int from) {
     const int rows = min(RC_M, M - m0);
     for (int oi = from; oi < op_base + nops; ++oi) {
-      const ChainOp& o = pp->ops[oi];
+      const ChainOp o = get_op(oi);
       const size_t nb = (size_t)o.N * 4;
       switch (o.kind) {
         case GD4D_CHAIN_LOAD:
@@ -648,23 +772,24 @@
   };
   auto touch_images = [&]() {
     for (int oi = op_base; oi < op_base + nops; ++oi) {
-      if (pp->ops[oi].kind == GD4D_CHAIN_HEADGEMM) {
+      const ChainOp o = get_op(oi);
+      if (o.kind == GD4D_CHAIN_HEADGEMM) {
         const int rows = min(RC_M, M - m0);
-        const char* a = reinterpret_cast<const char*>(pp->ops[oi].p2 + (size_t)m0 * pp->ops[oi].ld0 * pp->ops[oi].K);
-        const unsigned pieces = (unsigned)rows * (unsigned)pp->ops[oi].ld0 * (unsigned)pp->ops[oi].K / 16u;
+        const char* a = reinterpret_cast<const char*>(o.p2 + (size_t)m0 * o.ld0 * o.K);
+        const unsigned pieces = (unsigned)rows * (unsigned)o.ld0 * (unsigned)o.K / 16u;
         for (unsigned c = tid; c < pieces; c += 64 * RC_WAVES) touch1(a + (size_t)c * 64);
       }
-      if (pp->ops[oi].kind != GD4D_CHAIN_GEMM && pp->ops[oi].kind != GD4D_CHAIN_HEADGEMM) continue;
-      const char* img = reinterpret_cast<const char*>(pp->ops[oi].p0);
-      const unsigned chunks = (unsigned)((pp->ops[oi].N + 15) / 16) * (unsigned)(pp->ops[oi].K / 32) *
-                              ((pp->ops[oi].flags & GD4D_CHAIN_EXACT) ? 48u : 32u);
+      if (o.kind != GD4D_CHAIN_GEMM && o.kind != GD4D_CHAIN_HEADGEMM) continue;
+      const char* img = reinterpret_cast<const char*>(o.p0);
+      const unsigned chunks = (unsigned)((o.N + 15) / 16) * (unsigned)(o.K / 32) *
+                              ((o.flags & GD4D_CHAIN_EXACT) ? 48u : 32u);
       const unsigned lo = (unsigned)((unsigned long long)chunks * mine / share), hi = (unsigned)((unsigned long long)chunks * (mine + 1) / share);
       for (unsigned c = lo + tid; c < hi; c += 64 * RC_WAVES) touch1(img + (size_t)c * 64);
     }
   };
   int lead = 0;
   if (RC_PREFETCH & 4)
-    while (lead < nops && pp->ops[op_base + lead].kind == GD4D_CHAIN_LOAD) ++lead;
+    while (lead < nops && get_op(op_base + lead).kind == GD4D_CHAIN_LOAD) ++lead;
   if (RC_PREFETCH & 2) touch_small(op_base + lead);
   if ((RC_PREFETCH & 1) && lead == 0) touch_images();
 #endif
@@ -675,7 +800,7 @@
 #if RC_PREFETCH
     if ((RC_PREFETCH & 1) && lead > 0 && oi == op_base + lead) touch_images();
 #endif
-    const ChainOp op = pp->ops[oi];
+    ChainOp op = get_op(oi);
     switch (op.kind) {
       case GD4D_CHAIN_LOAD: {
         if ((op.N & 3) == 0 && (op.dst_col & 3) == 0) { rc_rows<false, TRAIN>(op, bufs, m0, M, lane, wave); break; }
@@ -690,12 +815,21 @@
         break;
       }
       case GD4D_CHAIN_GEMM:
-        if (op.flags & GD4D_CHAIN_EXACT) rc_gemm<true, TRAIN>(op, bufs, m0, M, lane, wave);
-        else rc_gemm<false, TRAIN>(op, bufs, m0, M, lane, wave);
+        if (op.flags & GD4D_CHAIN_EXACT) rc_gemm<true, TRAIN>(op, bufs, m0, M, lane, wave, rc_smem + RC_LDS_SCRATCH_AT);
+        else rc_gemm<false, TRAIN>(op, bufs, m0, M, lane, wave, rc_smem + RC_LDS_SCRATCH_AT);
         break;
       case GD4D_CHAIN_HEADGEMM: rc_headgemm(op, bufs, m0, M, lane, wave); break;
       case GD4D_CHAIN_LAYERNORM: rc_layernorm(op, bufs, m0, M, lane, wave); break;
-      case GD4D_CHAIN_ADD: rc_rows<true, TRAIN>(op, bufs, m0, M, lane, wave); break;
+      case GD4D_CHAIN_ADD:
+        if (RC_LN_EPI && !TRAIN && (op.flags & GD4D_CHAIN_LN_EPI)) {
+          const LnArgs ln_a = rc_ln_of_epi(op);
+          rc_ln_request_lds(ln_a, rc_smem + RC_LDS_SCRATCH_AT, m0, M, lane, wave);
+          rc_rows<true, TRAIN>(op, bufs, m0, M, lane, wave);
+          rc_ln_epilogue(ln_a, rc_smem + RC_LDS_SCRATCH_AT, bufs, m0, M, lane, wave);
+          break;
+        }
+        rc_rows<true, TRAIN>(op, bufs, m0, M, lane, wave);
+        break;
       case GD4D_CHAIN_DROPMASK: {
         if (!TRAIN) break;
         const uint32_t lo = reinterpret_cast<const uint32_t*>(op.p0)[0], hi = reinterpret_cast<const uint32_t*>(op.p0)[1];
@@ -715,7 +849,7 @@
       }
       case GD4D_CHAIN_LN_BWD:
         if (TRAIN)
-          rc_layernorm_bwd(op, bufs, reinterpret_cast<float*>(rc_smem + sizeof(float) * RC_BUFS * RC_M * RC_LD + 256 * RC_WAVES), m0, M, wg, tid);
+          rc_layernorm_bwd(op, bufs, reinterpret_cast<float*>(rc_smem + RC_LDS_SCRATCH_AT), m0, M, wg, tid);
         break;
       case GD4D_CHAIN_SMALL_LINEAR: {
         const int K = op.K, N = op.N;
@@ -777,6 +911,13 @@
         break;
       }
       case GD4D_CHAIN_WAIT: {
+        const bool early = RC_WAIT_EARLY && !TRAIN && (op.flags & GD4D_CHAIN_EARLY_P0) != 0;
+        float4 pre[RC_ROWS_PER_WAVE][2];
+        ChainOp nxt = op;
+        if (early) {
+          nxt = get_op(oi + 1);
+          rc_rows_request(nxt, pre, m0, M, lane, wave);
+        }
         if (tid == 0) {
           const unsigned* f = reinterpret_cast<const unsigned*>(op.p0) + wg;
           unsigned spins = 0;
@@ -790,6 +931,16 @@
           }
           if (!rc_poison) __hip_atomic_store(const_cast<unsigned*>(f), 0u, __ATOMIC_RELAXED, __HIP_MEMORY_SCOPE_AGENT);
         }
+        if (early) {
+          __syncthreads();
+          poisoned = rc_poison != 0;
+#if RC_TRACE_OPS
+          trace_mark_if(g_trace_rowchain, 0x40ull | ((unsigned long long)op.kind << 8) | (second ? 1ull << 63 : 0ull), wg == 0);
+#endif
+          op = nxt;
+          ++oi;
+          rc_rows<false, TRAIN>(op, bufs, m0, M, lane, wave, pre);
+        }
         break;
       }
       default: break;
@@ -805,7 +956,8 @@
       __syncthreads();
     }
 #if RC_TRACE_OPS
-    trace_mark_if(g_trace_rowchain, 0x40ull | ((unsigned long long)op.kind << 8) | ((unsigned long long)op.N << 16) | ((unsigned long long)op.K << 32) | (second ? 1ull << 63 : 0ull), wg == 0);
+    trace_mark_if(g_trace_rowchain, 0x40ull | ((unsigned long long)op.kind << 8) | ((unsigned long long)op.N << 16) | ((unsigned long long)(op.K & 0xffff) << 32) |
+                  ((op.flags & GD4D_CHAIN_LN_EPI) ? 1ull << 62 : 0ull) | (second ? 1ull << 63 : 0ull), wg == 0);
 #endif
   }
   trace_mark_if(g_trace_rowchain, (second ? 0x87ull : 0x81ull) | ((unsigned long long)nops << 8), wg == 0);
@@ -920,6 +1072,20 @@
   return check_launch();
 }
 
+static int rc_validate_ln_epi(const gd4d_chain_op& op) {
+  using namespace gd4d;
+  if (op.kind == GD4D_CHAIN_GEMM && (op.flags & (GD4D_CHAIN_SPLIT_OUT | GD4D_CHAIN_SPLIT_KV | GD4D_CHAIN_SRC2))) return GD4D_EINVAL;
+  const int d = op.reserved & 255, d2 = (op.reserved >> 8) & 255, width = (op.reserved >> 17) & 1023;
+  if (op.N != width) return GD4D_EINVAL;
+  if (!op.ln_gamma || !op.ln_beta || op.dst < 0 || op.dst_col != 0) return GD4D_EINVAL;
+  if ((d != 255 && d >= RC_BUFS) || (d2 != 255 && d2 >= RC_BUFS) || (d == 255 && !op.gout)) return GD4D_EINVAL;
+  if ((d2 != 255) != (op.p3 != nullptr) || (d2 != 255 && (d2 == op.dst || d2 == d))) return GD4D_EINVAL;
+  if (op.N % 64 != 0 || op.N > 64 * RC_LN_EPI_CH) return GD4D_EUNSUPPORTED;
+  if (!aligned16(op.ln_gamma) || !aligned16(op.ln_beta) || (op.gout && (!aligned16(op.gout) || (op.ldg & 3)))) return GD4D_EALIGN;
+  if (op.p3 && (!aligned16(op.p3) || (op.ld1 & 3))) return GD4D_EALIGN;
+  return GD4D_OK;
+}
+
 static int rc_validate(const gd4d_chain_op* program, int nops, int which) {
   const bool two_programs = which != 0;
   using namespace gd4d;
@@ -927,6 +1093,11 @@
     const gd4d_chain_op& op = program[i];
     const bool buf_ok = op.src < RC_BUFS && op.dst < RC_BUFS && op.res < RC_BUFS;
     if (!buf_ok) return GD4D_EINVAL;
+    if (op.flags & GD4D_CHAIN_LN_EPI) {
+      if (!RC_LN_EPI) return GD4D_EUNSUPPORTED;
+      if (op.kind != GD4D_CHAIN_GEMM && op.kind != GD4D_CHAIN_ADD) return GD4D_EINVAL;
+      if (int rc = rc_validate_ln_epi(op)) return rc;
+    }
     switch (op.kind) {
       case GD4D_CHAIN_LOAD:
         if (!op.p0 || op.dst < 0 || op.N <= 0 || op.dst_col < 0 || op.dst_col + op.N > RC_W) return GD4D_EINVAL;
@@ -936,7 +1107,7 @@
         break;
       case GD4D_CHAIN_GEMM:
         if (!op.p0 || op.src < 0 || op.K <= 0 || op.N <= 0 || (op.dst < 0 && !op.gout)) return GD4D_EINVAL;
-        if (op.p3 && !op.p2 && !(op.flags & GD4D_CHAIN_DROPOUT)) return GD4D_EINVAL;
+        if (op.p3 && !op.p2 && !(op.flags & (GD4D_CHAIN_DROPOUT | GD4D_CHAIN_LN_EPI))) return GD4D_EINVAL;
         if (op.K % (32 * RC_DEPTH) != 0 || op.K > RC_W) return GD4D_EUNSUPPORTED;
         if (op.dst >= 0 && (op.dst_col < 0 || op.dst_col + op.N > RC_W)) return GD4D_EINVAL;
         if (op.dst >= 0 && op.dst == op.src) return GD4D_EINVAL;
@@ -1000,6 +1171,7 @@
         break;
       case GD4D_CHAIN_WAIT:
         if (!op.p0 || !op.gout || !two_programs || which != 2 || i + 1 >= nops || program[i + 1].kind != GD4D_CHAIN_LOAD) return GD4D_EINVAL;
+        if ((op.flags & GD4D_CHAIN_EARLY_P0) && ((program[i + 1].N & 3) || (program[i + 1].dst_col & 3))) return GD4D_EINVAL;
         break;
       default: return GD4D_EINVAL;
     }
@@ -1033,12 +1205,20 @@
               ((op.kind == GD4D_CHAIN_LOAD || op.kind == GD4D_CHAIN_ADD || op.kind == GD4D_CHAIN_SMALL_LINEAR) && op.gout);
     }
   }
+  if (train)
+    for (int w = 0; w < 2; ++w)
+      for (int i = 0; i < (w ? nb : na); ++i)
+        if ((w ? b : a)[i].flags & GD4D_CHAIN_LN_EPI) return GD4D_EINVAL;
+  if (fills)
+    for (int w = 0; w < 2; ++w)
+      for (int i = 0; i < (w ? nb : na); ++i)
+        if ((w ? b : a)[i].flags & (GD4D_CHAIN_LN_EPI | GD4D_CHAIN_EARLY_P0)) return GD4D_EINVAL;
   VpaParams g{};
   if (guest) {
     if (train) return GD4D_EUNSUPPORTED;
     if (int rc = va_guest_params(guest, g)) return rc;
   }
-  const size_t lds = sizeof(float) * RC_BUFS * RC_M * RC_LD + 256 * RC_WAVES + (train ? sizeof(float) * 8 * RC_W : 0);
+  const size_t lds = train ? RC_LDS_TRAIN : RC_LDS_INFER;
   const void* kern = train ? reinterpret_cast<const void*>(row_chain_kernel<true>) : reinterpret_cast<const void*>(row_chain_kernel<false>);
   if (!allow_dynamic_lds(kern, (int)lds)) return GD4D_ELAUNCH;
   const int blocks = (M + RC_M - 1) / RC_M;
@@ -1068,7 +1248,7 @@
   if (fills) {
     if (guest) return GD4D_EINVAL;
     const void* fk = reinterpret_cast<const void*>(row_chain_fill_kernel);
-    const size_t flds = sizeof(float) * RC_BUFS * RC_M * RC_LD + 256 * RC_WAVES + sizeof(float) * 8 * RC_W;
+    const size_t flds = RC_LDS_TRAIN;
     if (!allow_dynamic_lds(fk, (int)flds)) return GD4D_ELAUNCH;
     const int gbase = nb > 0 ? split + blocks : blocks;
     int cus = 256, dev = 0;
diff --git a/graph-detr4d_amd/functional.py b/graph-detr4d_amd/functional.py
--- a/graph-detr4d_amd/functional.py
+++ b/graph-detr4d_amd/functional.py
@@ -312,7 +312,7 @@
             return None
         src = dst
         i += 2 if relu else 1
-    return prog
+    return ops.chain_fuse_layernorms(prog)
 
 
 def head_outputs(hs, init_reference, inter_references, cls_branches, reg_branches, pc_range, depth_factor=None):
diff --git a/graph-detr4d_amd/fused_decoder.py b/graph-detr4d_amd/fused_decoder.py
--- a/graph-detr4d_amd/fused_decoder.py
+++ b/graph-detr4d_amd/fused_decoder.py
@@ -114,7 +114,7 @@
             ops.chain_layernorm(1, seq[1], dst=0, relu=True),
             ops.chain_gemm(0, seq[3].weight, seq[3].bias, dst=1),
             ops.chain_layernorm(1, seq[4], relu=True, out=out.view(q, -1))]
-    ops.row_chain_fwd(prog, q)
+    ops.row_chain_fwd(ops.chain_fuse_layernorms(prog), q)
     return out, ref3d
 
 
@@ -126,10 +126,10 @@
         head, src, inv = [], ref_buf, True
     mid = 1 if src != 1 else 2
     nxt = [b for b in (0, 2, 3) if b not in (src, mid)][0]
-    return head + [ops.chain_small_linear(src, seq[0].weight, seq[0].bias, mid, inv_sigmoid=inv),
-                   ops.chain_layernorm(mid, seq[1], dst=nxt, relu=True),
-                   ops.chain_gemm(nxt, seq[3].weight, seq[3].bias, dst=mid),
-                   ops.chain_layernorm(mid, seq[4], relu=True, out=out)]
+    return head + ops.chain_fuse_layernorms([ops.chain_small_linear(src, seq[0].weight, seq[0].bias, mid, inv_sigmoid=inv),
+                                             ops.chain_layernorm(mid, seq[1], dst=nxt, relu=True),
+                                             ops.chain_gemm(nxt, seq[3].weight, seq[3].bias, dst=mid),
+                                             ops.chain_layernorm(mid, seq[4], relu=True, out=out)])
 
 
 def run_single(decoder, query, query_pos, value, reference_points, reg_branches, img_metas, attn_masks, order,
@@ -202,6 +202,7 @@
             ref = new_ref
         else:
             prog_b = None if pos_late else _position_ops(ca, pos_feat.view(q, c), ref=ref.view(q, 3))
+        prog_a = ops.chain_fuse_layernorms(prog_a)
         if prog_b is None:
             ops.row_chain_fwd(prog_a, q)
         else:
@@ -223,7 +224,7 @@
             first = ops.chain_headgemm(agg_raw, wsum, ca.value_proj.weight, ca.value_proj.bias, dst=0)
         guest = late.coarse_guest(layers[lid + 1].attentions[1]) if coarse and not last else None
         x3 = out_all[slot]
-        prog = [first] + ([ops.chain_wait(flags[lid], err)] if pos_late else []) + [
+        prog = [first] + ([ops.chain_wait(flags[lid], err, early_x=True)] if pos_late else []) + [
                 ops.chain_load(3, x1, pos_feat.view(q, c)),
                 ops.chain_gemm(0, ca.output_proj.weight, ca.output_proj.bias, dst=1, res=3),
                 ops.chain_layernorm(1, layer.norms[1], dst=2),
@@ -249,6 +250,7 @@
                 pending = (lins, x3.view(q, c), ref, new_ref)
         elif return_intermediate or last:
             ops.copy_into(ref_all[slot], ref)
+        prog = ops.chain_fuse_layernorms(prog)
         if pos_late:
             ops.row_chain2_fwd(_position_ops(ca, pos_feat.view(q, c), ref=ref.view(q, 3)) + [ops.chain_signal(flags[lid])], prog, q,
                                guest=guest)
@@ -422,7 +424,7 @@
     return out_all, ref_all
 
 
-ROUTE_SWITCHES = ('GD4D_POS_ENCODER', 'GD4D_COARSE', 'GD4D_FIRST_PROJ', 'GD4D_MHA_FP32', 'GD4D_AGG', 'GD4D_PLAN', 'GD4D_PROJECT',
+ROUTE_SWITCHES = ('GD4D_LN_EPI', 'GD4D_WAIT_EARLY', 'GD4D_POS_ENCODER', 'GD4D_COARSE', 'GD4D_FIRST_PROJ', 'GD4D_MHA_FP32', 'GD4D_AGG', 'GD4D_PLAN', 'GD4D_PROJECT',
                   'GD4D_COPY_CUS', 'GD4D_COARSE_MAX_ROWS', 'GD4D_QUERY_ORDER')
 _PROGRAMS = weakref.WeakKeyDictionary()
 _B_QUERY, _B_POS, _B_REF, _B_L2I, _B_IMG_H, _B_IMG_W, _B_MASK, _B_OUT, _B_REFS, _B_LEVEL0 = range(10)
diff --git a/graph-detr4d_amd/ops.py b/graph-detr4d_amd/ops.py
--- a/graph-detr4d_amd/ops.py
+++ b/graph-detr4d_amd/ops.py
@@ -1706,13 +1706,13 @@
                 ('ld0', ctypes.c_int32), ('ld1', ctypes.c_int32), ('ld2', ctypes.c_int32), ('ldg', ctypes.c_int32),
                 ('eps', ctypes.c_float), ('reserved', ctypes.c_int32),
                 ('p0', ctypes.c_void_p), ('p1', ctypes.c_void_p), ('p2', ctypes.c_void_p), ('gout', ctypes.c_void_p),
-                ('p3', ctypes.c_void_p)]
+                ('p3', ctypes.c_void_p), ('ln_gamma', ctypes.c_void_p), ('ln_beta', ctypes.c_void_p)]
 
 
 CHAIN_LOAD, CHAIN_GEMM, CHAIN_LAYERNORM, CHAIN_ADD, CHAIN_REFINE, CHAIN_SMALL_LINEAR, CHAIN_HEADGEMM, CHAIN_SIGNAL, CHAIN_WAIT = 1, 2, 3, 4, 5, 6, 7, 8, 9
 CHAIN_LN_BWD, CHAIN_DROPMASK = 10, 11
 CHAIN_RELU, CHAIN_INV_SIGMOID, CHAIN_SIGMOID, CHAIN_EXACT, CHAIN_SRC2, CHAIN_SPLIT_OUT, CHAIN_MASK_P2, CHAIN_DROPOUT = 1, 2, 4, 8, 16, 32, 64, 128
-CHAIN_SPLIT_KV, CHAIN_SPLIT_KV_KEEP, CHAIN_ADD_GOUT = 256, 512, 1024
+CHAIN_SPLIT_KV, CHAIN_SPLIT_KV_KEEP, CHAIN_ADD_GOUT, CHAIN_LN_EPI, CHAIN_EARLY_P0 = 256, 512, 1024, 2048, 4096
 
 
 def _rows(t, name):
@@ -2035,6 +2035,44 @@
                    p2=p2, gout=g)
 
 
+def chain_ln_pack(dst, dst2, relu, width):
+    return (dst & 255) | ((dst2 & 255) << 8) | ((1 << 16) if relu else 0) | ((width & 1023) << 17)
+
+
+def ln_epi_enabled():
+    return os.environ.get('GD4D_LN_EPI', '1') != '0'
+
+
+def chain_fuse_layernorm(op, ln):
+    if ln.kind != CHAIN_LAYERNORM or op.kind not in (CHAIN_GEMM, CHAIN_ADD) or op.flags & CHAIN_LN_EPI:
+        return None
+    if op.dst < 0 or ln.src != op.dst or op.N != ln.N or op.N % 64 or op.N > 256 or op.gout or op.p3:
+        return None
+    if op.kind == CHAIN_GEMM and (op.dst_col or op.flags & (CHAIN_SPLIT_OUT | CHAIN_SPLIT_KV | CHAIN_SRC2 | CHAIN_MASK_P2 | CHAIN_DROPOUT)):
+        return None
+    if ln.res >= 0 and ln.res in (op.dst, ln.dst):
+        return None
+    out = ChainOp.from_buffer_copy(op)
+    out.flags |= CHAIN_LN_EPI
+    out.eps = ln.eps
+    out.reserved = chain_ln_pack(ln.dst if ln.dst >= 0 else 255, ln.res if ln.res >= 0 else 255, ln.flags & CHAIN_RELU, ln.N)
+    out.ln_gamma, out.ln_beta = ln.p0, ln.p1
+    out.gout, out.ldg = ln.gout, ln.ldg
+    out.p3, out.ld1 = ln.p2, ln.ld2
+    return out
+
+
+def chain_fuse_layernorms(program):
+    if not ln_epi_enabled():
+        return program
+    out, i = [], 0
+    while i < len(program):
+        fused = chain_fuse_layernorm(program[i], program[i + 1]) if i + 1 < len(program) else None
+        out.append(program[i] if fused is None else fused)
+        i += 1 if fused is None else 2
+    return out
+
+
 def chain_add(dst, src, n, res=-1, add=None, out=None):
     p2, ld2 = _rows(add, 'add')
     g, ldg = _rows(out, 'out')
@@ -2147,8 +2185,9 @@
     return handoff_placement_ok(device)
 
 
-def chain_wait(flags, errors=None):
+def chain_wait(flags, errors=None, early_x=False):
     return ChainOp(kind=CHAIN_WAIT, src=-1, dst=-1, res=-1, p0=_dev(flags, 'flags', torch.int32).value,
+                   flags=CHAIN_EARLY_P0 if early_x and os.environ.get('GD4D_WAIT_EARLY', '1') != '0' else 0,
                    gout=None if errors is None else _dev(errors, 'errors', torch.int32).value)
 
 
@@ -2305,7 +2344,7 @@
             setattr(self, k, v)
 
 
-_CHAIN_POINTERS = ('p0', 'p1', 'p2', 'gout', 'p3')
+_CHAIN_POINTERS = ('p0', 'p1', 'p2', 'gout', 'p3', 'ln_gamma', 'ln_beta')
 
 
 class StepRecorder:
diff --git a/include/gd4d.h b/include/gd4d.h
--- a/include/gd4d.h
+++ b/include/gd4d.h
@@ -206,6 +206,10 @@
 #define GD4D_CHAIN_SPLIT_KV 256
 #define GD4D_CHAIN_SPLIT_KV_KEEP 512
 #define GD4D_CHAIN_ADD_GOUT 1024
+#define GD4D_CHAIN_LN_EPI 2048
+#define GD4D_CHAIN_EARLY_P0 4096
+#define GD4D_CHAIN_LN_PACK(dst, dst2, relu, width) \
+  ((int32_t)(((dst) & 255) | (((dst2) & 255) << 8) | ((relu) ? 1 << 16 : 0) | (((width) & 1023) << 17)))
 #define GD4D_CHAIN_MAX_OPS 32
 typedef struct gd4d_chain_op {
   int32_t kind, src, dst, res;
@@ -218,6 +222,8 @@
   const float* p2;
   float* gout;
   const float* p3;
+  const float* ln_gamma;
+  const float* ln_beta;
 } gd4d_chain_op;
 size_t gd4d_chain_op_bytes(void);
 size_t gd4d_chain_weight_image_bytes(int N, int K);
```

Result: slower. 651.7 (-2.5%).
